# FudanCVL/SynFMC

Measured on AMD Instinct MI355X. Metric: denoising steps/sec, 16x320x512 bf16 U-Net+CMC+OMC, higher is better.
Workload: dtype bf16; 1 GPU; 16x320x512 clip, CFG batch 2, full-width 3D U-Net (1.39B params, random init) + Camera Adapter (CMC) + Object Motion Control (OMC) features, DDIM step; configs/obj.yaml shapes; 1 clip per GPU; frames=16, height=320, width=512, hip_graph=True, fp8_temporal_attention=False, parallelism=dp1 (independent clips, no collective)

## Files before the change

include/fmc_hip.h:

```cpp
#ifndef FMC_HIP_H
#define FMC_HIP_H

#include <stdint.h>

#ifdef __cplusplus
extern "C" {
#endif

#define FMC_VERSION 100

enum { FMC_BF16 = 0, FMC_F32 = 1 };

enum {
    FMC_OK = 0,
    FMC_E_SHAPE = -1,
    FMC_E_DTYPE = -2,
    FMC_E_ALIGN = -3,
    FMC_E_LAUNCH = -4,
    FMC_E_NULL = -5
};

int fmc_version(void);
const char* fmc_last_error(void);

int64_t fmc_groupnorm_workspace_bytes(int N, int C, int G);
int fmc_groupnorm_silu_fwd(const void* x, void* y, const float* gamma, const float* beta, float* stats,
                           void* workspace, int N, int HW, int C, int G, float eps, int act, int dtype,
                           const void* x2, int C1, void* stream);
int fmc_groupnorm_silu_bwd(const void* dy, const void* x, void* dx, const float* gamma, const float* beta,
                           const float* stats, void* workspace, int N, int HW, int C, int G, int act,
                           int dtype, void* stream);

int fmc_layernorm_fwd(const void* x, void* y, const float* gamma, const float* beta, const float* pe,
                      int64_t M, int C, float eps, int pe_inner, int pe_frames, int dtype, void* stream);
int fmc_layernorm_add_fwd(const void* x, const void* addend, void* sum_out, void* y, const float* gamma, const float* beta,
                          const float* pe, int64_t M, int C, float eps, int pe_inner, int pe_frames, int dtype, void* stream);

int fmc_geglu_fwd(const void* x, void* y, int64_t M, int Cff, int dtype, void* stream);

int fmc_spatial_attn_fwd(const void* q, const void* k, const void* v, void* o, float* lse, int B, int H,
                         int Sq, int Skv, int D, int64_t q_batch_stride, int64_t q_row_stride,
                         int64_t kv_batch_stride, int64_t kv_row_stride, int64_t o_batch_stride,
                         int64_t o_row_stride, int kv_batch_div, float scale, int dtype, void* stream);

int fmc_temporal_attn_fwd(const void* q, const void* k, const void* v, void* o, int n_clips, int n_pix,
                          int F, int H, int D, int64_t clip_stride, int64_t frame_stride,
                          int64_t pix_stride, int64_t o_clip_stride, int64_t o_frame_stride,
                          int64_t o_pix_stride, float scale, int dtype, void* stream);

int fmc_plucker_fwd(const float* K, const float* c2w, void* out, int B, int F, int H, int W, int c2w_rows,
                    int layout, int dtype, void* stream);

int fmc_omc_rasterize_fwd(const float* poses, const float* masks, void* feat, float* mask_out, int BF,
                          int n_obj, int H, int W, int layout, int dtype, void* stream);

int fmc_gaussian_circle_mask_fwd(const float* circles, float* out, int N, int H, int W, void* stream);

int fmc_mask_modulate_fwd(const void* x, const float* mask_in, void* y, float* mask_out, int N, int h, int w,
                          int C, int Hin, int Win, int dtype, void* stream);

int fmc_feature_add_fwd(const void* h, const void* t, void* out, int64_t n_elems, int64_t skip_elems,
                        int dtype, void* stream);

int fmc_cfg_ddim_step(const void* eps_uc, const float* x, float* x_out, int64_t n, int has_uncond,
                      float guidance, float alpha_t, float alpha_prev, int dtype, void* stream);

typedef struct fmc_sampler_coef {
    float g;
    float m_x, m_e, m_clamp;
    float c_x, c_e, c_m, c_n;
    float c_h[3];
    float in_scale;
} fmc_sampler_coef;
int64_t fmc_sampler_step_elems_per_trip(void);
int fmc_sampler_step(const void* eps_uc, const float* x, const void* noise, const float* hist0, const float* hist1,
                     const float* hist2, float* x_out, float* m_out, void* x_in, int64_t n, int has_uncond, int n_hist,
                     int in_reps, fmc_sampler_coef coef, int dtype, int in_dtype, void* stream);

int fmc_linear_bf16(const void* x, const void* w, const void* bias, const void* residual, void* out, int64_t M, int N,
                    int K, int64_t ldx, int64_t ldres, int64_t ldo, float alpha, int epilogue, int tile, int split_k,
                    void* workspace, int64_t workspace_bytes, const void* x2, int64_t ldx2, int k_split,
                    const void* residual2, void* stream);

int fmc_conv3x3_bf16(const void* x, const void* w, const void* bias, const void* temb, const void* residual, void* out,
                     int n_img, int H, int W, int Cin, int Cout, int64_t temb_row_stride, int temb_img_div,
                     int upsample2x, int tile, int split_k, void* workspace, int64_t workspace_bytes, void* stream);

int fmc_linear_bf16_gn(const void* x, const void* w, const void* bias, const void* residual, void* out, int64_t M, int N, int K,
                       int64_t ldx, int64_t ldres, int64_t ldo, float alpha, const void* residual2, float* gn_partials, int gn_hw,
                       int w_tilemajor, void* stream);
int fmc_linear_bf16_ln(const void* x, const void* w, const void* bias, const void* residual, void* out, int64_t M, int N, int K,
                       int64_t ldx, int64_t ldres, int64_t ldo, float alpha, const void* residual2, void* ln_out, const float* ln_gamma,
                       const float* ln_beta, float ln_eps, const float* ln_pe, int ln_pe_inner, int ln_pe_frames, float* ln_stats, int w_tilemajor,
                       void* stream);
int fmc_linear_bf16_lnc(const void* x, const void* w_gamma, void* out, int64_t M, int N, int K, int64_t ldx, int64_t ldo, int epilogue,
                        const float* ln_stats, const float* ln_c, const float* ln_bias, int w_tilemajor, void* stream);
int fmc_linear_bf16_ffblk(const void* x, const void* w, const void* bias, const void* residual, void* out, int64_t M, int N, int K,
                          int64_t ldres, float alpha, int epilogue, int x_blocked, int out_blocked, const float* ln_stats, const float* ln_c,
                          const float* ln_bias, int w_tilemajor, void* stream);
int fmc_groupnorm_fold_linear(const float* partials, int part_splits, const float* gamma, const float* beta, const void* w, const void* bias,
                              void* w_out, float* bias_out, int n_img, int HW, int C, int G, int N, float eps, int w_tilemajor, void* stream);
int fmc_linear_bf16_imgw(const void* x, const void* w_img, const float* bias_img, void* out, int64_t M, int N, int K, int64_t ldx, int64_t ldo,
                         int img_rows, float* ln_stats, float ln_eps, int w_tilemajor, void* stream);
int fmc_linear_bf16_fftail(const void* x_blocked, const void* x2, const void* w, const void* bias, const void* residual, void* out, int64_t M,
                           int N, int K, int k_split, int64_t ldx2, int64_t ldres, float* gn_partials, int gn_hw, int w_tilemajor, void* stream);
int fmc_conv3x3_bf16_gn(const void* x, const void* w, const void* bias, const void* temb, const void* residual, void* out, int n_img,
                        int H, int W, int Cin, int Cout, int64_t temb_row_stride, int temb_img_div, int upsample2x,
                        float* gn_partials, int w_tilemajor, void* stream);
int fmc_groupnorm_apply_fwd(const void* x, void* y, const float* gamma, const float* beta, float* stats, const float* partials,
                            int part_splits, int N, int HW, int C, int G, float eps, int act, int dtype, void* stream);

int fmc_linear4_supported(int64_t M, int N, int K, int64_t ldx);
int fmc_linear4_bf16(const void* x, const void* w, const void* bias, const void* residual, const void* residual2, void* out, int64_t M, int N, int K,
                     int64_t ldx, int64_t ldres, int64_t ldo, float alpha, void* stream);

int fmc_vendor_init(void);
int fmc_vendor_destroy(void);
int fmc_vendor_version(void);
int64_t fmc_vendor_workspace_bytes(void);
int fmc_vendor_linear_candidates(int64_t M, int N, int K, int64_t ldx, int64_t ldres, int64_t ldo, int has_bias, int has_residual);
int fmc_vendor_linear_bf16(const void* x, const void* w, const void* bias, const void* residual, void* out, int64_t M, int N, int K,
                           int64_t ldx, int64_t ldres, int64_t ldo, int algo, void* workspace, int64_t workspace_bytes, void* stream);

int fmc_attention_supported(int D);
int fmc_attention_fwd(const void* q, const void* k, const void* v, void* o, const unsigned char* key_keep, int B, int H, int Sq, int Skv, int D,
                      int64_t q_batch_stride, int64_t q_row_stride, int64_t kv_batch_stride, int64_t kv_row_stride, int64_t o_batch_stride,
                      int64_t o_row_stride, float scale, int causal, int dtype, void* stream);

int fmc_geglu_pipe_supported(int64_t M, int cff, int C, int variant);
int fmc_geglu_pipe_ln_bf16(const void* h, void* out, const float* ln_gamma, const float* ln_beta, float ln_eps, const void* w_packed, const void* bias,
                           int64_t M, int cff, int C, int out_blocked, int variant, void* stream);

int fmc_groupnorm_partial_splits(int HW, int C);
int fmc_groupnorm_partials(const void* x, const void* x2, int C1, float* partials, int N, int HW, int C, int G, int dtype, void* stream);
int fmc_conv3x3_halo_supported(int n_img, int H, int W, int Cin, int Cin1, int Cout, int upsample2x);
int64_t fmc_conv3x3_halo_packed_bytes(int Cin, int Cout);
int fmc_conv3x3_halo_pack_weight(const void* w, void* dst, int Cin, int Cout, void* stream);
int fmc_conv3x3_halo_tiles_per_image(int H, int W);
int fmc_conv3x3_halo_bf16(const void* x, const void* x2, int Cin1, const void* w_packed, const void* bias, const void* temb, const void* residual,
                          void* out, int n_img, int H, int W, int Cin, int Cout, int64_t temb_row_stride, int temb_img_div, int upsample2x,
                          const float* gn_coef, int gn_act, float* gn_partials, void* stream);
int fmc_conv3x3_halo4_supported(int n_img, int H, int W, int Cin, int Cin1, int Cout, int upsample2x, int wide);
int fmc_conv3x3_halo4_pack_weight(const void* w, void* dst, int Cin, int Cout, int wide, void* stream);
int fmc_conv3x3_halo4_row_blocks_per_image(int H, int W);
int fmc_conv3x3_halo4_tiles(int n_img, int H, int W, int Cout, int wide);
int fmc_conv3x3_halo4_bf16(const void* x, const void* x2, int Cin1, const void* w_packed, const void* bias, const void* temb, const void* residual,
                           void* out, int n_img, int H, int W, int Cin, int Cout, int64_t temb_row_stride, int temb_img_div, int upsample2x,
                           float* gn_partials, int split_k, void* workspace, int64_t workspace_bytes, int wide, void* stream);
int64_t fmc_conv3x3_upfold_packed_bytes(int Cin, int Cout);
int fmc_conv3x3_upfold_pack_weight(const void* w, void* dst, int Cin, int Cout, int tile_channels, void* stream);
int fmc_conv3x3_halo_fold_supported(int n_img, int Hs, int Ws, int Cin, int Cout);
int fmc_conv3x3_halo_fold_bf16(const void* x, const void* w_folded, const void* bias, void* out, int n_img, int Hs, int Ws, int Cin, int Cout,
                               float* gn_partials, void* stream);
int fmc_conv3x3_halo4_fold_supported(int n_img, int Hs, int Ws, int Cin, int Cout, int wide);
int fmc_conv3x3_halo4_fold_bf16(const void* x, const void* w_folded, const void* bias, void* out, int n_img, int Hs, int Ws, int Cin, int Cout,
                                float* gn_partials, int wide, void* stream);
int fmc_conv3x3_down_bwd_supported(int n_img, int H, int W, int Cin, int Cout);
int64_t fmc_conv3x3_down_bwd_packed_bytes(int Cin, int Cout);
int fmc_conv3x3_down_bwd_pack_weight(const void* w, void* dst, int Cin, int Cout, void* stream);
int fmc_conv3x3_down_bwd_tile(int n_img, int H, int W, int Cin, int Cout);
int fmc_conv3x3_down_bwd_bf16(const void* dy, const void* w_packed, void* dx, int n_img, int H, int W, int Cin, int Cout, int tile, void* stream);
int fmc_conv3x3_up_bwd_supported(int n_img, int Hs, int Ws, int Cin, int Cout);
int64_t fmc_conv3x3_up_bwd_packed_bytes(int Cin, int Cout);
int fmc_conv3x3_up_bwd_pack_weight(const void* w, void* dst, int Cin, int Cout, void* stream);
int fmc_conv3x3_up_bwd_tile(int n_img, int Hs, int Ws, int Cin, int Cout);
int fmc_conv3x3_up_bwd_bf16(const void* dy, const void* w_packed, void* dx, int n_img, int Hs, int Ws, int Cin, int Cout, int tile, void* stream);
int fmc_groupnorm_coef(const float* partials, int part_splits, const float* gamma, const float* beta, float* coef, float* stats, int N, int HW,
                       int C, int G, float eps, void* stream);

int fmc_split_bf16x3(const float* src, void* dst, int64_t rows, int C, int64_t ld_src, int64_t ld_dst, int col0, int K,
                     int role, void* stream);
int fmc_linear_x3_f32(const void* x3, const void* w3, const float* bias, const float* residual, float* out, int64_t M, int N,
                      int K3, int64_t ldx, int64_t ldres, int64_t ldo, float alpha, int epilogue, int tile, int split_k,
                      void* workspace, int64_t workspace_bytes, const float* residual2, void* stream);
int fmc_conv3x3_x3_f32(const void* x3, const void* w3, const float* bias, const float* temb, const float* residual, float* out,
                       int n_img, int H, int W, int Cin3, int Cout, int64_t temb_row_stride, int temb_img_div,
                       int upsample2x, int tile, int split_k, void* workspace, int64_t workspace_bytes, void* stream);

int fmc_layernorm_bwd(const void* dy, const void* x, const float* gamma, void* dx, float* dgamma, float* dbeta,
                      int64_t M, int C, float eps, int dtype, void* stream);
int fmc_layernorm_bwd_add(const void* dy, const void* x, const float* gamma, void* dx, float* dgamma, float* dbeta, const void* addend,
                          int64_t M, int C, float eps, int dtype, void* stream);
int fmc_groupnorm_silu_bwd_add(const void* dy, const void* x, void* dx, const float* gamma, const float* beta, const float* stats,
                               void* workspace, int N, int HW, int C, int G, int act, const void* addend, int dtype, void* stream);
int64_t fmc_groupnorm_silu_bwd_params_workspace_bytes(int N, int HW, int C, int G);
int fmc_groupnorm_silu_bwd_params(const void* dy, const void* x, void* dx, float* dgamma, float* dbeta, const float* gamma,
                                  const float* beta, const float* stats, const void* addend, int accumulate, void* workspace,
                                  int N, int HW, int C, int G, int act, int dtype, void* stream);
int64_t fmc_column_sum_workspace_bytes(int64_t M, int N);
int fmc_column_sum(const void* x, float* out, int64_t M, int N, int64_t ld, float alpha, int accumulate, void* workspace, int dtype,
                   void* stream);
int fmc_geglu_bwd(const void* dy, const void* x, void* dx, int64_t M, int Cff, int dtype, void* stream);
int fmc_spatial_attn_bwd(const void* q, const void* k, const void* v, const void* o, const void* d_o, const float* lse,
                         float* dvec, void* dq, void* dk, void* dv, int B, int H, int Sq, int Skv, int D,
                         int64_t q_batch_stride, int64_t q_row_stride, int64_t kv_batch_stride, int64_t kv_row_stride,
                         int64_t o_batch_stride, int64_t o_row_stride, int64_t dq_batch_stride, int64_t dq_row_stride,
                         int64_t dkv_batch_stride, int64_t dkv_row_stride, int kv_batch_div, float scale, int dtype,
                         void* stream);
int fmc_temporal_attn_bwd(const void* q, const void* k, const void* v, const void* d_o, void* dq, void* dk, void* dv,
                          int n_clips, int n_pix, int F, int H, int D, int64_t clip_stride, int64_t frame_stride,
                          int64_t pix_stride, int64_t do_clip_stride, int64_t do_frame_stride, int64_t do_pix_stride,
                          int64_t dq_clip_stride, int64_t dq_frame_stride, int64_t dq_pix_stride, float scale,
                          int dtype, void* stream);

int fmc_fp8_scales_roll(void* amax, void* scale, void* inv_scale, float margin, void* stream);
int fmc_linear_fp8_qkv(const void* x, const void* w, void* out_fp8, int64_t M, int N, int K, int64_t ldx,
                       const void* inv_scales, void* amax_bits, void* stream);
int fmc_temporal_attn_fp8_fwd(const void* q, const void* k, const void* v, void* o, const void* scales, int n_clips,
                              int n_pix, int F, int H, int D, int64_t clip_stride, int64_t frame_stride,
                              int64_t pix_stride, int64_t o_clip_stride, int64_t o_frame_stride, int64_t o_pix_stride,
                              float scale, void* stream);
int fmc_temporal_attn_fp8_bwd(const void* q, const void* k, const void* v, const void* scales, const void* d_o, void* dq,
                              void* dk, void* dv, int n_clips, int n_pix, int F, int H, int D, int64_t clip_stride,
                              int64_t frame_stride, int64_t pix_stride, int64_t do_clip_stride, int64_t do_frame_stride,
                              int64_t do_pix_stride, int64_t dq_clip_stride, int64_t dq_frame_stride,
                              int64_t dq_pix_stride, float scale, void* stream);

int fmc_nhwc_to_cmajor_padded(const void* src, void* dst, int n_img, int H, int W, int C, int64_t row_len, int guard,
                              int shifts, void* stream);

typedef struct fmc_wgrad_problem {
    const void* a;
    const void* b;
    float* out;
    int64_t M, lda, ldb, ldo;
    int N, K;
    float alpha;
    int accumulate;
} fmc_wgrad_problem;
int64_t fmc_linear_wgrad_workspace_bytes(const fmc_wgrad_problem* problems, int n_problems);
int fmc_linear_wgrad_bf16(const fmc_wgrad_problem* problems, int n_problems, void* workspace, int64_t workspace_bytes, void* stream);

int fmc_temporal_block_bf16(const void* h, void* out, const float* ln_gamma, const float* ln_bpe, float ln_eps, const void* w_merge_tm,
                            const void* pose_term, float merge_scale, const void* w_qkv_packed, const void* w_out_tm, const void* b_out,
                            float* ln_stats, float ln_stats_eps, int n_clips, int frames, int hw, int channels, int heads, float scale,
                            void* stream);
int fmc_xattn_block640_bf16(const void* h, void* out, const float* ln_gamma, const float* ln_bpe, float ln_eps, const void* w_q_packed,
                            const void* kvfrag, const void* w_out_frag, const void* b_out, int n_images, int hw, int n_keys, int images_per_text,
                            float scale, void* stream);
int fmc_xattn_pack_kv(const void* kv, void* out, int batch, int S, int64_t ld_batch, void* stream);
int fmc_xattn_block320_bf16(const void* h, void* out, const float* ln_gamma, const float* ln_bpe, float ln_eps, const void* w_q_packed,
                            const void* kvfrag, const void* w_out_tm, const void* b_out, float* ln_stats, float ln_stats_eps, int n_images, int hw,
                            int n_keys, int images_per_text, float scale, void* stream);
int fmc_xattn_pack_kv40(const void* kv, void* out, int batch, int S, int64_t ld_batch, void* stream);
int fmc_geglu640_ln_bf16(const void* h, void* out, const float* ln_gamma, const float* ln_beta, float ln_eps, const void* w_packed, const void* bias,
                         int64_t M, int cff, int out_blocked, void* stream);
int fmc_geglu320_ln_bf16(const void* h, void* out, const float* ln_gamma, const float* ln_beta, float ln_eps, const void* w_packed, const void* bias,
                         int64_t M, int cff, int out_blocked, void* stream);
int fmc_temporal_block_set_debug(void* buf);

enum { FMC_OPTIM_ZERO_GRAD = 1 };
typedef struct fmc_optim_tensor {
    float* p;
    float* g;
    float* m;
    float* v;
    uint16_t* shadow_bf16;
    float* shadow_f32;
    float* step;
    int64_t n;
    int32_t clip_group;
    int32_t hyper_group;
    int32_t flags;
    int32_t reserved;
} fmc_optim_tensor;
typedef struct fmc_optim_chunk {
    int32_t tensor;
    int32_t chunk;
} fmc_optim_chunk;
int fmc_optim_chunk_elems(void);
int64_t fmc_optim_workspace_bytes(int n_tensors, int n_chunks, int n_clip_groups);
int fmc_optim_check_tables(const fmc_optim_tensor* h_tensors, int n_tensors, const fmc_optim_chunk* h_chunks, int n_chunks, int n_hyper,
                           int n_clip_groups);
int fmc_optim_grad_norm(const fmc_optim_tensor* tensors, int n_tensors, const fmc_optim_chunk* chunks, int n_chunks, const float* hyper,
                        int n_hyper, int n_clip_groups, void* workspace, int64_t workspace_bytes, void* stream);
int fmc_optim_adamw_step(const fmc_optim_tensor* tensors, int n_tensors, const fmc_optim_chunk* chunks, int n_chunks, const float* hyper,
                         int n_hyper, int n_clip_groups, void* workspace, int64_t workspace_bytes, void* stream);

#ifdef __cplusplus
}
#endif
#endif
```

synfmc_amd/_lib.py:

```python
from __future__ import annotations

import ctypes
import os
from ctypes import c_char_p, c_float, c_int, c_int64, c_void_p

_HERE = os.path.dirname(os.path.abspath(__file__))
LIB_PATH = os.environ.get("FMC_HIP_LIB") or os.path.join(_HERE, "lib", "libfmc_hip.so")

FMC_BF16, FMC_F32 = 0, 1

_ERRORS = {-1: ValueError, -2: TypeError, -3: ValueError, -4: RuntimeError, -5: ValueError}


class SamplerCoef(ctypes.Structure):
    _fields_ = [("g", c_float), ("m_x", c_float), ("m_e", c_float), ("m_clamp", c_float), ("c_x", c_float), ("c_e", c_float),
                ("c_m", c_float), ("c_n", c_float), ("c_h", c_float * 3), ("in_scale", c_float)]

SIGNATURES = {
    "fmc_version": (c_int, []),
    "fmc_last_error": (c_char_p, []),
    "fmc_groupnorm_workspace_bytes": (c_int64, [c_int, c_int, c_int]),
    "fmc_groupnorm_silu_fwd": (c_int, [c_void_p, c_void_p, c_void_p, c_void_p, c_void_p, c_void_p, c_int, c_int, c_int,
                                       c_int, c_float, c_int, c_int, c_void_p, c_int, c_void_p]),
    "fmc_groupnorm_silu_bwd": (c_int, [c_void_p, c_void_p, c_void_p, c_void_p, c_void_p, c_void_p, c_void_p, c_int,
                                       c_int, c_int, c_int, c_int, c_int, c_void_p]),
    "fmc_layernorm_add_fwd": (c_int, [c_void_p, c_void_p, c_void_p, c_void_p, c_void_p, c_void_p, c_void_p, c_int64, c_int, c_float, c_int,
                                      c_int, c_int, c_void_p]),
    "fmc_layernorm_fwd": (c_int, [c_void_p, c_void_p, c_void_p, c_void_p, c_void_p, c_int64, c_int, c_float, c_int,
                                  c_int, c_int, c_void_p]),
    "fmc_geglu_fwd": (c_int, [c_void_p, c_void_p, c_int64, c_int, c_int, c_void_p]),
    "fmc_spatial_attn_fwd": (c_int, [c_void_p, c_void_p, c_void_p, c_void_p, c_void_p, c_int, c_int, c_int, c_int, c_int,
                                     c_int64, c_int64, c_int64, c_int64, c_int64, c_int64, c_int, c_float, c_int,
                                     c_void_p]),
    "fmc_temporal_attn_fwd": (c_int, [c_void_p, c_void_p, c_void_p, c_void_p, c_int, c_int, c_int, c_int, c_int,
                                      c_int64, c_int64, c_int64, c_int64, c_int64, c_int64, c_float, c_int, c_void_p]),
    "fmc_plucker_fwd": (c_int, [c_void_p, c_void_p, c_void_p, c_int, c_int, c_int, c_int, c_int, c_int, c_int, c_void_p]),
    "fmc_omc_rasterize_fwd": (c_int, [c_void_p, c_void_p, c_void_p, c_void_p, c_int, c_int, c_int, c_int, c_int, c_int,
                                      c_void_p]),
    "fmc_gaussian_circle_mask_fwd": (c_int, [c_void_p, c_void_p, c_int, c_int, c_int, c_void_p]),
    "fmc_mask_modulate_fwd": (c_int, [c_void_p, c_void_p, c_void_p, c_void_p, c_int, c_int, c_int, c_int, c_int, c_int,
                                      c_int, c_void_p]),
    "fmc_feature_add_fwd": (c_int, [c_void_p, c_void_p, c_void_p, c_int64, c_int64, c_int, c_void_p]),
    "fmc_cfg_ddim_step": (c_int, [c_void_p, c_void_p, c_void_p, c_int64, c_int, c_float, c_float, c_float, c_int,
                                  c_void_p]),
    "fmc_sampler_step_elems_per_trip": (c_int64, []),
    "fmc_sampler_step": (c_int, [c_void_p] * 9 + [c_int64, c_int, c_int, c_int, SamplerCoef, c_int, c_int, c_void_p]),
    "fmc_linear_bf16": (c_int, [c_void_p, c_void_p, c_void_p, c_void_p, c_void_p, c_int64, c_int, c_int, c_int64,
                                c_int64, c_int64, c_float, c_int, c_int, c_int, c_void_p, c_int64, c_void_p, c_int64, c_int,
                                c_void_p, c_void_p]),
    "fmc_linear_bf16_gn": (c_int, [c_void_p, c_void_p, c_void_p, c_void_p, c_void_p, c_int64, c_int, c_int, c_int64, c_int64, c_int64,
                                   c_float, c_void_p, c_void_p, c_int, c_int, c_void_p]),
    "fmc_linear_bf16_ln": (c_int, [c_void_p, c_void_p, c_void_p, c_void_p, c_void_p, c_int64, c_int, c_int, c_int64, c_int64, c_int64,
                                   c_float, c_void_p, c_void_p, c_void_p, c_void_p, c_float, c_void_p, c_int, c_int, c_void_p, c_int, c_void_p]),
    "fmc_linear_bf16_lnc": (c_int, [c_void_p, c_void_p, c_void_p, c_int64, c_int, c_int, c_int64, c_int64, c_int, c_void_p, c_void_p, c_void_p,
                                    c_int, c_void_p]),
    "fmc_linear_bf16_ffblk": (c_int, [c_void_p, c_void_p, c_void_p, c_void_p, c_void_p, c_int64, c_int, c_int, c_int64, c_float, c_int, c_int, c_int,
                                      c_void_p, c_void_p, c_void_p, c_int, c_void_p]),
    "fmc_groupnorm_fold_linear": (c_int, [c_void_p, c_int, c_void_p, c_void_p, c_void_p, c_void_p, c_void_p, c_void_p, c_int, c_int, c_int, c_int, c_int,
                                          c_float, c_int, c_void_p]),
    "fmc_linear_bf16_imgw": (c_int, [c_void_p, c_void_p, c_void_p, c_void_p, c_int64, c_int, c_int, c_int64, c_int64, c_int, c_void_p, c_float, c_int,
                                     c_void_p]),
    "fmc_linear_bf16_fftail": (c_int, [c_void_p, c_void_p, c_void_p, c_void_p, c_void_p, c_void_p, c_int64, c_int, c_int, c_int, c_int64, c_int64,
                                       c_void_p, c_int, c_int, c_void_p]),
    "fmc_conv3x3_bf16_gn": (c_int, [c_void_p, c_void_p, c_void_p, c_void_p, c_void_p, c_void_p, c_int, c_int, c_int, c_int, c_int,
                                    c_int64, c_int, c_int, c_void_p, c_int, c_void_p]),
    "fmc_groupnorm_partial_splits": (c_int, [c_int, c_int]),
    "fmc_groupnorm_partials": (c_int, [c_void_p, c_void_p, c_int, c_void_p, c_int, c_int, c_int, c_int, c_int, c_void_p]),
    "fmc_conv3x3_halo_supported": (c_int, [c_int, c_int, c_int, c_int, c_int, c_int, c_int]),
    "fmc_conv3x3_halo_packed_bytes": (c_int64, [c_int, c_int]),
    "fmc_conv3x3_halo_pack_weight": (c_int, [c_void_p, c_void_p, c_int, c_int, c_void_p]),
    "fmc_conv3x3_halo_tiles_per_image": (c_int, [c_int, c_int]),
    "fmc_conv3x3_halo_bf16": (c_int, [c_void_p, c_void_p, c_int, c_void_p, c_void_p, c_void_p, c_void_p, c_void_p, c_int, c_int, c_int, c_int, c_int,
                                      c_int64, c_int, c_int, c_void_p, c_int, c_void_p, c_void_p]),
    "fmc_conv3x3_halo4_supported": (c_int, [c_int, c_int, c_int, c_int, c_int, c_int, c_int, c_int]),
    "fmc_conv3x3_halo4_pack_weight": (c_int, [c_void_p, c_void_p, c_int, c_int, c_int, c_void_p]),
    "fmc_conv3x3_halo4_row_blocks_per_image": (c_int, [c_int, c_int]),
    "fmc_conv3x3_halo4_tiles": (c_int, [c_int, c_int, c_int, c_int, c_int]),
    "fmc_conv3x3_halo4_bf16": (c_int, [c_void_p, c_void_p, c_int, c_void_p, c_void_p, c_void_p, c_void_p, c_void_p, c_int, c_int, c_int, c_int, c_int,
                                       c_int64, c_int, c_int, c_void_p, c_int, c_void_p, c_int64, c_int, c_void_p]),
    "fmc_conv3x3_upfold_packed_bytes": (c_int64, [c_int, c_int]),
    "fmc_conv3x3_upfold_pack_weight": (c_int, [c_void_p, c_void_p, c_int, c_int, c_int, c_void_p]),
    "fmc_conv3x3_halo_fold_supported": (c_int, [c_int, c_int, c_int, c_int, c_int]),
    "fmc_conv3x3_halo_fold_bf16": (c_int, [c_void_p, c_void_p, c_void_p, c_void_p, c_int, c_int, c_int, c_int, c_int, c_void_p, c_void_p]),
    "fmc_conv3x3_halo4_fold_supported": (c_int, [c_int, c_int, c_int, c_int, c_int, c_int]),
    "fmc_conv3x3_halo4_fold_bf16": (c_int, [c_void_p, c_void_p, c_void_p, c_void_p, c_int, c_int, c_int, c_int, c_int, c_void_p, c_int, c_void_p]),
    "fmc_conv3x3_down_bwd_supported": (c_int, [c_int, c_int, c_int, c_int, c_int]),
    "fmc_conv3x3_down_bwd_packed_bytes": (c_int64, [c_int, c_int]),
    "fmc_conv3x3_down_bwd_pack_weight": (c_int, [c_void_p, c_void_p, c_int, c_int, c_void_p]),
    "fmc_conv3x3_down_bwd_tile": (c_int, [c_int, c_int, c_int, c_int, c_int]),
    "fmc_conv3x3_down_bwd_bf16": (c_int, [c_void_p, c_void_p, c_void_p, c_int, c_int, c_int, c_int, c_int, c_int, c_void_p]),
    "fmc_conv3x3_up_bwd_supported": (c_int, [c_int, c_int, c_int, c_int, c_int]),
    "fmc_conv3x3_up_bwd_packed_bytes": (c_int64, [c_int, c_int]),
    "fmc_conv3x3_up_bwd_pack_weight": (c_int, [c_void_p, c_void_p, c_int, c_int, c_void_p]),
    "fmc_conv3x3_up_bwd_tile": (c_int, [c_int, c_int, c_int, c_int, c_int]),
    "fmc_conv3x3_up_bwd_bf16": (c_int, [c_void_p, c_void_p, c_void_p, c_int, c_int, c_int, c_int, c_int, c_int, c_void_p]),
    "fmc_linear4_supported": (c_int, [c_int64, c_int, c_int, c_int64]),
    "fmc_vendor_linear_candidates": (c_int, [c_int64, c_int, c_int, c_int64, c_int64, c_int64, c_int, c_int]),
    "fmc_vendor_linear_bf16": (c_int, [c_void_p, c_void_p, c_void_p, c_void_p, c_void_p, c_int64, c_int, c_int, c_int64, c_int64, c_int64, c_int, c_void_p,
                                       c_int64, c_void_p]),
    "fmc_geglu_pipe_supported": (c_int, [c_int64, c_int, c_int, c_int]),
    "fmc_geglu_pipe_ln_bf16": (c_int, [c_void_p, c_void_p, c_void_p, c_void_p, c_float, c_void_p, c_void_p, c_int64, c_int, c_int, c_int, c_int, c_void_p]),
    "fmc_attention_supported": (c_int, [c_int]),
    "fmc_attention_fwd": (c_int, [c_void_p, c_void_p, c_void_p, c_void_p, c_void_p, c_int, c_int, c_int, c_int, c_int, c_int64, c_int64, c_int64, c_int64,
                                  c_int64, c_int64, c_float, c_int, c_int, c_void_p]),
    "fmc_vendor_init": (c_int, []),
    "fmc_vendor_destroy": (c_int, []),
    "fmc_vendor_version": (c_int, []),
    "fmc_vendor_workspace_bytes": (c_int64, []),
    "fmc_linear4_bf16": (c_int, [c_void_p, c_void_p, c_void_p, c_void_p, c_void_p, c_void_p, c_int64, c_int, c_int, c_int64, c_int64, c_int64, c_float, c_void_p]),
    "fmc_groupnorm_coef": (c_int, [c_void_p, c_int, c_void_p, c_void_p, c_void_p, c_void_p, c_int, c_int, c_int, c_int, c_float, c_void_p]),
    "fmc_groupnorm_apply_fwd": (c_int, [c_void_p, c_void_p, c_void_p, c_void_p, c_void_p, c_void_p, c_int, c_int, c_int, c_int, c_int,
                                        c_float, c_int, c_int, c_void_p]),
    "fmc_split_bf16x3": (c_int, [c_void_p, c_void_p, c_int64, c_int, c_int64, c_int64, c_int, c_int, c_int, c_void_p]),
    "fmc_linear_x3_f32": (c_int, [c_void_p, c_void_p, c_void_p, c_void_p, c_void_p, c_int64, c_int, c_int, c_int64,
                                  c_int64, c_int64, c_float, c_int, c_int, c_int, c_void_p, c_int64, c_void_p, c_void_p]),
    "fmc_conv3x3_x3_f32": (c_int, [c_void_p, c_void_p, c_void_p, c_void_p, c_void_p, c_void_p, c_int, c_int, c_int,
                                   c_int, c_int, c_int64, c_int, c_int, c_int, c_int, c_void_p, c_int64, c_void_p]),
    "fmc_layernorm_bwd": (c_int, [c_void_p, c_void_p, c_void_p, c_void_p, c_void_p, c_void_p, c_int64, c_int, c_float,
                                  c_int, c_void_p]),
    "fmc_layernorm_bwd_add": (c_int, [c_void_p, c_void_p, c_void_p, c_void_p, c_void_p, c_void_p, c_void_p, c_int64, c_int, c_float,
                                      c_int, c_void_p]),
    "fmc_groupnorm_silu_bwd_add": (c_int, [c_void_p, c_void_p, c_void_p, c_void_p, c_void_p, c_void_p, c_void_p, c_int, c_int, c_int, c_int,
                                           c_int, c_void_p, c_int, c_void_p]),
    "fmc_groupnorm_silu_bwd_params_workspace_bytes": (c_int64, [c_int, c_int, c_int, c_int]),
    "fmc_groupnorm_silu_bwd_params": (c_int, [c_void_p] * 9 + [c_int, c_void_p] + [c_int] * 6 + [c_void_p]),
    "fmc_column_sum_workspace_bytes": (c_int64, [c_int64, c_int]),
    "fmc_column_sum": (c_int, [c_void_p, c_void_p, c_int64, c_int, c_int64, c_float, c_int, c_void_p, c_int, c_void_p]),
    "fmc_geglu_bwd": (c_int, [c_void_p, c_void_p, c_void_p, c_int64, c_int, c_int, c_void_p]),
    "fmc_spatial_attn_bwd": (c_int, [c_void_p] * 10 + [c_int] * 5 + [c_int64] * 10 + [c_int, c_float, c_int, c_void_p]),
    "fmc_temporal_attn_bwd": (c_int, [c_void_p] * 7 + [c_int] * 5 + [c_int64] * 9 + [c_float, c_int, c_void_p]),
    "fmc_fp8_scales_roll": (c_int, [c_void_p, c_void_p, c_void_p, c_float, c_void_p]),
    "fmc_linear_fp8_qkv": (c_int, [c_void_p, c_void_p, c_void_p, c_int64, c_int, c_int, c_int64, c_void_p, c_void_p, c_void_p]),
    "fmc_temporal_attn_fp8_fwd": (c_int, [c_void_p] * 5 + [c_int] * 5 + [c_int64] * 6 + [c_float, c_void_p]),
    "fmc_temporal_attn_fp8_bwd": (c_int, [c_void_p] * 8 + [c_int] * 5 + [c_int64] * 9 + [c_float, c_void_p]),
    "fmc_nhwc_to_cmajor_padded": (c_int, [c_void_p, c_void_p, c_int, c_int, c_int, c_int, c_int64, c_int, c_int, c_void_p]),
    "fmc_linear_wgrad_workspace_bytes": (c_int64, [c_void_p, c_int]),
    "fmc_linear_wgrad_bf16": (c_int, [c_void_p, c_int, c_void_p, c_int64, c_void_p]),
    "fmc_optim_chunk_elems": (c_int, []),
    "fmc_optim_workspace_bytes": (c_int64, [c_int, c_int, c_int]),
    "fmc_optim_check_tables": (c_int, [c_void_p, c_int, c_void_p, c_int, c_int, c_int]),
    "fmc_optim_grad_norm": (c_int, [c_void_p, c_int, c_void_p, c_int, c_void_p, c_int, c_int, c_void_p, c_int64, c_void_p]),
    "fmc_optim_adamw_step": (c_int, [c_void_p, c_int, c_void_p, c_int, c_void_p, c_int, c_int, c_void_p, c_int64, c_void_p]),
    "fmc_temporal_block_bf16": (c_int, [c_void_p, c_void_p, c_void_p, c_void_p, c_float, c_void_p, c_void_p, c_float, c_void_p, c_void_p, c_void_p,
                                        c_void_p, c_float, c_int, c_int, c_int, c_int, c_int, c_float, c_void_p]),
    "fmc_temporal_block_set_debug": (c_int, [c_void_p]),
    "fmc_xattn_block640_bf16": (c_int, [c_void_p, c_void_p, c_void_p, c_void_p, c_float, c_void_p, c_void_p, c_void_p, c_void_p, c_int, c_int, c_int, c_int,
                                        c_float, c_void_p]),
    "fmc_xattn_pack_kv": (c_int, [c_void_p, c_void_p, c_int, c_int, c_int64, c_void_p]),
    "fmc_geglu320_ln_bf16": (c_int, [c_void_p, c_void_p, c_void_p, c_void_p, c_float, c_void_p, c_void_p, c_int64, c_int, c_int, c_void_p]),
    "fmc_geglu640_ln_bf16": (c_int, [c_void_p, c_void_p, c_void_p, c_void_p, c_float, c_void_p, c_void_p, c_int64, c_int, c_int, c_void_p]),
    "fmc_xattn_pack_kv40": (c_int, [c_void_p, c_void_p, c_int, c_int, c_int64, c_void_p]),
    "fmc_xattn_block320_bf16": (c_int, [c_void_p, c_void_p, c_void_p, c_void_p, c_float, c_void_p, c_void_p, c_void_p, c_void_p, c_void_p, c_float,
                                        c_int, c_int, c_int, c_int, c_float, c_void_p]),
    "fmc_conv3x3_bf16": (c_int, [c_void_p, c_void_p, c_void_p, c_void_p, c_void_p, c_void_p, c_int, c_int, c_int,
                                 c_int, c_int, c_int64, c_int, c_int, c_int, c_int, c_void_p, c_int64, c_void_p]),
}

_lib = None


class FmcLibraryMissing(ImportError):
    pass


def load() -> ctypes.CDLL:
    global _lib
    if _lib is not None:
        return _lib
    if not os.path.isfile(LIB_PATH):
        raise FmcLibraryMissing(
            f"{LIB_PATH} not found: build it with `make -C synfmc_amd/csrc` (hipcc --offload-arch=gfx950). "
            "There is no fallback path.")
    import torch
    lib = ctypes.CDLL(LIB_PATH)
    for name, (res, args) in SIGNATURES.items():
        fn = getattr(lib, name)
        fn.restype, fn.argtypes = res, args
    _lib = lib
    return lib


def check(rc: int, what: str) -> None:
    if rc != 0:
        msg = load().fmc_last_error()
        raise _ERRORS.get(rc, RuntimeError)(f"{what} failed ({rc}): {msg.decode() if msg else '?'}")
```

synfmc_amd/csrc/conv_halo.hip:

```cpp
#include "conv_halo_common.h"

namespace {

using halo::IC;
constexpr int TH = 10, TW = 32, BM = TH * TW, BN = 160;
constexpr int HWID = TW + 2, HPIX = (TH + 2) * HWID;
constexpr int NP = 416;
constexpr int PLANE = NP * 16;
constexpr int HALO = 8 * PLANE;
constexpr int NBW = 5;
constexpr int WSUB = BN * 64;
constexpr int OFF_W = 2 * HALO, OFF_COEF = OFF_W + NBW * WSUB;
constexpr int LDS_BYTES = OFF_COEF + 2 * 512;
constexpr int NPIECE = 7;

struct CHParams : halo::Params {
    const float* gn_coef; int gn_act;
    float* gn_part;
    int tiles_y, tiles_x, tiles_n;
    int64_t x_bytes, x2_bytes, w_bytes;
};

__device__ __forceinline__ float silu_fast(float z) { return z * __builtin_amdgcn_rcpf(1.f + __builtin_amdgcn_exp2f(-1.4426950408889634f * z)); }

constexpr int nh(int i) { return (i >= 0 && i <= 12 && (i & 1) == 0) ? 1 : 0; }

constexpr int nhp(int i) { return (i >= 0 && i <= 3) ? (i < 3 ? 2 : 1) : 0; }

template <int GN, bool PH = false>
__global__ __launch_bounds__(512, 2)
void conv_halo_kernel(const CHParams P) {
    extern __shared__ __attribute__((aligned(16))) unsigned char smem_raw[];
    const int tid = threadIdx.x, lane = tid & 63;
    const int wave = __builtin_amdgcn_readfirstlane(tid >> 6);
    const int half = wave >> 2, wq = wave & 3;
    const int wc = wq & 1, wr = half * 2 + (wq >> 1);
    const int l15 = lane & 15, kq = lane >> 4;
    const bool clsA = wave < 2;

    int tile_p, tile_n;
    {
        const int total = P.n_img * P.tiles_y * P.tiles_x * P.tiles_n;
        const int id = blockIdx.x, q = total >> 3, r = total & 7, xcd = id & 7;
        const int lin = (xcd < r ? xcd * (q + 1) : r * (q + 1) + (xcd - r) * q) + (id >> 3);
        tile_p = lin / P.tiles_n;
        tile_n = lin - tile_p * P.tiles_n;
    }
    const int tpi = P.tiles_y * P.tiles_x;
    const int img = tile_p / tpi, tin = tile_p - img * tpi;
    const int y0 = (tin / P.tiles_x) * TH, x0 = (tin % P.tiles_x) * TW;
    constexpr int NS = PH ? 8 : 18;
    const int tn1 = P.cout / BN;
    const int phase = PH ? tile_n / tn1 : 0, py = phase >> 1, px_ = phase & 1;
    const int n0 = (tile_n - phase * tn1) * BN;
    const int nchunk = P.cin >> 6, nsub = nchunk * NS;

    const int Hs = P.ups ? P.H >> 1 : P.H, Ws = P.ups ? P.W >> 1 : P.W;
    const int pp = lane & 7, pg = ((lane & 7) + (lane >> 3)) & 7;
    int h_pix[NPIECE];
#pragma unroll
    for (int j = 0; j < NPIECE; ++j) {
        const int b = 8 * j + wave, px = 8 * b + pp;
        const int hy = px / HWID, hx = px - hy * HWID;
        const int y = y0 - 1 + hy, x = x0 - 1 + hx;
        const bool in = b < HPIX / 8 && (unsigned)y < (unsigned)P.H && (unsigned)x < (unsigned)P.W;
        const int ys = P.ups ? y >> 1 : y, xs = P.ups ? x >> 1 : x;
        h_pix[j] = in ? (img * Hs + ys) * Ws + xs : -1;
    }
    const int h_lds = pg * PLANE + (8 * wave + pp) * 16;
    const bool last_piece = wave < HPIX / 8 - 48;
    const __amdgpu_buffer_rsrc_t rsX = __builtin_amdgcn_make_buffer_rsrc((void*)P.x, 0, (int)P.x_bytes, 0x00020000);
    const __amdgpu_buffer_rsrc_t rsX2 = __builtin_amdgcn_make_buffer_rsrc((void*)(P.x2 ? P.x2 : P.x), 0, (int)(P.x2 ? P.x2_bytes : P.x_bytes), 0x00020000);
    const __amdgpu_buffer_rsrc_t rsW = __builtin_amdgcn_make_buffer_rsrc((void*)P.w, 0, (int)P.w_bytes, 0x00020000);
    const int c2 = P.cin - P.c1;
    u32x4 hreg[2];
    auto halo_load = [&](int j, int ch64, u32x4& dst) { dst = halo::piece_load(rsX, rsX2, P.c1, c2, h_pix[j], pg, ch64 * 64, ch64, nchunk); };
    auto halo_transform = [&](int j, int coefbuf, const u32x4& raw) -> u32x4 {
        if constexpr (GN == 0) return raw;
        const f32x4* src = reinterpret_cast<const f32x4*>(smem_raw + OFF_COEF + coefbuf * 512 + pg * 64);
        float f[8];
#pragma unroll
        for (int k = 0; k < 4; ++k) { f[2 * k] = __uint_as_float(raw[k] << 16); f[2 * k + 1] = __uint_as_float(raw[k] & 0xffff0000u); }
#pragma unroll
        for (int k = 0; k < 4; ++k) {
            const f32x4 t = src[k];
            const float z0 = fmaf(f[2 * k], t[0], t[1]), z1 = fmaf(f[2 * k + 1], t[2], t[3]);
            f[2 * k] = GN == 1 ? silu_fast(z0) : z0;
            f[2 * k + 1] = GN == 1 ? silu_fast(z1) : z1;
        }
        const bool in = h_pix[j] >= 0;
        u32x4 v;
#pragma unroll
        for (int k = 0; k < 4; ++k) v[k] = in ? pack_bf2(f[2 * k], f[2 * k + 1]) : 0u;
        return v;
    };
    auto halo_store = [&](int j, int buf, const u32x4& v) {
        if (j == NPIECE - 1 && !last_piece) return;
        *reinterpret_cast<u32x4*>(smem_raw + buf * HALO + h_lds + j * 1024) = v;
    };
    auto coef_fetch = [&](int ch64) -> float {
        const int cc = ch64 < nchunk ? ch64 : nchunk - 1;
        const float* src = GN ? P.gn_coef + ((size_t)img * P.cin + cc * 64) * 2 + (tid & 127) : reinterpret_cast<const float*>(P.w);
        return *src;
    };

    const int my_piece = clsA ? 2 * wave : wave + 2;
    const unsigned w_vo0 = (unsigned)(lane * 16 + my_piece * 1024);
    const int w_dst0 = OFF_W + my_piece * 1024;
    halo::WStream<NBW, WSUB, 1024> ws;
    ws.start(tile_n * nsub * WSUB, nsub);
    auto w_issue = [&](auto cls) { ws.template issue<decltype(cls)::value>(smem_raw, rsW, w_vo0, w_dst0, 0, tile_n * nsub * WSUB, nsub); };

    f32x4 acc[5][5];
    bf16x8 wf[5], af[5];
    const int wfrag = OFF_W + ((wc * 80 + l15) * 32 + (kq ^ (3 * ((l15 >> 3) & 1))) * 8) * 2;
    int afrag[5];
#pragma unroll
    for (int mb = 0; mb < 5; ++mb) {
        const int idx = wr * 80 + mb * 16 + l15, ty = idx >> 5, tx = idx & 31;
        afrag[mb] = kq * PLANE + (ty * HWID + tx) * 16 + (PH ? (py * HWID + px_) * 16 : 0);
    }

    {
        u32x4 t[NPIECE];
#pragma unroll
        for (int j = 0; j < NPIECE; ++j) halo_load(j, 0, t[j]);
        const float c0v = coef_fetch(0), c1v = coef_fetch(1);
        if (tid < 128) {
            *reinterpret_cast<float*>(smem_raw + OFF_COEF + tid * 4) = c0v;
            *reinterpret_cast<float*>(smem_raw + OFF_COEF + 512 + tid * 4) = c1v;
        }
        __syncthreads();
#pragma unroll
        for (int j = 0; j < NPIECE; ++j) halo_store(j, 0, halo_transform(j, 0, t[j]));
    }
    asm volatile("s_waitcnt vmcnt(0) lgkmcnt(0)" ::: "memory");

    auto main_loop = [&](auto cls) {
        constexpr int NW = decltype(cls)::value ? 2 : 1;
        int rd_slot = 0;
        w_issue(cls); w_issue(cls); w_issue(cls);
        asm volatile("s_waitcnt vmcnt(%0)" ::"n"(2 * NW) : "memory");
        __builtin_amdgcn_s_barrier();
        if (half == 1) __builtin_amdgcn_s_barrier();
        __builtin_amdgcn_sched_barrier(0);
#pragma unroll
        for (int a = 0; a < 5; ++a)
#pragma unroll
            for (int b = 0; b < 5; ++b) acc[a][b] = f32x4{0.f, 0.f, 0.f, 0.f};
        __builtin_amdgcn_sched_barrier(0);

        int cbuf = 0;
        float coef_next = 0.f;
        u32x4 hpk = {0u, 0u, 0u, 0u};
        u32x4 hregp[3][2];
        for (int c = 0; c < nchunk; ++c) {
            const int abase = cbuf * HALO, nbuf = cbuf ^ 1;
            if constexpr (PH) {
                static_assert(!PH || GN == 0, "the phase mode has no GroupNorm operand path");
                auto subp = [&](auto ic) {
                    constexpr int i = decltype(ic)::value;
                    constexpr int tap = i >> 1, hk = i & 1, ta = tap >> 1, tb = tap & 1;
                    constexpr int aimm = hk * 4 * PLANE + (ta * HWID + tb) * 16;
                    if constexpr (nhp(i - 3) >= 1) halo_store(2 * (i - 3), nbuf, hregp[(i - 3) % 3][0]);
                    if constexpr (nhp(i - 3) == 2) halo_store(2 * (i - 3) + 1, nbuf, hregp[(i - 3) % 3][1]);
                    {
                        const unsigned char* Wp = smem_raw + wfrag + rd_slot * WSUB;
#pragma unroll
                        for (int nb = 0; nb < 5; ++nb) wf[nb] = __builtin_bit_cast(bf16x8, *reinterpret_cast<const u32x4*>(Wp + nb * 1024));
#pragma unroll
                        for (int mb = 0; mb < 5; ++mb)
                            af[mb] = __builtin_bit_cast(bf16x8, *reinterpret_cast<const u32x4*>(smem_raw + abase + afrag[mb] + aimm));
                        rd_slot = rd_slot + 1 == NBW ? 0 : rd_slot + 1;
                    }
                    if constexpr (nhp(i) >= 1) halo_load(2 * i, c + 1, hregp[i % 3][0]);
                    if constexpr (nhp(i) == 2) halo_load(2 * i + 1, c + 1, hregp[i % 3][1]);
                    w_issue(cls);
                    {
                        constexpr int extra = nhp(i - 1) + nhp(i);
                        asm volatile("s_waitcnt vmcnt(%0)" ::"n"(2 * NW + extra) : "memory");
                    }
                    __builtin_amdgcn_sched_barrier(0);
                    __builtin_amdgcn_s_barrier();
                    __builtin_amdgcn_sched_barrier(0);
                    __builtin_amdgcn_s_setprio(1);
#pragma unroll
                    for (int mb = 0; mb < 5; ++mb)
#pragma unroll
                        for (int nb = 0; nb < 5; ++nb)
                            acc[mb][nb] = __builtin_amdgcn_mfma_f32_16x16x32_bf16(wf[nb], af[mb], acc[mb][nb], 0, 0, 0);
                    __builtin_amdgcn_s_setprio(0);
                    __builtin_amdgcn_sched_barrier(0);
                    __builtin_amdgcn_s_barrier();
                    __builtin_amdgcn_sched_barrier(0);
                };
                subp(IC<0>{}); subp(IC<1>{}); subp(IC<2>{}); subp(IC<3>{}); subp(IC<4>{}); subp(IC<5>{}); subp(IC<6>{}); subp(IC<7>{});
                cbuf = nbuf;
                continue;
            }
            auto sub = [&](auto ic) {
                constexpr int i = decltype(ic)::value;
                constexpr int tap = i >> 1, hk = i & 1, ky = tap / 3, kx = tap % 3;
                constexpr int aimm = hk * 4 * PLANE + (ky * HWID + kx) * 16;
                if constexpr (i >= 3 && i <= 15 && (i & 1) == 1) halo_store((i - 3) / 2, nbuf, hpk);
                if constexpr (i == 16) {
                    if (tid < 128) *reinterpret_cast<float*>(smem_raw + OFF_COEF + cbuf * 512 + tid * 4) = coef_next;
                }
                {
                    const unsigned char* Wp = smem_raw + wfrag + rd_slot * WSUB;
#pragma unroll
                    for (int nb = 0; nb < 5; ++nb) wf[nb] = __builtin_bit_cast(bf16x8, *reinterpret_cast<const u32x4*>(Wp + nb * 1024));
#pragma unroll
                    for (int mb = 0; mb < 5; ++mb)
                        af[mb] = __builtin_bit_cast(bf16x8, *reinterpret_cast<const u32x4*>(smem_raw + abase + afrag[mb] + aimm));
                    rd_slot = rd_slot + 1 == NBW ? 0 : rd_slot + 1;
                }
                if constexpr (nh(i) == 1) halo_load(i / 2, c + 1, hreg[(i / 2) & 1]);
                if constexpr (i == 13) coef_next = coef_fetch(c + 2);
                w_issue(cls);
                {
                    constexpr int extra = nh(i - 1) + nh(i) + (i == 13 || i == 14 ? 1 : 0);
                    asm volatile("s_waitcnt vmcnt(%0)" ::"n"(2 * NW + extra) : "memory");
                }
                __builtin_amdgcn_sched_barrier(0);
                __builtin_amdgcn_s_barrier();
                __builtin_amdgcn_sched_barrier(0);
                __builtin_amdgcn_s_setprio(1);
                if constexpr (i >= 2 && i <= 14 && (i & 1) == 0) hpk = halo_transform((i - 2) / 2, nbuf, hreg[((i - 2) / 2) & 1]);
#pragma unroll
                for (int mb = 0; mb < 5; ++mb)
#pragma unroll
                    for (int nb = 0; nb < 5; ++nb)
                        acc[mb][nb] = __builtin_amdgcn_mfma_f32_16x16x32_bf16(wf[nb], af[mb], acc[mb][nb], 0, 0, 0);
                if constexpr (GN != 0 && i >= 2 && i <= 14 && (i & 1) == 0) {
#pragma unroll
                    for (int k = 0; k < 25; ++k) {
                        __builtin_amdgcn_sched_group_barrier(0x008, 1, 0);
                        __builtin_amdgcn_sched_group_barrier(0x102, 3, 0);
                    }
                }
                __builtin_amdgcn_s_setprio(0);
                __builtin_amdgcn_sched_barrier(0);
                __builtin_amdgcn_s_barrier();
                __builtin_amdgcn_sched_barrier(0);
            };
            sub(IC<0>{}); sub(IC<1>{}); sub(IC<2>{}); sub(IC<3>{}); sub(IC<4>{}); sub(IC<5>{});
            sub(IC<6>{}); sub(IC<7>{}); sub(IC<8>{}); sub(IC<9>{}); sub(IC<10>{}); sub(IC<11>{});
            sub(IC<12>{}); sub(IC<13>{}); sub(IC<14>{}); sub(IC<15>{}); sub(IC<16>{}); sub(IC<17>{});
            cbuf = nbuf;
        }
    };
    if (clsA) main_loop(std::true_type{}); else main_loop(std::false_type{});
    if (half == 0) __builtin_amdgcn_s_barrier();
    asm volatile("s_waitcnt vmcnt(0)" ::: "memory");
    __syncthreads();

    constexpr int OP = BN + 8;
    bf16_t* Os = reinterpret_cast<bf16_t*>(smem_raw);
    constexpr int CPR = BN / 8;
    const int vrows = min(TH, P.H - y0) * TW;
    auto row_pixel = [&](int r) -> int64_t {
        if constexpr (PH) return ((int64_t)img * (2 * P.H) + 2 * (y0 + (r >> 5)) + py) * (2 * P.W) + 2 * (x0 + (r & 31)) + px_;
        return ((int64_t)img * P.H + y0 + (r >> 5)) * P.W + x0 + (r & 31);
    };
    {
        u32x2 bt[5], tt[5];
        if (P.bias) {
#pragma unroll
            for (int nb = 0; nb < 5; ++nb) bt[nb] = *reinterpret_cast<const u32x2*>(P.bias + n0 + wc * 80 + nb * 16 + 4 * kq);
        }
        if (P.temb) {
            const bf16_t* trow = P.temb + (int64_t)(img / P.temb_div) * P.temb_ld + n0 + wc * 80 + 4 * kq;
#pragma unroll
            for (int nb = 0; nb < 5; ++nb) tt[nb] = *reinterpret_cast<const u32x2*>(trow + nb * 16);
        }
#pragma unroll
        for (int nb = 0; nb < 5; ++nb) {
            float b4[4] = {0.f, 0.f, 0.f, 0.f};
            if (P.bias) {
                b4[0] = __uint_as_float(bt[nb][0] << 16); b4[1] = __uint_as_float(bt[nb][0] & 0xffff0000u);
                b4[2] = __uint_as_float(bt[nb][1] << 16); b4[3] = __uint_as_float(bt[nb][1] & 0xffff0000u);
            }
            if (P.temb) {
                b4[0] += __uint_as_float(tt[nb][0] << 16); b4[1] += __uint_as_float(tt[nb][0] & 0xffff0000u);
                b4[2] += __uint_as_float(tt[nb][1] << 16); b4[3] += __uint_as_float(tt[nb][1] & 0xffff0000u);
            }
#pragma unroll
            for (int mb = 0; mb < 5; ++mb)
#pragma unroll
                for (int j = 0; j < 4; ++j) acc[mb][nb][j] += b4[j];
        }
    }
    if (P.res) {
#pragma unroll
        for (int h = 0; h < 2; ++h) {
            u32x4 rv[7];
#pragma unroll
            for (int it = 0; it < 7; ++it) {
                const int cidx = min(tid + (7 * h + it) * 512, BM * CPR - 1), r = cidx / CPR, ch = cidx - r * CPR;
                rv[it] = *reinterpret_cast<const u32x4*>(P.res + row_pixel(r < vrows ? r : 0) * P.cout + n0 + ch * 8);
            }
#pragma unroll
            for (int it = 0; it < 7; ++it) {
                const int cidx = tid + (7 * h + it) * 512, r = cidx / CPR, ch = cidx - r * CPR;
                if (cidx < BM * CPR) *reinterpret_cast<u32x4*>(Os + r * OP + ch * 8) = rv[it];
            }
        }
        __syncthreads();
#pragma unroll
        for (int mb = 0; mb < 5; ++mb)
#pragma unroll
            for (int nb = 0; nb < 5; ++nb) {
                const u32x2 t = *reinterpret_cast<const u32x2*>(Os + (wr * 80 + mb * 16 + l15) * OP + wc * 80 + nb * 16 + 4 * kq);
                acc[mb][nb][0] += __uint_as_float(t[0] << 16); acc[mb][nb][1] += __uint_as_float(t[0] & 0xffff0000u);
                acc[mb][nb][2] += __uint_as_float(t[1] << 16); acc[mb][nb][3] += __uint_as_float(t[1] & 0xffff0000u);
            }
        __syncthreads();
    }
#pragma unroll
    for (int mb = 0; mb < 5; ++mb)
#pragma unroll
        for (int nb = 0; nb < 5; ++nb)
            *reinterpret_cast<u32x2*>(Os + (wr * 80 + mb * 16 + l15) * OP + wc * 80 + nb * 16 + 4 * kq) =
                u32x2{pack_bf2(acc[mb][nb][0], acc[mb][nb][1]), pack_bf2(acc[mb][nb][2], acc[mb][nb][3])};
    __syncthreads();
    float gs = 0.f, gss = 0.f;
    const int cpg = P.cout >> 5, GT = BN / cpg, RP = 512 / GT;
    if (P.gn_part) {
        const int gl = tid % GT;
        for (int r = tid / GT; r < vrows; r += RP) {
            const unsigned* wsrc = reinterpret_cast<const unsigned*>(Os + r * OP + gl * cpg);
            for (int k = 0; k < cpg / 2; ++k) {
                const unsigned u = wsrc[k];
                const float a = __uint_as_float(u << 16), b = __uint_as_float(u & 0xffff0000u);
                gs += a + b;
                gss += a * a + b * b;
            }
        }
    }
    for (int cidx = tid; cidx < BM * CPR; cidx += 512) {
        const int r = cidx / CPR, ch = cidx - r * CPR;
        if (r < vrows)
            *reinterpret_cast<u32x4*>(P.out + row_pixel(r) * P.cout + n0 + ch * 8) = *reinterpret_cast<const u32x4*>(Os + r * OP + ch * 8);
    }
    if (P.gn_part) {
        float* red = reinterpret_cast<float*>(smem_raw + (size_t)BM * OP * 2);
        red[2 * tid] = gs;
        red[2 * tid + 1] = gss;
        __syncthreads();
        if (tid < GT) {
            float a = 0.f, b = 0.f;
            for (int k = 0; k < RP; ++k) { a += red[2 * (tid + k * GT)]; b += red[2 * (tid + k * GT) + 1]; }
            float* dst = P.gn_part + ((PH ? ((int64_t)img * tpi + tin) * 4 + phase : (int64_t)img * tpi + tin) * 32 + (n0 / cpg + tid)) * 2;
            dst[0] = a;
            dst[1] = b;
        }
    }
}

__global__ __launch_bounds__(256) void conv_halo_pack_kernel(const bf16_t* __restrict__ w, bf16_t* __restrict__ dst, int cout, int cin, int BN) {
    const int64_t total = (int64_t)cout * 9 * cin / 8;
    for (int64_t id = (int64_t)blockIdx.x * blockDim.x + threadIdx.x; id < total; id += (int64_t)gridDim.x * blockDim.x) {
        int64_t t = id;
        const int p = (int)(t & 3); t >>= 2;
        const int row = (int)(t % BN); t /= BN;
        const int hk = (int)(t & 1); t >>= 1;
        const int tap = (int)(t % 9); t /= 9;
        const int nchunk = cin >> 6;
        const int ch64 = (int)(t % nchunk); t /= nchunk;
        const int nt = (int)t;
        const int lc = p ^ (3 * ((row >> 3) & 1));
        const int64_t src = (((int64_t)(nt * BN + row) * 9 + tap) * cin + ch64 * 64 + hk * 32 + lc * 8);
        *reinterpret_cast<u32x4*>(dst + id * 8) = *reinterpret_cast<const u32x4*>(w + src);
    }
}

__global__ __launch_bounds__(256) void conv_upfold_pack_kernel(const bf16_t* __restrict__ w, bf16_t* __restrict__ dst, int cout, int cin, int BN) {
    const int64_t total = (int64_t)cout * 16 * cin / 8;
    const int nchunk = cin >> 6, tn1 = cout / BN;
    for (int64_t id = (int64_t)blockIdx.x * blockDim.x + threadIdx.x; id < total; id += (int64_t)gridDim.x * blockDim.x) {
        int64_t t = id;
        const int p = (int)(t & 3); t >>= 2;
        const int row = (int)(t % BN); t /= BN;
        const int hk = (int)(t & 1); t >>= 1;
        const int tap = (int)(t & 3); t >>= 2;
        const int ch64 = (int)(t % nchunk); t /= nchunk;
        const int nt = (int)(t % tn1), phase = (int)(t / tn1);
        const int py = phase >> 1, px = phase & 1, ta = tap >> 1, tb = tap & 1;
        const int ky0 = py == 0 ? ta : 2 * ta, ky1 = py == 0 ? 2 * ta : ta + 1;
        const int kx0 = px == 0 ? tb : 2 * tb, kx1 = px == 0 ? 2 * tb : tb + 1;
        const int lc = p ^ (3 * ((row >> 3) & 1));
        float v[8] = {0.f, 0.f, 0.f, 0.f, 0.f, 0.f, 0.f, 0.f};
        for (int ky = ky0; ky <= ky1; ++ky)
            for (int kx = kx0; kx <= kx1; ++kx) {
                float f[8];
                Vec8<bf16_t>::unpack(Vec8<bf16_t>::load_raw(w + (((int64_t)(nt * BN + row) * 9 + ky * 3 + kx) * cin + ch64 * 64 + hk * 32 + lc * 8)), f);
#pragma unroll
                for (int k = 0; k < 8; ++k) v[k] += f[k];
            }
        Vec8<bf16_t>::store(dst + id * 8, v);
    }
}

__global__ __launch_bounds__(256) void gn_coef_kernel(const float* __restrict__ part, int splits, const float* __restrict__ gamma,
                                                      const float* __restrict__ beta, float* __restrict__ coef, float* __restrict__ stats,
                                                      int C, int G, double count, float eps) {
    __shared__ float s_mean[64], s_rstd[64];
    const int n = blockIdx.x;
    if ((int)threadIdx.x < G) {
        double a = 0.0, b = 0.0;
        for (int s = 0; s < splits; ++s) {
            const float* p = part + (((int64_t)n * splits + s) * G + threadIdx.x) * 2;
            a += (double)p[0];
            b += (double)p[1];
        }
        const double mean = a / count;
        double var = b / count - mean * mean;
        if (var < 0.0) var = 0.0;
        const float rstd = (float)(1.0 / sqrt(var + (double)eps));
        s_mean[threadIdx.x] = (float)mean;
        s_rstd[threadIdx.x] = rstd;
        if (stats) { stats[((int64_t)n * G + threadIdx.x) * 2] = (float)mean; stats[((int64_t)n * G + threadIdx.x) * 2 + 1] = rstd; }
    }
    __syncthreads();
    const int cpg = C / G;
    for (int c = threadIdx.x; c < C; c += blockDim.x) {
        const int g = c / cpg;
        const float a = s_rstd[g] * gamma[c];
        coef[((int64_t)n * C + c) * 2] = a;
        coef[((int64_t)n * C + c) * 2 + 1] = beta[c] - s_mean[g] * a;
    }
}

}

void halo::pack_filter(const bf16_t* w, bf16_t* dst, int Cin, int Cout, int bn, hipStream_t st) {
    const int64_t chunks = (int64_t)Cout * 9 * Cin / 8;
    const int grid = (int)((chunks + 255) / 256 < 4096 ? (chunks + 255) / 256 : 4096);
    hipLaunchKernelGGL(conv_halo_pack_kernel, dim3(grid), dim3(256), 0, st, w, dst, Cout, Cin, bn);
}

extern "C" int64_t fmc_conv3x3_halo_packed_bytes(int Cin, int Cout) { return (int64_t)Cout * 9 * Cin * 2; }

extern "C" int fmc_conv3x3_halo_pack_weight(const void* w, void* dst, int Cin, int Cout, void* stream) {
    if (!w || !dst) FMC_FAIL(FMC_E_NULL, "conv3x3_halo_pack_weight: NULL pointer");
    if (Cin % 64 || Cout % BN) FMC_FAIL(FMC_E_SHAPE, "conv3x3_halo_pack_weight: Cin %% 64 / Cout %% 160 (Cin=%d Cout=%d)", Cin, Cout);
    if (!fmc_aligned16(w) || !fmc_aligned16(dst)) FMC_FAIL(FMC_E_ALIGN, "conv3x3_halo_pack_weight: pointers must be 16-byte aligned");
    halo::pack_filter((const bf16_t*)w, (bf16_t*)dst, Cin, Cout, BN, (hipStream_t)stream);
    FMC_CHECK_LAUNCH("fmc_conv3x3_halo_pack_weight");
    return 0;
}

extern "C" int fmc_conv3x3_halo_supported(int n_img, int H, int W, int Cin, int Cin1, int Cout, int upsample2x) {
    if (n_img < 1 || H < 1 || W < 1 || W % TW || Cin % 64 || Cout % BN) return 0;
    if (Cin1 <= 0 || Cin1 > Cin || Cin1 % 64) return 0;
    if (upsample2x && ((H | W) & 1)) return 0;
    const int64_t hs = upsample2x ? H / 2 : H, ws = upsample2x ? W / 2 : W;
    if ((int64_t)n_img * hs * ws * Cin1 * 2 >= (1ll << 31) || (int64_t)n_img * hs * ws * (Cin - Cin1) * 2 >= (1ll << 31)) return 0;
    if ((int64_t)Cout * 9 * Cin * 2 >= (1ll << 31)) return 0;
    return 1;
}

extern "C" int fmc_conv3x3_halo_bf16(const void* x, const void* x2, int Cin1, const void* w_packed, const void* bias, const void* temb,
                                     const void* residual, void* out, int n_img, int H, int W, int Cin, int Cout, int64_t temb_row_stride,
                                     int temb_img_div, int upsample2x, const float* gn_coef, int gn_act, float* gn_partials, void* stream) {
    if (!x2) Cin1 = Cin;
    if (int e = halo::check_args("conv3x3_halo", true, x, x2, w_packed, bias, temb, residual, out, temb_row_stride, temb_img_div, gn_partials, Cout, BN,
                                 fmc_conv3x3_halo_supported(n_img, H, W, Cin, Cin1, Cout, upsample2x),
                                 "%s: needs W %% 32 == 0, Cin %% 64 == 0 (both sources), Cout %% 160 == 0, operands < 2 GiB "
                                 "(n=%d H=%d W=%d Cin=%d+%d Cout=%d ups=%d)", n_img, H, W, Cin1, Cin - Cin1, Cout, upsample2x))
        return e;
    CHParams P;
    halo::fill_params(P, x, x2, Cin1, w_packed, bias, temb, residual, out, n_img, H, W, Cin, Cout, temb_row_stride, temb_img_div, upsample2x, gn_partials, 9);
    P.gn_coef = gn_coef; P.gn_act = gn_act;
    P.tiles_y = (H + TH - 1) / TH; P.tiles_x = W / TW; P.tiles_n = Cout / BN;
    const unsigned grid = (unsigned)(n_img * P.tiles_y * P.tiles_x * P.tiles_n);
    if (!gn_coef) fmc_launch<conv_halo_kernel<0>>(dim3(grid), dim3(512), LDS_BYTES, (hipStream_t)stream, P);
    else if (gn_act) fmc_launch<conv_halo_kernel<1>>(dim3(grid), dim3(512), LDS_BYTES, (hipStream_t)stream, P);
    else fmc_launch<conv_halo_kernel<2>>(dim3(grid), dim3(512), LDS_BYTES, (hipStream_t)stream, P);
    FMC_CHECK_LAUNCH("fmc_conv3x3_halo_bf16");
    return 0;
}

extern "C" int64_t fmc_conv3x3_upfold_packed_bytes(int Cin, int Cout) { return (int64_t)Cout * 16 * Cin * 2; }

extern "C" int fmc_conv3x3_upfold_pack_weight(const void* w, void* dst, int Cin, int Cout, int tile_channels, void* stream) {
    if (!w || !dst) FMC_FAIL(FMC_E_NULL, "conv3x3_upfold_pack_weight: NULL pointer");
    if ((tile_channels != 80 && tile_channels != 160) || Cin % 64 || Cout % tile_channels)
        FMC_FAIL(FMC_E_SHAPE, "conv3x3_upfold_pack_weight: tile_channels 80 / 160, Cin %% 64, Cout %% tile_channels (Cin=%d Cout=%d tile=%d)", Cin, Cout, tile_channels);
    if (!fmc_aligned16(w) || !fmc_aligned16(dst)) FMC_FAIL(FMC_E_ALIGN, "conv3x3_upfold_pack_weight: pointers must be 16-byte aligned");
    const int64_t chunks = (int64_t)Cout * 16 * Cin / 8;
    const int grid = (int)((chunks + 255) / 256 < 4096 ? (chunks + 255) / 256 : 4096);
    hipLaunchKernelGGL(conv_upfold_pack_kernel, dim3(grid), dim3(256), 0, (hipStream_t)stream, (const bf16_t*)w, (bf16_t*)dst, Cout, Cin, tile_channels);
    FMC_CHECK_LAUNCH("fmc_conv3x3_upfold_pack_weight");
    return 0;
}

extern "C" int fmc_conv3x3_halo_fold_supported(int n_img, int Hs, int Ws, int Cin, int Cout) {
    if (!fmc_conv3x3_halo_supported(n_img, Hs, Ws, Cin, Cin, Cout, 0)) return 0;
    if ((int64_t)Cout * 16 * Cin * 2 >= (1ll << 31)) return 0;
    if ((int64_t)n_img * Hs * Ws * 4 >= (1ll << 31)) return 0;
    return 1;
}

extern "C" int fmc_conv3x3_halo_fold_bf16(const void* x, const void* w_folded, const void* bias, void* out, int n_img, int Hs, int Ws, int Cin,
                                          int Cout, float* gn_partials, void* stream) {
    if (int e = halo::check_args("conv3x3_halo_fold", false, x, nullptr, w_folded, bias, nullptr, nullptr, out, 0, 1, gn_partials, Cout, BN,
                                 fmc_conv3x3_halo_fold_supported(n_img, Hs, Ws, Cin, Cout),
                                 "%s: needs Ws %% 32 == 0, Cin %% 64 == 0, Cout %% 160 == 0, operands < 2 GiB (n=%d Hs=%d Ws=%d Cin=%d Cout=%d)",
                                 n_img, Hs, Ws, Cin, Cout))
        return e;
    CHParams P;
    halo::fill_params(P, x, nullptr, Cin, w_folded, bias, nullptr, nullptr, out, n_img, Hs, Ws, Cin, Cout, 0, 1, 0, gn_partials, 16);
    P.gn_coef = nullptr; P.gn_act = 0;
    P.tiles_y = (Hs + TH - 1) / TH; P.tiles_x = Ws / TW; P.tiles_n = 4 * (Cout / BN);
    const unsigned grid = (unsigned)(n_img * P.tiles_y * P.tiles_x * P.tiles_n);
    fmc_launch<conv_halo_kernel<0, true>>(dim3(grid), dim3(512), LDS_BYTES, (hipStream_t)stream, P);
    FMC_CHECK_LAUNCH("fmc_conv3x3_halo_fold_bf16");
    return 0;
}

extern "C" int fmc_conv3x3_halo_tiles_per_image(int H, int W) { return ((H + TH - 1) / TH) * (W / TW); }

extern "C" int fmc_groupnorm_coef(const float* partials, int part_splits, const float* gamma, const float* beta, float* coef, float* stats,
                                  int N, int HW, int C, int G, float eps, void* stream) {
    if (!partials || !gamma || !beta || !coef) FMC_FAIL(FMC_E_NULL, "groupnorm_coef: NULL pointer");
    if (N < 1 || C < 1 || G < 1 || G > 64 || C % G || part_splits < 1) FMC_FAIL(FMC_E_SHAPE, "groupnorm_coef: N=%d C=%d G=%d splits=%d", N, C, G, part_splits);
    hipLaunchKernelGGL(gn_coef_kernel, dim3((unsigned)N), dim3(256), 0, (hipStream_t)stream, partials, part_splits, gamma, beta, coef, stats, C, G,
                       (double)HW * (double)(C / G), eps);
    FMC_CHECK_LAUNCH("fmc_groupnorm_coef");
    return 0;
}
```

synfmc_amd/csrc/conv_halo_common.h:

```cpp
#pragma once
#include <type_traits>

#include "common.h"

namespace halo {

constexpr unsigned OOB = 0x80000000u;

template <int I> using IC = std::integral_constant<int, I>;

struct Params {
    const bf16_t* x; const bf16_t* x2;
    int c1;
    const bf16_t* w;
    const bf16_t* bias; const bf16_t* temb; const bf16_t* res; bf16_t* out;
    int n_img, H, W, cin, cout, ups;
    int64_t temb_ld; int temb_div;
};

__device__ __forceinline__ u32x4 piece_load(const __amdgpu_buffer_rsrc_t& rsX, const __amdgpu_buffer_rsrc_t& rsX2, int c1, int c2, int hp, int pg,
                                            int cbeg, int crel, int nchunk) {
    const bool second = cbeg >= c1, past = crel >= nchunk;
    const int pitch = past ? 0 : (second ? c2 : c1) * 2;
    const unsigned coff = past ? OOB : (unsigned)(((second ? cbeg - c1 : cbeg) + pg * 8) * 2);
    unsigned vo = (unsigned)(hp * pitch) + coff;
    vo = hp < 0 ? OOB : vo;
    const __amdgpu_buffer_rsrc_t rs = second ? rsX2 : rsX;
    return __builtin_bit_cast(u32x4, __builtin_amdgcn_raw_buffer_load_b128(rs, (int)vo, 0, 0));
}

template <int NBW, int WSUB, int SECOND> struct WStream {
    int slot, left, soff;
    __device__ __forceinline__ void start(int base, int nsub) { soff = base; left = nsub; slot = 0; }
    template <bool TWO>
    __device__ __forceinline__ void issue(unsigned char* smem_raw, const __amdgpu_buffer_rsrc_t& rs, unsigned vo, int ring, int piece, int base, int nsub) {
        unsigned char* dst = smem_raw + ring + slot * WSUB + piece;
        __builtin_amdgcn_raw_ptr_buffer_load_lds(rs, (__attribute__((address_space(3))) void*)dst, 16, (int)vo, soff, 0, 0);
        if constexpr (TWO)
            __builtin_amdgcn_raw_ptr_buffer_load_lds(rs, (__attribute__((address_space(3))) void*)(dst + SECOND), 16, (int)vo, soff + SECOND, 0, 0);
        soff += WSUB;
        if (--left == 0) { left = nsub; soff = base; }
        slot = slot + 1 == NBW ? 0 : slot + 1;
    }
};

void pack_filter(const bf16_t* w, bf16_t* dst, int Cin, int Cout, int bn, hipStream_t st);

template <class... A>
int check_args(const char* name, bool full, const void* x, const void* x2, const void* w, const void* bias, const void* temb, const void* residual,
               const void* out, int64_t temb_row_stride, int temb_img_div, const float* gn_partials, int Cout, int bn, bool shape_ok,
               const char* shape_fmt, A... shape_args) {
    if (!x || !w || !out) FMC_FAIL(FMC_E_NULL, "%s: NULL x / w / out", name);
    if (!shape_ok) FMC_FAIL(FMC_E_SHAPE, shape_fmt, name, shape_args...);
    if (!fmc_aligned16(x) || !fmc_aligned16(w) || !fmc_aligned16(out) || (x2 && !fmc_aligned16(x2)) || (residual && !fmc_aligned16(residual)) ||
        (bias && (reinterpret_cast<uintptr_t>(bias) & 7)) || (temb && ((reinterpret_cast<uintptr_t>(temb) & 7) || temb_row_stride % 4)))
        FMC_FAIL(FMC_E_ALIGN, full ? "%s: x / w / out / residual must be 16-byte aligned, bias / temb rows 8-byte aligned"
                                   : "%s: x / w / out must be 16-byte aligned, bias 8-byte aligned", name);
    if (temb && temb_img_div < 1) FMC_FAIL(FMC_E_SHAPE, "%s: temb_img_div %d", name, temb_img_div);
    if (gn_partials && (Cout % 64 || bn % (Cout / 32)))
        FMC_FAIL(FMC_E_SHAPE, "%s: the statistics epilogue needs Cout %% 64 == 0 and %d %% (Cout / 32) == 0 (Cout=%d)", name, bn, Cout);
    return 0;
}

template <class P_>
void fill_params(P_& P, const void* x, const void* x2, int Cin1, const void* w, const void* bias, const void* temb, const void* residual, void* out,
                 int n_img, int H, int W, int Cin, int Cout, int64_t temb_row_stride, int temb_img_div, int upsample2x, float* gn_partials, int taps) {
    P.x = (const bf16_t*)x; P.x2 = (const bf16_t*)x2; P.c1 = Cin1;
    P.w = (const bf16_t*)w; P.bias = (const bf16_t*)bias; P.temb = (const bf16_t*)temb; P.res = (const bf16_t*)residual; P.out = (bf16_t*)out;
    P.n_img = n_img; P.H = H; P.W = W; P.cin = Cin; P.cout = Cout; P.ups = upsample2x ? 1 : 0;
    P.temb_ld = temb_row_stride; P.temb_div = temb ? temb_img_div : 1;
    P.gn_part = gn_partials;
    const int64_t hs = upsample2x ? H / 2 : H, ws = upsample2x ? W / 2 : W;
    P.x_bytes = (int64_t)n_img * hs * ws * Cin1 * 2; P.x2_bytes = (int64_t)n_img * hs * ws * (Cin - Cin1) * 2;
    P.w_bytes = (int64_t)Cout * taps * Cin * 2;
}

}
```

synfmc_amd/hip_ops.py:

```python
from __future__ import annotations

import atexit
import ctypes
import math
import os
from typing import Optional, Tuple

import torch

from . import _lib
from ._lib import FMC_BF16, FMC_F32
from .derived import derived_on_owner

_DT = {torch.bfloat16: FMC_BF16, torch.float32: FMC_F32}


def _dt(t: torch.Tensor) -> int:
    try:
        return _DT[t.dtype]
    except KeyError:
        raise TypeError(f"fmc kernels take bf16 or fp32 activations, got {t.dtype}") from None


def _dev(*ts: torch.Tensor) -> None:
# ... 1372 lines not shown
            and (ln.pe is None or (ln.pe.dtype == torch.float32 and ln.pe.is_contiguous() and ln.pe.shape[-1] == 320 and ln.pe_inner % 160 == 0
                                   and ln.pe.shape[0] >= ln.pe_frames))
            and (residual is None or (residual.is_contiguous() and residual.dtype == x.dtype))
            and (residual2 is None or residual2.is_contiguous()) and M * max(Kd, 320) * 2 < (1 << 31) and os.environ.get("FMC_G160_PERSIST", "1") != "0")


def carry_ln(src: torch.Tensor, dst: torch.Tensor) -> torch.Tensor:
    tag = getattr(src, "_fmc_ln", None)
    if tag is not None:
        dst._fmc_ln = tag
    return dst


def take_ln(x: torch.Tensor, key) -> Optional[torch.Tensor]:
    tag = getattr(x, "_fmc_ln", None)
    if tag is None or tag[1] != key or torch.is_grad_enabled() or tag[2]:
        return None
    ln_epilogue_calls["consumed"] += 1
    return tag[0].view(x.shape)


def take_ln_stats(x: torch.Tensor, key) -> Optional[torch.Tensor]:
    tag = getattr(x, "_fmc_ln", None)
    if tag is None or tag[1] != key or torch.is_grad_enabled() or not tag[2]:
        return None
    return tag[0]


def pending_ln(x: torch.Tensor, stats: torch.Tensor, gamma: torch.Tensor, beta: torch.Tensor, eps: float) -> torch.Tensor:
    v = x.view(x.shape)
    v._fmc_pending_ln = (stats, gamma, beta, eps)
    return v


def resolve_pending_ln(x: torch.Tensor) -> torch.Tensor:
    pend = getattr(x, "_fmc_pending_ln", None)
    if pend is None:
        return x
    ln_epilogue_calls["materialised"] = ln_epilogue_calls.get("materialised", 0) + 1
    return _layernorm_raw(x.contiguous(), pend[1], pend[2], pend[3], None, 1, 1)


def _ln_folded_weight(weight: torch.Tensor, bias: Optional[torch.Tensor], gamma: torch.Tensor, beta: torch.Tensor):
    def build():
        w32 = weight.detach().float()
        wg = (w32 * gamma.float()[None, :]).to(torch.bfloat16).contiguous()
        b = w32 @ beta.float()
        if bias is not None:
            b = b + bias.detach().float()
        return wg, wg.float().sum(dim=1).contiguous(), b.contiguous()
    tag = (gamma.data_ptr(), gamma._version, beta.data_ptr(), beta._version, None if bias is None else (bias.data_ptr(), bias._version))
    return derived_on_owner(weight, "_fmc_lnw", tag, build)


def lnc_ok(x: torch.Tensor, weight: torch.Tensor) -> bool:
    N, Kd = weight.shape
    M = x.numel() // x.shape[-1]
    return (LN_EPILOGUE and not torch.is_grad_enabled() and x.is_cuda and x.dtype == torch.bfloat16 and weight.dtype == torch.bfloat16
            and x.is_contiguous() and N % 320 == 0 and Kd % 64 == 0 and M % 160 == 0 and (M // 160) * (N // 320) > _cus(x.device)
            and M * max(Kd, 320) * 2 < (1 << 31) and N * Kd * 2 < (1 << 31) and os.environ.get("FMC_G160_PERSIST", "1") != "0")


def linear_lnc(x: torch.Tensor, weight: torch.Tensor, bias, pend, geglu: bool = False) -> torch.Tensor:
    stats, gamma, beta, _ = pend
    wg, c, b = _ln_folded_weight(weight, bias, gamma, beta)
    _dev(x, wg, c, b, stats)
    N, Kd = weight.shape
    M, ldx = _rows2d(x)
    n_out = N // 2 if geglu else N
    out = torch.empty(*x.shape[:-1], n_out, dtype=x.dtype, device=x.device)
    ln_epilogue_calls["consumed"] += 1
    wt = _w_tilemajor(wg) if W_TILEMAJOR else wg
    _log_call("own_linear", (M, N, Kd, "lnc-geglu" if geglu else "lnc", 0), 2.0 * M * N * Kd)
    _lib.check(_lib.load().fmc_linear_bf16_lnc(x.data_ptr(), wt.data_ptr(), out.data_ptr(), M, N, Kd, ldx, n_out, int(geglu), stats.data_ptr(),
                                               c.data_ptr(), b.data_ptr(), int(W_TILEMAJOR), _stream()), "fmc_linear_bf16_lnc")
    return out


def linear_ln(x: torch.Tensor, weight: torch.Tensor, bias, residual, alpha: float, residual2, ln: LnSpec) -> torch.Tensor:
    _dev(x, weight, bias, residual, ln.gamma, ln.beta, ln.pe)
    N, Kd = weight.shape
    M, ldx = _rows2d(x)
    out = torch.empty(*x.shape[:-1], N, dtype=x.dtype, device=x.device)
    ldres = 0 if residual is None else _rows2d(residual)[1]
    ln_epilogue_calls["emitted"] += 1
    if ln.stats_only:
        stats = torch.empty(M, 2, dtype=torch.float32, device=x.device)
        ln_out = None
    else:
        stats, ln_out = None, torch.empty_like(out)
    wt = _w_tilemajor(weight) if W_TILEMAJOR else weight
    _log_call("own_linear", (M, N, Kd, "ln", (residual is not None) + (residual2 is not None)), 2.0 * M * N * Kd)
    _lib.check(_lib.load().fmc_linear_bf16_ln(x.data_ptr(), wt.data_ptr(), _p(bias), _p(residual), out.data_ptr(), M, N, Kd, ldx, ldres, N,
                                              float(alpha), _p(residual2), _p(ln_out), ln.gamma.data_ptr(), ln.beta.data_ptr(), float(ln.eps),
                                              _p(ln.pe), int(ln.pe_inner), int(ln.pe_frames), _p(stats), int(W_TILEMAJOR), _stream()),
               "fmc_linear_bf16_ln")
    out._fmc_ln = (stats, ln.key, True) if ln.stats_only else (ln_out, ln.key, False)
    return out


GN_FOLD = os.environ.get("FMC_GN_FOLD", "1") != "0"
GN_FOLD_MAX_BYTES = 8 << 20


def gn_fold_ok(x: torch.Tensor, gn_tag, groups: int, weight: torch.Tensor, ln: Optional[LnSpec]) -> bool:
    if not GN_FOLD or gn_tag is None or torch.is_grad_enabled() or x.ndim != 3 or weight.ndim != 2:
        return False
    n_img, hw, C = x.shape
    N = weight.shape[0]
    M = n_img * hw
    return (x.is_cuda and x.dtype == torch.bfloat16 and x.is_contiguous() and weight.dtype == torch.bfloat16 and weight.is_contiguous() and weight.shape[1] == C
            and groups == 32 and gn_tag[1] == C and gn_tag[0].shape[0] == n_img and gn_tag[0].shape[1] <= 64 and gn_tag[0].shape[2] == groups
            and hw % 160 == 0 and C % 64 == 0 and N % 320 == 0 and (M // 160) * (N // 320) >= _cus(x.device) and n_img * N * C * 2 <= GN_FOLD_MAX_BYTES
            and M * max(C, N) * 2 < (1 << 31) and (ln is None or (LN_EPILOGUE and ln.stats_only and N == 320))
            and os.environ.get("FMC_G160_PERSIST", "1") != "0")


def linear_gnfold(x: torch.Tensor, gn_tag, gamma: torch.Tensor, beta: torch.Tensor, groups: int, eps: float, weight: torch.Tensor, bias,
                  ln: Optional[LnSpec] = None) -> torch.Tensor:
    part = gn_tag[0]
    _dev(x, part, gamma, beta, weight, bias)
    n_img, hw, C = x.shape
    N = weight.shape[0]
    M = n_img * hw
    lib = _lib.load()
    w_img = torch.empty(n_img, N, C, dtype=torch.bfloat16, device=x.device)
    b_img = torch.empty(n_img, N, dtype=torch.float32, device=x.device)
    gn_epilogue_calls["consumed"] += 1
    _lib.check(lib.fmc_groupnorm_fold_linear(part.data_ptr(), int(part.shape[1]), gamma.data_ptr(), beta.data_ptr(), weight.data_ptr(), _p(bias),
                                             w_img.data_ptr(), b_img.data_ptr(), n_img, hw, C, int(groups), N, float(eps), int(W_TILEMAJOR), _stream()),
               "fmc_groupnorm_fold_linear")
    out = torch.empty(n_img, hw, N, dtype=x.dtype, device=x.device)
    stats = None
    if ln is not None:
        stats = torch.empty(M, 2, dtype=torch.float32, device=x.device)
        ln_epilogue_calls["emitted"] += 1
    _log_call("own_linear", (M, N, C, "gn-fold", 0), 2.0 * M * N * C)
    _lib.check(lib.fmc_linear_bf16_imgw(x.data_ptr(), w_img.data_ptr(), b_img.data_ptr(), out.data_ptr(), M, N, C, C, N, hw, _p(stats),
                                        float(ln.eps) if ln is not None else 0.0, int(W_TILEMAJOR), _stream()), "fmc_linear_bf16_imgw")
    if ln is not None:
        out._fmc_ln = (stats, ln.key, True)
    return out


FF_BLOCKED = os.environ.get("FMC_FF_BLOCKED", "1") != "0"


def ff_blocked_ok(x: torch.Tensor, w1_il160: Optional[torch.Tensor], w2: torch.Tensor, residual) -> bool:
    if not FF_BLOCKED or w1_il160 is None or torch.is_grad_enabled():
        return False
    N1, Kd = w1_il160.shape
    N2, Cff = w2.shape
    M = x.numel() // x.shape[-1]
    return (x.is_cuda and x.dtype == torch.bfloat16 and w1_il160.dtype == torch.bfloat16 and w2.dtype == torch.bfloat16 and x.is_contiguous()
            and w1_il160.is_contiguous() and w2.is_contiguous() and N1 == 2 * Cff and Cff % 160 == 0 and N2 % 320 == 0 and Kd % 64 == 0
            and M % 160 == 0 and M >= 16384 and (M // 160) * (N1 // 320) > _cus(x.device) and M * Cff * 2 < (1 << 31)
            and (residual is None or (residual.is_contiguous() and residual.dtype == x.dtype))
            and os.environ.get("FMC_G160_PERSIST", "1") != "0")


def geglu_linear_blocked(x: torch.Tensor, weight_il160: torch.Tensor, bias_il160) -> torch.Tensor:
    pend = getattr(x, "_fmc_pending_ln", None)
    N, Kd = weight_il160.shape
    M = x.numel() // Kd
    out = torch.empty(*x.shape[:-1], N // 2, dtype=x.dtype, device=x.device)
    if pend is not None:
        stats, gamma, beta, _ = pend
        wg, c, b = _ln_folded_weight(weight_il160, bias_il160, gamma, beta)
        _dev(x, wg, c, b, stats)
        ln_epilogue_calls["consumed"] += 1
        wt = _w_tilemajor(wg) if W_TILEMAJOR else wg
        args = (wt.data_ptr(), None, None, out.data_ptr(), M, N, Kd, 0, 1.0, 1, 0, 1, stats.data_ptr(), c.data_ptr(), b.data_ptr(), int(W_TILEMAJOR))
    else:
        _dev(x, weight_il160, bias_il160)
        wt = _w_tilemajor(weight_il160) if W_TILEMAJOR else weight_il160
        args = (wt.data_ptr(), _p(bias_il160), None, out.data_ptr(), M, N, Kd, 0, 1.0, 1, 0, 1, None, None, None, int(W_TILEMAJOR))
    _log_call("own_linear", (M, N, Kd, "geglu-blocked", 0), 2.0 * M * N * Kd)
    _lib.check(_lib.load().fmc_linear_bf16_ffblk(x.data_ptr(), *args, _stream()), "fmc_linear_bf16_ffblk")
    return out


def linear_from_blocked(xb: torch.Tensor, weight: torch.Tensor, bias, residual, alpha: float = 1.0, out: Optional[torch.Tensor] = None) -> torch.Tensor:
    _dev(xb, weight, bias, residual, out)
    N, Kd = weight.shape
    M = xb.numel() // Kd
    if out is None:
        out = torch.empty(*xb.shape[:-1], N, dtype=xb.dtype, device=xb.device)
    assert out.is_contiguous() and out.numel() == M * N and out.dtype == xb.dtype
    wt = _w_tilemajor(weight) if W_TILEMAJOR else weight
    _log_call("own_linear", (M, N, Kd, "from-blocked", int(residual is not None)), 2.0 * M * N * Kd)
    _lib.check(_lib.load().fmc_linear_bf16_ffblk(xb.data_ptr(), wt.data_ptr(), _p(bias), _p(residual), out.data_ptr(), M, N, Kd,
                                                 0 if residual is None else N, float(alpha), 0, 1, 0, None, None, None, int(W_TILEMAJOR), _stream()),
               "fmc_linear_bf16_ffblk")
    return out


FF_TAIL = os.environ.get("FMC_FF_TAIL", "1") != "0"


def ff_tail_ok(h: torch.Tensor, w2: torch.Tensor, wp: torch.Tensor, tail_residual: Optional[torch.Tensor]) -> bool:
    C = h.shape[-1]
    M = h.numel() // C
    return (FF_TAIL and not torch.is_grad_enabled() and h.dtype == torch.bfloat16 and h.is_contiguous() and wp.dtype == torch.bfloat16 and w2.dtype == torch.bfloat16
            and wp.ndim == 2 and wp.shape[1] == w2.shape[0] == C and wp.shape[0] % 320 == 0 and C % 64 == 0 and w2.shape[1] % 64 == 0
            and M % 160 == 0 and (M // 160) * (wp.shape[0] // 320) >= _cus(h.device) and M * max(w2.shape[1], C) * 2 < (1 << 31)
            and tail_residual is not None and tail_residual.dtype == h.dtype and tail_residual.is_contiguous()
            and tail_residual.numel() == M * wp.shape[0] and os.environ.get("FMC_G160_PERSIST", "1") != "0")


def fold_ff_tail(w2: torch.Tensor, b2: Optional[torch.Tensor], wp: torch.Tensor, bp: Optional[torch.Tensor]):
    with torch.no_grad():
        wpf = wp.detach().float()
        wc = torch.cat([wpf @ w2.detach().float(), wpf], dim=1).to(torch.bfloat16).contiguous()
        bc = None
        if b2 is not None or bp is not None:
            bc = (wpf @ b2.detach().float()) if b2 is not None else torch.zeros(wp.shape[0], dtype=torch.float32, device=wp.device)
            if bp is not None:
                bc = bc + bp.detach().float()
            bc = bc.to(torch.bfloat16).contiguous()
    return wc, bc


def ff_tail(mid_blocked: torch.Tensor, h: torch.Tensor, w_cat: torch.Tensor, b_cat: Optional[torch.Tensor], tail_residual: torch.Tensor,
            gn_hw: int = 0) -> torch.Tensor:
    _dev(mid_blocked, h, w_cat, b_cat, tail_residual)
    N, Kd = w_cat.shape
    C = h.shape[-1]
    M = h.numel() // C
    assert mid_blocked.numel() == M * (Kd - C) and tail_residual.numel() == M * N
    out = torch.empty_like(tail_residual)
    part = None
    if gn_hw and gn_emit_ok(M, N, Kd, gn_hw, h.dtype):
        part = torch.empty(M // gn_hw, gn_hw // 160, 32, 2, dtype=torch.float32, device=h.device)
        gn_epilogue_calls["emitted"] += 1
    wt = _w_tilemajor(w_cat) if W_TILEMAJOR else w_cat
    _log_call("own_linear", (M, N, Kd, "ff-tail", 1), 2.0 * M * N * Kd)
    _lib.check(_lib.load().fmc_linear_bf16_fftail(mid_blocked.data_ptr(), h.data_ptr(), wt.data_ptr(), _p(b_cat), tail_residual.data_ptr(), out.data_ptr(),
                                                  M, N, Kd, Kd - C, C, N, _p(part), int(gn_hw if part is not None else 0), int(W_TILEMAJOR), _stream()),
               "fmc_linear_bf16_fftail")
    if part is not None:
        out._fmc_gn = (part, N)
    return out


def linear_gn(x: torch.Tensor, weight: torch.Tensor, bias, residual, alpha: float, residual2, hw: int):
    _dev(x, weight, bias, residual)
    N, Kd = weight.shape
    M, ldx = _rows2d(x)
    out = torch.empty(*x.shape[:-1], N, dtype=x.dtype, device=x.device)
    part = torch.empty(M // hw, hw // 160, 32, 2, dtype=torch.float32, device=x.device)
    ldres = 0 if residual is None else _rows2d(residual)[1]
    gn_epilogue_calls["emitted"] += 1
    wt = _w_tilemajor(weight) if W_TILEMAJOR else weight
    _log_call("own_linear", (M, N, Kd, "gn", (residual is not None) + (residual2 is not None)), 2.0 * M * N * Kd)
    _lib.check(_lib.load().fmc_linear_bf16_gn(x.data_ptr(), wt.data_ptr(), _p(bias), _p(residual), out.data_ptr(), M, N, Kd, ldx, ldres, N,
                                              float(alpha), _p(residual2), part.data_ptr(), int(hw), int(W_TILEMAJOR), _stream()), "fmc_linear_bf16_gn")
    out._fmc_gn = (part, N)
    return out


def conv3x3_gn(x_nhwc: torch.Tensor, weight_cl: torch.Tensor, bias, temb, residual_nhwc, temb_div: int, upsample: bool, stride2: bool):
    n, h, w, cin = x_nhwc.shape
    if upsample:
        h, w = 2 * h, 2 * w
    if stride2:
        h, w = h // 2, w // 2
    cout = weight_cl.shape[0]
    out = torch.empty(n, h, w, cout, dtype=x_nhwc.dtype, device=x_nhwc.device)
    part = torch.empty(n, (h * w) // 160, 32, 2, dtype=torch.float32, device=x_nhwc.device)
    gn_epilogue_calls["emitted"] += 1
    wt = _w_tilemajor_conv(weight_cl) if W_TILEMAJOR else weight_cl
    _lib.check(_lib.load().fmc_conv3x3_bf16_gn(x_nhwc.data_ptr(), wt.data_ptr(), _p(bias), _p(temb), _p(residual_nhwc), out.data_ptr(),
                                               n, h, w, cin, cout, 0 if temb is None else temb.stride(0), int(temb_div),
                                               2 if stride2 else int(upsample), part.data_ptr(), int(W_TILEMAJOR), _stream()), "fmc_conv3x3_bf16_gn")
    return out, (part, cout)


CONV_HALO = os.environ.get("FMC_CONV_HALO", "1") != "0"
CONV_HALO_MIN_TILES = int(os.environ.get("FMC_CONV_HALO_MIN_TILES", "200"))
LINEAR4 = os.environ.get("FMC_LINEAR4", "1") != "0"
CONV_HALO4 = os.environ.get("FMC_CONV_HALO4", "1") != "0"
CONV_GN_FUSED = os.environ.get("FMC_CONV_GN_FUSED", "0") == "1"
conv_halo_calls = {"conv": 0, "gn_fused": 0, "stats_pass": 0, "stats_from_producer": 0}


def conv3x3_halo_supported(n: int, h: int, w: int, cin: int, cin1: int, cout: int, upsample: bool) -> bool:
    return bool(_lib.load().fmc_conv3x3_halo_supported(n, h, w, cin, cin1, cout, int(upsample)))


def _w_packed(weight_cl: torch.Tensor, key: str, factor: int, fn: str, *args) -> torch.Tensor:
    def build():
        cout, cin = weight_cl.shape[:2]
        assert weight_cl.is_contiguous(memory_format=torch.channels_last)
        out = torch.empty(cout * factor * cin, dtype=weight_cl.dtype, device=weight_cl.device)
        _lib.check(getattr(_lib.load(), fn)(weight_cl.data_ptr(), out.data_ptr(), cin, cout, *args, _stream()), fn)
        return out
    return derived_on_owner(weight_cl, "_fmc_wtm", key, build)


def _w_halo_packed(weight_cl: torch.Tensor) -> torch.Tensor:
    return _w_packed(weight_cl, "halo", 9, "fmc_conv3x3_halo_pack_weight")


def _gn_tagged(y, want: bool, cout: int):
    if not want:
        return y.permute(0, 3, 1, 2)
    y, part = y
    gn_epilogue_calls["emitted"] += 1
    y = y.permute(0, 3, 1, 2)
    y._fmc_gn = (part, cout)
    return y


def _halo_args(x_nhwc, weight_cl, temb, residual_nhwc, temb_div, upsample, x2_nhwc):
    n, hs, ws, c1 = x_nhwc.shape
    h, w = (2 * hs, 2 * ws) if upsample else (hs, ws)
    cout, cin = weight_cl.shape[:2]
    assert x_nhwc.is_contiguous() and x_nhwc.dtype == torch.bfloat16 and weight_cl.dtype == torch.bfloat16
    if x2_nhwc is not None:
        assert x2_nhwc.is_contiguous() and x2_nhwc.shape[:3] == x_nhwc.shape[:3] and x2_nhwc.dtype == x_nhwc.dtype and c1 + x2_nhwc.shape[3] == cin
    else:
        assert c1 == cin
    assert temb is None or (temb.stride(1) == 1 and temb.shape == (n // temb_div, cout) and n % temb_div == 0)
    assert residual_nhwc is None or (residual_nhwc.is_contiguous() and residual_nhwc.shape == (n, h, w, cout))
    return n, h, w, c1, cin, cout


def groupnorm_coef(partials: torch.Tensor, gamma: torch.Tensor, beta: torch.Tensor, hw: int, C: int, groups: int, eps: float,
                   want_stats: bool = False):
    _dev(partials, gamma, beta)
    N, splits, G, _ = partials.shape
    assert G == groups and partials.dtype == torch.float32 and partials.is_contiguous() and gamma.dtype == torch.float32
    coef = torch.empty(N, C, 2, dtype=torch.float32, device=partials.device)
    stats = torch.empty(N, G, 2, dtype=torch.float32, device=partials.device) if want_stats else None
    _lib.check(_lib.load().fmc_groupnorm_coef(partials.data_ptr(), splits, gamma.data_ptr(), beta.data_ptr(), coef.data_ptr(), _p(stats), N, hw, C,
                                              groups, float(eps), _stream()), "fmc_groupnorm_coef")
    return (coef, stats) if want_stats else coef


def conv3x3_halo4_supported(n: int, h: int, w: int, cin: int, cin1: int, cout: int, upsample: bool, wide: bool = False) -> bool:
    return bool(_lib.load().fmc_conv3x3_halo4_supported(n, h, w, cin, cin1, cout, int(upsample), int(wide)))


def _w_halo4_packed(weight_cl: torch.Tensor, wide: bool = False) -> torch.Tensor:
    return _w_packed(weight_cl, "halo4w" if wide else "halo4", 9, "fmc_conv3x3_halo4_pack_weight", int(wide))


def conv3x3_halo4_split(n: int, h: int, w: int, cin: int, cout: int, cus: int = 256, wide: bool = False) -> int:
    tiles = _lib.load().fmc_conv3x3_halo4_tiles(n, h, w, cout, int(wide))
    if tiles >= (3 * cus) // 4:
        return 1
    nchunk = cin // 64
    best = 1
    for s in range(2, min(nchunk, 16) + 1):
        if nchunk % s == 0 and tiles * s <= cus + cus // 8:
            best = s
    return best


def conv3x3_halo4(x_nhwc: torch.Tensor, weight_cl: torch.Tensor, bias=None, temb=None, residual_nhwc=None, temb_div: int = 1, upsample: bool = False,
                  x2_nhwc: Optional[torch.Tensor] = None, emit_gn: bool = False, split_k: Optional[int] = None, wide: bool = False):
    _dev(x_nhwc, weight_cl, bias, temb, residual_nhwc, x2_nhwc)
    n, h, w, c1, cin, cout = _halo_args(x_nhwc, weight_cl, temb, residual_nhwc, temb_div, upsample, x2_nhwc)
    L = _lib.load()
    wp = _w_halo4_packed(weight_cl, wide)
    out = torch.empty(n, h, w, cout, dtype=x_nhwc.dtype, device=x_nhwc.device)
    if split_k is None:
        split_k = 1 if emit_gn else conv3x3_halo4_split(n, h, w, cin, cout, wide=wide)
    ws, ws_bytes = (None, 0) if split_k <= 1 else _splitk_workspace(x_nhwc.device, split_k, n * h * w, cout)
    part = torch.empty(n, L.fmc_conv3x3_halo4_row_blocks_per_image(h, w), 32, 2, dtype=torch.float32, device=x_nhwc.device) if emit_gn else None
    conv_halo_calls["conv4"] = conv_halo_calls.get("conv4", 0) + 1
    if call_log is not None:
        call_log.append(("conv_halo4", (n, h, w, cin, cout, bool(upsample)), 2.0 * n * h * w * cout * 9 * cin))
    _lib.check(L.fmc_conv3x3_halo4_bf16(x_nhwc.data_ptr(), _p(x2_nhwc), c1, wp.data_ptr(), _p(bias), _p(temb), _p(residual_nhwc), out.data_ptr(),
                                        n, h, w, cin, cout, 0 if temb is None else temb.stride(0), int(temb_div), int(upsample), _p(part), int(split_k),
                                        ws, ws_bytes, int(wide), _stream()), "fmc_conv3x3_halo4_bf16")
    return (out, part) if emit_gn else out


def groupnorm_partials(x: torch.Tensor, groups: int, x2: Optional[torch.Tensor] = None) -> torch.Tensor:
    _dev(x, x2)
    N, S, C1 = x.shape
    C = C1 + (x2.shape[2] if x2 is not None else 0)
    assert x.is_contiguous() and (x2 is None or (x2.is_contiguous() and x2.shape[:2] == x.shape[:2] and x2.dtype == x.dtype))
    L = _lib.load()
    part = torch.empty(N, L.fmc_groupnorm_partial_splits(S, C), groups, 2, dtype=torch.float32, device=x.device)
    conv_halo_calls["stats_pass"] += 1
    _lib.check(L.fmc_groupnorm_partials(x.data_ptr(), _p(x2), C1 if x2 is not None else 0, part.data_ptr(), N, S, C, groups, _dt(x), _stream()),
               "fmc_groupnorm_partials")
    return part


def conv3x3_halo(x_nhwc: torch.Tensor, weight_cl: torch.Tensor, bias=None, temb=None, residual_nhwc=None, temb_div: int = 1, upsample: bool = False,
                 x2_nhwc: Optional[torch.Tensor] = None, gn_coef: Optional[torch.Tensor] = None, gn_act: bool = True, emit_gn: bool = False):
    _dev(x_nhwc, weight_cl, bias, temb, residual_nhwc, x2_nhwc, gn_coef)
    n, h, w, c1, cin, cout = _halo_args(x_nhwc, weight_cl, temb, residual_nhwc, temb_div, upsample, x2_nhwc)
    assert gn_coef is None or (gn_coef.shape == (n, cin, 2) and gn_coef.dtype == torch.float32 and gn_coef.is_contiguous())
    L = _lib.load()
    wp = _w_halo_packed(weight_cl)
    out = torch.empty(n, h, w, cout, dtype=x_nhwc.dtype, device=x_nhwc.device)
    part = torch.empty(n, L.fmc_conv3x3_halo_tiles_per_image(h, w), 32, 2, dtype=torch.float32, device=x_nhwc.device) if emit_gn else None
    conv_halo_calls["conv"] += 1
    conv_halo_calls["gn_fused"] += gn_coef is not None
    if call_log is not None:
        call_log.append(("conv_halo", (n, h, w, cin, cout, bool(upsample)), 2.0 * n * h * w * cout * 9 * cin))
    _lib.check(L.fmc_conv3x3_halo_bf16(x_nhwc.data_ptr(), _p(x2_nhwc), c1, wp.data_ptr(), _p(bias), _p(temb), _p(residual_nhwc), out.data_ptr(),
                                       n, h, w, cin, cout, 0 if temb is None else temb.stride(0), int(temb_div), int(upsample), _p(gn_coef),
                                       int(gn_act), _p(part), _stream()), "fmc_conv3x3_halo_bf16")
    return (out, part) if emit_gn else out


UPS_FOLD = os.environ.get("FMC_UPS_FOLD", "1") != "0"
UPS_FOLD_MIN_WS = int(os.environ.get("FMC_UPS_FOLD_MIN_WS", "8"))
UPS_FOLD_WIDE = os.environ.get("FMC_UPS_FOLD_WIDE", "0") == "1"


def upsample_fold_weights(weight: torch.Tensor) -> torch.Tensor:
    rows = (((0,), (1, 2)), ((0, 1), (2,)))
    cout, cin = weight.shape[:2]
    wf = weight.new_zeros(2, 2, 2, 2, cout, cin)
    for py in range(2):
        for px in range(2):
            for a in range(2):
                for b in range(2):
                    for ky in rows[py][a]:
                        for kx in rows[px][b]:
                            wf[py, px, a, b] += weight[:, :, ky, kx]
    return wf


def conv3x3_upfold_reference(x_nchw: torch.Tensor, wf: torch.Tensor, bias: Optional[torch.Tensor] = None) -> torch.Tensor:
    import torch.nn.functional as F
    n, _, hs, ws = x_nchw.shape
    cout = wf.shape[4]
    xp = F.pad(x_nchw, (1, 1, 1, 1))
    out = x_nchw.new_zeros(n, cout, 2 * hs, 2 * ws)
    for py in range(2):
        for px in range(2):
            k = wf[py, px].permute(2, 3, 0, 1)
            out[:, :, py::2, px::2] = F.conv2d(xp[:, :, py:py + hs + 1, px:px + ws + 1], k)
    return out if bias is None else out + bias[None, :, None, None]


def conv3x3_upfold_arm(n: int, hs: int, ws: int, cin: int, cout: int) -> Optional[str]:
    if not (UPS_FOLD and CONV_HALO) or ws < UPS_FOLD_MIN_WS:
        return None
    L = _lib.load()
    if (L.fmc_conv3x3_halo_fold_supported(n, hs, ws, cin, cout)
            and n * L.fmc_conv3x3_halo_tiles_per_image(hs, ws) * 4 * (cout // 160) >= CONV_HALO_MIN_TILES):
        return "halo"
    if not CONV_HALO4:
        return None
    wide = UPS_FOLD_WIDE and bool(L.fmc_conv3x3_halo4_fold_supported(n, hs, ws, cin, cout, 1))
    if (L.fmc_conv3x3_halo4_fold_supported(n, hs, ws, cin, cout, int(wide))
            and 4 * L.fmc_conv3x3_halo4_tiles(n, hs, ws, cout, int(wide)) >= CONV_HALO_MIN_TILES):
        return "halo4w" if wide else "halo4"
    return None


def _w_upfold_packed(weight_cl: torch.Tensor, tile_channels: int) -> torch.Tensor:
    return _w_packed(weight_cl, "upfold%d" % tile_channels, 16, "fmc_conv3x3_upfold_pack_weight", tile_channels)


def conv3x3_upfold(x_nhwc: torch.Tensor, weight_cl: torch.Tensor, bias=None, emit_gn: bool = False, arm: Optional[str] = None):
    _dev(x_nhwc, weight_cl, bias)
    n, hs, ws, cin = x_nhwc.shape
    cout = weight_cl.shape[0]
    assert x_nhwc.is_contiguous() and x_nhwc.dtype == torch.bfloat16 and weight_cl.dtype == torch.bfloat16 and weight_cl.shape[1] == cin
    assert not (torch.is_grad_enabled() and (x_nhwc.requires_grad or weight_cl.requires_grad)), "conv3x3_upfold: inference only"
    if arm is None:
        arm = conv3x3_upfold_arm(n, hs, ws, cin, cout)
    if arm not in ("halo", "halo4", "halo4w"):
        raise ValueError(f"conv3x3_upfold: no phase-mode launch for n={n} {hs}x{ws} {cin}->{cout} (arm {arm})")
    L = _lib.load()
    out = torch.empty(n, 2 * hs, 2 * ws, cout, dtype=x_nhwc.dtype, device=x_nhwc.device)
    shape, flops = (n, 2 * hs, 2 * ws, cin, cout, True), 2.0 * n * 4 * hs * ws * cout * 9 * cin
    conv_halo_calls["upfold"] = conv_halo_calls.get("upfold", 0) + 1
    if arm == "halo":
        wp = _w_upfold_packed(weight_cl, 160)
        part = torch.empty(n, 4 * L.fmc_conv3x3_halo_tiles_per_image(hs, ws), 32, 2, dtype=torch.float32, device=x_nhwc.device) if emit_gn else None
        conv_halo_calls["conv"] += 1
        if call_log is not None:
            call_log.append(("conv_halo", shape, flops))
        _lib.check(L.fmc_conv3x3_halo_fold_bf16(x_nhwc.data_ptr(), wp.data_ptr(), _p(bias), out.data_ptr(), n, hs, ws, cin, cout, _p(part), _stream()),
                   "fmc_conv3x3_halo_fold_bf16")
    else:
        wide = arm == "halo4w"
        wp = _w_upfold_packed(weight_cl, 160 if wide else 80)
        part = torch.empty(n, 4 * L.fmc_conv3x3_halo4_row_blocks_per_image(hs, ws), 32, 2, dtype=torch.float32, device=x_nhwc.device) if emit_gn else None
        conv_halo_calls["conv4"] = conv_halo_calls.get("conv4", 0) + 1
        if call_log is not None:
            call_log.append(("conv_halo4", shape, flops))
        _lib.check(L.fmc_conv3x3_halo4_fold_bf16(x_nhwc.data_ptr(), wp.data_ptr(), _p(bias), out.data_ptr(), n, hs, ws, cin, cout, _p(part), int(wide),
                                                 _stream()), "fmc_conv3x3_halo4_fold_bf16")
    return (out, part) if emit_gn else out


F32_GEMM = os.environ.get("FMC_F32_GEMM", "1") != "0"
f32_gemm_calls = {"linear": 0, "geglu": 0, "conv3x3": 0}


def split_bf16x3(src: torch.Tensor, role: int, dst: Optional[torch.Tensor] = None, col0: int = 0, K: Optional[int] = None) -> torch.Tensor:
    _dev(src)
    assert src.dtype == torch.float32
    C = src.shape[-1]
    rows, ld = _rows2d(src)
    K = C if K is None else K
    if dst is None:
        dst = torch.empty(rows, 3 * K, dtype=torch.bfloat16, device=src.device)
    assert dst.shape == (rows, 3 * K) and dst.is_contiguous()
    _lib.check(_lib.load().fmc_split_bf16x3(src.data_ptr(), dst.data_ptr(), rows, C, ld, 3 * K, col0, K, role, _stream()),
               "fmc_split_bf16x3")
    return dst


def _split_weight_cached(weight: torch.Tensor, rows: int, C: int) -> torch.Tensor:
    def build():
        w2 = weight.detach()
        w2 = w2.contiguous(memory_format=torch.channels_last).permute(0, 2, 3, 1).reshape(rows, C) if weight.ndim == 4 else w2.reshape(rows, C)
        return split_bf16x3(w2.contiguous(), 1)
    return derived_on_owner(weight, "_fmc_w3", (rows, C), build)


def _f32_arm(key_bf16, tile: int) -> int:
    if tile:
        return tile
    return _f32_arm_of(_choice.get(key_bf16, 0))


def _f32_arm_of(use: int) -> int:
    if ARM_160 <= use < ARM_160 + 5 or ARM_160B <= use < ARM_160B + 5 or use == ARM_256:
        return ARM_160
    if use >= 384:
        use -= 384
    elif use >= 256:
        use -= 256
    elif use >= 128:
        use -= 128
    if 16 <= use < 128:
        use &= 15
    return use if 1 <= use <= 14 else 0


def linear_f32(x: torch.Tensor, weight: torch.Tensor, bias=None, residual=None, alpha: float = 1.0, geglu: bool = False,
               tile: int = 0, split_k: int = 1, x2=None, residual2=None) -> torch.Tensor:
    tile, split_k = _decode_arm(tile, split_k)
    if split_k < 1:
        split_k = 1
    _dev(x, weight, bias, residual, x2)
    N, Kd = weight.shape
    M, _ = _rows2d(x)
    if x2 is None:
        x3 = split_bf16x3(x, 0)
    else:
        k1 = x.shape[-1]
        assert k1 + x2.shape[-1] == Kd and _rows2d(x2)[0] == M
        x3 = torch.empty(M, 3 * Kd, dtype=torch.bfloat16, device=x.device)
        split_bf16x3(x, 0, x3, 0, Kd)
        split_bf16x3(x2, 0, x3, k1, Kd)
    w3 = _split_weight_cached(weight, N, Kd)
    n_out = N // 2 if geglu else N
    out = torch.empty(*x.shape[:-1], n_out, dtype=torch.float32, device=x.device)
    ldres = 0
    if residual is not None:
        assert residual.shape == out.shape and residual.dtype == torch.float32
        _, ldres = _rows2d(residual)
    if residual2 is not None:
        assert residual is not None and residual2.shape == out.shape and _rows2d(residual2)[1] == ldres
    b = None if bias is None else bias.float()
    ws, ws_bytes = _splitk_workspace(x.device, split_k, M, N)
    f32_gemm_calls["geglu" if geglu else "linear"] += 1
    _lib.check(_lib.load().fmc_linear_x3_f32(x3.data_ptr(), w3.data_ptr(), _p(b), _p(residual), out.data_ptr(), M, N, 3 * Kd,
                                             3 * Kd, ldres, n_out, float(alpha), int(geglu), int(tile), int(split_k), ws, ws_bytes,
                                             _p(residual2), _stream()), "fmc_linear_x3_f32")
    return out


def conv3x3_f32(x_nhwc: torch.Tensor, weight: torch.Tensor, bias=None, temb=None, residual_nhwc=None, tile: int = 0,
                split_k: int = 1, temb_div: int = 1, upsample: bool = False, stride2: bool = False) -> torch.Tensor:
    tile, split_k = _decode_arm(tile, split_k)
    if split_k < 1:
        split_k = 1
    _dev(x_nhwc, weight, bias, temb, residual_nhwc)
    n, h, w, cin = x_nhwc.shape
    if upsample:
        h, w = 2 * h, 2 * w
    if stride2:
        assert not upsample and h % 2 == 0 and w % 2 == 0
        h, w = h // 2, w // 2
    cout = weight.shape[0]
    assert x_nhwc.is_contiguous() and x_nhwc.dtype == torch.float32
    assert temb is None or (temb.stride(1) == 1 and temb.shape == (n // temb_div, cout) and temb.dtype == torch.float32)
    assert residual_nhwc is None or (residual_nhwc.is_contiguous() and residual_nhwc.shape == (n, h, w, cout))
    x3 = split_bf16x3(x_nhwc.view(-1, cin), 0)
    w3 = _split_weight_cached(weight, cout * 9, cin)
    out = torch.empty(n, h, w, cout, dtype=torch.float32, device=x_nhwc.device)
    b = None if bias is None else bias.float()
    ws, ws_bytes = _splitk_workspace(x_nhwc.device, split_k, n * h * w, cout)
    f32_gemm_calls["conv3x3"] += 1
    _lib.check(_lib.load().fmc_conv3x3_x3_f32(x3.data_ptr(), w3.data_ptr(), _p(b), _p(temb), _p(residual_nhwc), out.data_ptr(),
                                              n, h, w, 3 * cin, cout, 0 if temb is None else temb.stride(0), int(temb_div),
                                              2 if stride2 else int(upsample), int(tile), int(split_k), ws, ws_bytes, _stream()),
               "fmc_conv3x3_x3_f32")
    return out


_choice = {}
_tune_log = {}
_calls = {}
AUTOTUNE = os.environ.get("FMC_AUTOTUNE", "1") != "0"
DETERMINISTIC = os.environ.get("FMC_DETERMINISTIC", "0") == "1"
_CACHE_ENV = os.environ.get("FMC_AUTOTUNE_CACHE", "")
_cache_state = {"loaded": False, "dirty": False, "meta": None}


def _cache_path():
    if _CACHE_ENV == "0":
        return None
    return _CACHE_ENV or os.path.join(os.path.dirname(_lib.LIB_PATH), "autotune_cache.json")


def _cache_meta():
    if _cache_state["meta"] is None:
        import hashlib
        with open(_lib.LIB_PATH, "rb") as f:
            sha = hashlib.sha256(f.read()).hexdigest()[:16]
        _cache_state["meta"] = {"lib_sha16": sha, "device": torch.cuda.get_device_name() if torch.cuda.is_available() else "cpu",
                                "arms": list(GEMM_TILES), "hipblaslt": vendor_version() if torch.cuda.is_available() else 0}
    return _cache_state["meta"]


DEFAULT_ARM_TABLE = os.path.join(os.path.dirname(os.path.abspath(__file__)), "autotune_default_mi355x.json")
stale_table_entries = [0]
autotune_sources = {"cache": 0, "defaults": 0}


def _load_table_file(path: str, strict_meta: bool) -> int:
    import ast
    import json
    if not path or not os.path.isfile(path):
        return 0
    try:
        with open(path) as f:
            blob = json.load(f)
        meta, mine = blob.get("meta") or {}, _cache_meta()
        if strict_meta and meta != mine:
            return 0
        if not strict_meta:
            arch = torch.cuda.get_device_properties(torch.cuda.current_device()).gcnArchName.split(":")[0]
            if meta.get("arch") != arch:
                return 0
        n = 0
        for k, v in blob["choices"].items():
            key = ast.literal_eval(k)
            if key[0] == "valgo" and meta.get("hipblaslt") != mine["hipblaslt"]:
                continue
            if key not in _choice:
                _choice[key] = int(v["arm"])
                _tune_log[key] = {int(a): ms for a, ms in v.get("ms", {}).items()}
                n += 1
        return n
    except Exception:
        return 0


def load_autotune_table(path: Optional[str] = None) -> int:
    _cache_state["loaded"] = True
    n = _load_table_file(path or _cache_path(), True)
    autotune_sources["cache"] += n
    if os.environ.get("FMC_AUTOTUNE_DEFAULTS", "1") != "0" and torch.cuda.is_available():
        d = _load_table_file(DEFAULT_ARM_TABLE, False)
        autotune_sources["defaults"] += d
        n += d
    return n


def save_autotune_table(path: Optional[str] = None) -> Optional[str]:
    import json
    path = path or _cache_path()
    if not path or not _choice:
        return None
    blob = {"meta": _cache_meta(),
            "choices": {repr(k): {"arm": v, "ms": _tune_log.get(k, {})} for k, v in _choice.items()}}
    tmp = f"{path}.{os.getpid()}.tmp"
    try:
        with open(tmp, "w") as f:
            json.dump(blob, f)
        os.replace(tmp, path)
    except OSError:
        return None
    _cache_state["dirty"] = False
    return path


def _save_at_exit():
    if _cache_state["dirty"] and os.environ.get("RANK", "0") == "0":
        save_autotune_table()


atexit.register(_save_at_exit)
GEMM_TILES = (1, 2, 3, 4, 5, 6, 7, 11,
              13,
              15,
              ARM_160B if W_TILEMAJOR else ARM_160,
              128 + 2, 128 + 3,
              128 + 13,
              256 + 13,
              384 + 13)
if os.environ.get("FMC_GEMM_ARMS"):
    GEMM_TILES = tuple(int(a) for a in os.environ["FMC_GEMM_ARMS"].split(","))


def autotune_report():
    return [(k, _choice[k], _tune_log.get(k, {}), _calls.get(k, 0)) for k in _choice]


_tune_stream = None
def _graph_ms(body, reps):
    g = torch.cuda.CUDAGraph()
    with torch.cuda.graph(g, stream=_tune_stream):
        for _ in range(reps):
            body()
    g.replay()
    _tune_stream.synchronize()
    ms = float("inf")
    for _ in range(3):
        e0, e1 = torch.cuda.Event(enable_timing=True), torch.cuda.Event(enable_timing=True)
        e0.record()
        g.replay()
        e1.record()
        _tune_stream.synchronize()
        ms = min(ms, e0.elapsed_time(e1) / reps)
    del g
    return ms


def _time_ms(fn, reps=8):
    global _tune_stream
    if _tune_stream is None:
        _tune_stream = torch.cuda.Stream()
    cur = torch.cuda.current_stream()
    _tune_stream.wait_stream(cur)
    with torch.cuda.stream(_tune_stream):
        fn()
        _tune_stream.synchronize()
        ms = _graph_ms(fn, reps)
    cur.wait_stream(_tune_stream)
    return ms


NO_VENDOR = os.environ.get("FMC_NO_VENDOR", "0") == "1"
dispatch_calls = {k: {"own": 0, "vendor": 0, "ineligible": 0} for k in ("linear", "geglu", "conv3x3")}
call_log = None


def _log_call(family: str, shape: tuple, flops: float) -> None:
    if call_log is not None:
        call_log.append((family, tuple(shape), float(flops)))


def _pick(key, hip_fn, lib_fn, static_hip: bool, extra_arms=(), k320: bool = False, own_only: bool = False) -> int:
    if not _cache_state["loaded"]:
        load_autotune_table()
    no_lib = (DETERMINISTIC and key[0] == "conv") or own_only or NO_VENDOR
    if no_lib:
        key = key + ("det",)
    use = _choice.get(key)
    _calls[key] = _calls.get(key, 0) + 1
    n320 = (key[5] if key[0] == "conv" else key[2]) % 320 == 0
    cands = tuple(t for t in GEMM_TILES + tuple(extra_arms)
                  if (t != 15 or k320)
                  and (not (ARM_160 <= t < ARM_160 + 5 or ARM_160B <= t < ARM_160B + 5 or t == ARM_256) or n320))
    if use is not None and not (use in cands or (use == 0 and not no_lib) or (use == -1 and key not in _tune_log)):
        _choice.pop(key, None)
        _tune_log.pop(key, None)
        stale_table_entries[0] += 1
        use = None
    if use is None:
        if not AUTOTUNE or torch.cuda.is_current_stream_capturing():
            return 0 if not (static_hip or no_lib) else -1
        times = ([] if no_lib else [(_time_ms(lib_fn), 0)]) + [(_time_ms(lambda t=t: hip_fn(t)), t) for t in cands]
        use = min(times)[1]
        _choice[key] = use
        _tune_log[key] = {arm: round(ms, 4) for ms, arm in times}
        _cache_state["dirty"] = True
    return use


def linear(x: torch.Tensor, weight: torch.Tensor, bias: Optional[torch.Tensor] = None,
           residual: Optional[torch.Tensor] = None, alpha: float = 1.0, x2: Optional[torch.Tensor] = None,
           residual2: Optional[torch.Tensor] = None, gn_hw: int = 0, ln: Optional["LnSpec"] = None,
           lazy_residual: bool = False) -> torch.Tensor:
    import torch.nn.functional as F
    pend = getattr(x, "_fmc_pending_ln", None)
    if pend is not None:
        if (x2 is None and residual is None and residual2 is None and alpha == 1.0 and not gn_hw and ln is None and weight.is_contiguous()
                and lnc_ok(x, weight)):
            dispatch_calls["linear"]["own"] += 1
            return linear_lnc(x, weight, bias, pend)
        x = resolve_pending_ln(x)

    def lib():
        xin = x if x2 is None else torch.cat([x, x2], dim=-1)
        if alpha == 1.0 and vendor_linear_ok(xin, weight, bias, residual):
            y = vendor_linear(xin, weight, bias, residual)
            return y if residual2 is None else y + residual2
        y = F.linear(xin, weight, bias)
        _log_call("vendor", (xin.numel() // xin.shape[-1], weight.shape[0], weight.shape[1], bias is not None, False), 2.0 * xin.numel() * weight.shape[0])
        if residual is not None:
            y = torch.add(residual, y, alpha=alpha)
            return y if residual2 is None else y + residual2
        return y if alpha == 1.0 else y * alpha

    N, Kd = weight.shape
    if (F32_GEMM and x.is_cuda and x.dtype == torch.float32 and weight.dtype == torch.float32 and Kd % 64 == 0 and N % 8 == 0
            and x.shape[-1] % 8 == 0 and (x.is_contiguous() or x.ndim == 2) and (x2 is None or x2.is_contiguous())
            and (residual is None or residual.dtype == torch.float32)):
        M = x.numel() // x.shape[-1]
        key = ("lin", M, N, Kd, bias is not None, (residual is not None) + (residual2 is not None), 0 if x2 is None else x.shape[-1])
        return linear_f32(x, weight, bias, residual, alpha, tile=_f32_arm(key, 0), x2=x2, residual2=residual2)
    ok = x.is_cuda and x.dtype == torch.bfloat16 and weight.dtype == torch.bfloat16 and Kd % 64 == 0 and N % 8 == 0
    if x2 is None:
        ok = ok and linear_supported(x, weight)
    else:
        ok = ok and x.shape[-1] % 64 == 0 and x2.dtype == x.dtype and x2.is_contiguous()
    if not ok or (x.ndim > 2 and not x.is_contiguous()):
        dispatch_calls["linear"]["ineligible"] += 1
        return lib()
    M = x.numel() // x.shape[-1]
    if ln is not None and x2 is None and not gn_hw and ln_emit_ok(x, weight, residual, residual2, ln):
        dispatch_calls["linear"]["own"] += 1
        return linear_ln(x, weight, bias, residual, alpha, residual2, ln)
    if (gn_hw and x2 is None and x.is_contiguous() and gn_emit_ok(M, N, Kd, gn_hw, x.dtype)
            and (residual is None or (residual.is_contiguous() and residual.dtype == x.dtype))
            and (residual2 is None or residual2.is_contiguous())):
        dispatch_calls["linear"]["own"] += 1
        return linear_gn(x, weight, bias, residual, alpha, residual2, gn_hw)
    key = ("lin", M, N, Kd, bias is not None, (residual is not None) + (residual2 is not None),
           0 if x2 is None else x.shape[-1])
    hip = lambda tile: (linear4_bf16(x, weight, bias, residual, alpha, residual2) if tile == ARM_G4
                        else linear_bf16(x, weight, bias, residual, alpha, tile=tile, x2=x2, residual2=residual2))
    small = (ARM_SMALLM, ARM_SMALLM + 2) if (M <= 2560 and x2 is None and residual2 is None) else ()
    t160 = ((M + 159) // 160) * ((N + 159) // 160)
    if (LINEAR4 and x2 is None and weight.is_contiguous() and 48 <= t160 <= 640 and Kd >= 320
            and _lib.load().fmc_linear4_supported(M, N, Kd, _rows2d(x)[1])
            and (residual is None or _rows2d(residual)[1] % 8 == 0)
            and (residual2 is None or (residual is not None and _rows2d(residual2)[1] == _rows2d(residual)[1]))):
        small = small + (ARM_G4,)
    use = _pick(key, hip, lib, Kd <= 640 and N <= 1024 and M >= 16384, split_arms(M, N, Kd) + small,
                k320=(Kd == 320 and N % 320 == 0 and M % 64 == 0 and x2 is None and residual2 is None))
    if (use == 0 and lazy_residual and LAZY_RESIDUAL and residual is not None and residual2 is None and alpha == 1.0 and x2 is None
            and N in (320, 640, 1280) and residual.is_contiguous() and not torch.is_grad_enabled()
            and not vendor_linear_ok(x, weight, bias, residual)):
        dispatch_calls["linear"]["vendor"] += 1
        y = F.linear(x, weight, bias)
        y._fmc_pending_add = residual
        return y
    dispatch_calls["linear"]["vendor" if use == 0 else "own"] += 1
    return lib() if use == 0 else hip(max(use, 0))


def geglu_linear(x: torch.Tensor, weight: torch.Tensor, bias, weight_il: torch.Tensor, bias_il, weight_il160=None,
                 bias_il160=None) -> torch.Tensor:
    import torch.nn.functional as F
    pend = getattr(x, "_fmc_pending_ln", None)
    if pend is not None:
        if weight_il160 is not None and weight_il160.is_contiguous() and lnc_ok(x, weight_il160):
            return linear_lnc(x, weight_il160, bias_il160, pend, geglu=True)
        x = resolve_pending_ln(x)
    lib = lambda: geglu(F.linear(x, weight, bias))
    if (F32_GEMM and x.is_cuda and x.dtype == torch.float32 and weight_il.dtype == torch.float32 and weight_il.shape[0] % 64 == 0
            and weight_il.shape[1] % 64 == 0 and x.is_contiguous()):
        N, Kd = weight.shape
        arm = _f32_arm(("geglu", x.numel() // Kd, N, Kd), 0)
        if arm in (ARM_160, ARM_160B) and weight_il160 is not None:
            return linear_f32(x, weight_il160, bias_il160, geglu=True, tile=ARM_160)
        return linear_f32(x, weight_il, bias_il, geglu=True, tile=0 if arm in (ARM_160, ARM_160B) else arm)
    if not linear_supported(x, weight_il) or weight_il.shape[0] % 64 or (x.ndim > 2 and not x.is_contiguous()):
        dispatch_calls["geglu"]["ineligible"] += 1
        return lib()
    N, Kd = weight.shape
    M = x.numel() // Kd
    has160 = weight_il160 is not None and N % 320 == 0

    def hip(tile):
        if tile in (ARM_160, ARM_256, ARM_160B):
            return linear_bf16(x, weight_il160, bias_il160, geglu=True, tile=tile) if has160 else linear_bf16(x, weight_il, bias_il, geglu=True, tile=13)
        return linear_bf16(x, weight_il, bias_il, geglu=True, tile=tile)
    use = _pick(("geglu", M, N, Kd), hip, lib, M >= 65536)
    dispatch_calls["geglu"]["vendor" if use == 0 else "own"] += 1
    return lib() if use == 0 else hip(max(use, 0))


def conv3x3(x_nchw: torch.Tensor, weight_cl: torch.Tensor, bias, temb=None, residual_nchw=None, stride=(1, 1),
            padding=(1, 1), temb_div: int = 1, upsample: bool = False, emit_gn: bool = False, own_only: bool = False) -> torch.Tensor:
    import torch.nn.functional as F

    def lib():
        xin = F.interpolate(x_nchw, scale_factor=2.0, mode="nearest") if upsample else x_nchw
        y = F.conv2d(xin, weight_cl, bias, stride, padding)
        if temb is not None:
            y = y + (temb if temb_div == 1 else temb.repeat_interleave(temb_div, dim=0))[:, :, None, None]
        if residual_nchw is not None:
            y = y + residual_nchw
        return y

    if (F32_GEMM and x_nchw.is_cuda and x_nchw.dtype == torch.float32 and weight_cl.dtype == torch.float32
            and tuple(weight_cl.shape[2:]) == (3, 3) and tuple(padding) == (1, 1) and weight_cl.shape[1] % 64 == 0
            and weight_cl.shape[0] % 8 == 0 and (tuple(stride) == (1, 1) or (tuple(stride) == (2, 2) and not upsample
                                                                           and x_nchw.shape[-1] % 2 == 0 and x_nchw.shape[-2] % 2 == 0))):
        n, cin, h, w = x_nchw.shape
        x = x_nchw.permute(0, 2, 3, 1)
        r = None if residual_nchw is None else residual_nchw.permute(0, 2, 3, 1)
        if x.is_contiguous() and (r is None or r.is_contiguous()) and (temb is None or temb.stride(1) == 1):
            s2 = tuple(stride) == (2, 2)
            ho, wo = (2 * h, 2 * w) if upsample else ((h // 2, w // 2) if s2 else (h, w))
            key = ("conv", n, ho, wo, cin, weight_cl.shape[0], temb is not None, r is not None, upsample, s2)
            return conv3x3_f32(x, weight_cl, bias, temb, r, tile=_f32_arm(key, 0), temb_div=temb_div, upsample=upsample,
                               stride2=s2).permute(0, 3, 1, 2)
    if not conv3x3_supported(x_nchw, weight_cl, stride, padding):
        dispatch_calls["conv3x3"]["ineligible"] += 1
        return lib()
    n, cin, h, w = x_nchw.shape
    cout = weight_cl.shape[0]
    x = x_nchw.permute(0, 2, 3, 1)
    r = None if residual_nchw is None else residual_nchw.permute(0, 2, 3, 1)
    if not x.is_contiguous() or (r is not None and not r.is_contiguous()):
        dispatch_calls["conv3x3"]["ineligible"] += 1
        return lib()
    if upsample:
        h, w = 2 * h, 2 * w
    stride2 = tuple(stride) == (2, 2)
    if stride2:
        h, w = h // 2, w // 2
    if upsample and temb is None and r is None and not torch.is_grad_enabled() and x.dtype == torch.bfloat16 and weight_cl.dtype == torch.bfloat16:
        arm = conv3x3_upfold_arm(n, h // 2, w // 2, cin, cout)
        if arm is not None:
            bn = 80 if arm == "halo4" else 160
            want = bool(emit_gn and GN_EPILOGUE and cout % 64 == 0 and bn % (cout // 32) == 0 and (arm == "halo" or h * w >= GN_MIN_HW))
            dispatch_calls["conv3x3"]["own"] += 1
            y = conv3x3_upfold(x, weight_cl, bias, emit_gn=want, arm=arm)
            return _gn_tagged(y, want, cout)
    if (CONV_HALO and not stride2 and (temb is None or temb.stride(1) == 1) and conv3x3_halo_supported(n, h, w, cin, cin, cout, upsample)
            and n * _lib.load().fmc_conv3x3_halo_tiles_per_image(h, w) * (cout // 160) >= CONV_HALO_MIN_TILES):
        want = bool(emit_gn and GN_EPILOGUE and cout % 64 == 0 and 160 % (cout // 32) == 0 and not torch.is_grad_enabled())
        dispatch_calls["conv3x3"]["own"] += 1
        y = conv3x3_halo(x, weight_cl, bias, temb, r, temb_div, upsample, emit_gn=want)
        return _gn_tagged(y, want, cout)
    if (CONV_HALO and CONV_HALO4 and not stride2 and w % 8 == 0 and (temb is None or temb.stride(1) == 1)
            and conv3x3_halo4_supported(n, h, w, cin, cin, cout, upsample)
            and _lib.load().fmc_conv3x3_halo4_tiles(n, h, w, cout, 0) * conv3x3_halo4_split(n, h, w, cin, cout) >= CONV_HALO_MIN_TILES):
        dispatch_calls["conv3x3"]["own"] += 1
        want = bool(emit_gn and GN_EPILOGUE and h * w >= GN_MIN_HW and cout % 64 == 0 and 80 % (cout // 32) == 0 and not torch.is_grad_enabled()
                    and conv3x3_halo4_split(n, h, w, cin, cout) == 1)
        y = conv3x3_halo4(x, weight_cl, bias, temb, r, temb_div, upsample, emit_gn=want)
        return _gn_tagged(y, want, cout)
    if emit_gn and gn_emit_ok(n * h * w, cout, 9 * cin, h * w, x.dtype):
        dispatch_calls["conv3x3"]["own"] += 1
        y, tag = conv3x3_gn(x, weight_cl, bias, temb, r, temb_div, upsample, stride2)
        y = y.permute(0, 3, 1, 2)
        y._fmc_gn = tag
        return y
    key = ("conv", n, h, w, cin, cout, temb is not None, r is not None, upsample, stride2)
    hip = lambda tile: conv3x3_bf16(x, weight_cl, bias, temb, r, tile=tile, temb_div=temb_div,
                                    upsample=upsample, stride2=stride2).permute(0, 3, 1, 2)
    tiles = ((n * h * w + 127) // 128) * ((cout + 127) // 128)
    use = _pick(key, hip, lib, tiles >= 256, split_arms(n * h * w, cout, 9 * cin), own_only=own_only)
    dispatch_calls["conv3x3"]["vendor" if use == 0 else "own"] += 1
    return lib() if use == 0 else hip(max(use, 0))


def _flipped_filter(weight_cl: torch.Tensor) -> torch.Tensor:
    return derived_on_owner(weight_cl, "_fmc_flipped", None,
                            lambda: weight_cl.detach().flip(2, 3).permute(1, 0, 2, 3).contiguous(memory_format=torch.channels_last))


class _Conv3x3Frozen(torch.autograd.Function):
    @staticmethod
    def forward(ctx, x, weight_cl, bias, temb, residual, temb_div):
        ctx.save_for_backward(weight_cl)
        ctx.has_res = residual is not None and residual.requires_grad
        with torch.no_grad():
            return conv3x3(x, weight_cl, bias, temb, residual, (1, 1), (1, 1), temb_div)

    @staticmethod
    def backward(ctx, dy):
        (weight_cl,) = ctx.saved_tensors
        dy = dy.contiguous(memory_format=torch.channels_last)
        dx = None
        if ctx.needs_input_grad[0]:
            with torch.no_grad():
                dx = conv3x3(dy, _flipped_filter(weight_cl), None)
        return dx, None, None, None, (dy if ctx.has_res else None), None


def conv3x3_frozen(x, weight_cl, bias, temb=None, residual=None, temb_div: int = 1):
    return _Conv3x3Frozen.apply(x, weight_cl, bias, temb, residual, temb_div)


RESAMPLE_BWD = os.environ.get("FMC_RESAMPLE_BWD", "1") != "0"
resample_bwd_calls = {"down": 0, "up": 0, "edge": 0}


def conv3x3_down_bwd_supported(n: int, h: int, w: int, cin: int, cout: int) -> bool:
    return bool(_lib.load().fmc_conv3x3_down_bwd_supported(n, h, w, cin, cout))


def conv3x3_up_bwd_supported(n: int, hs: int, ws: int, cin: int, cout: int) -> bool:
    return bool(_lib.load().fmc_conv3x3_up_bwd_supported(n, hs, ws, cin, cout))


def _w_resample_bwd_packed(weight_cl: torch.Tensor, up: bool) -> torch.Tensor:
    return _w_packed(weight_cl, "up_bwd" if up else "down_bwd", 16 if up else 9,
                     "fmc_conv3x3_up_bwd_pack_weight" if up else "fmc_conv3x3_down_bwd_pack_weight")


def conv3x3_down_bwd(dy_nhwc: torch.Tensor, w_packed: torch.Tensor, cin: int, out: Optional[torch.Tensor] = None, tile: int = 0) -> torch.Tensor:
    _dev(dy_nhwc, w_packed, out)
    n, ho, wo, cout = dy_nhwc.shape
    assert dy_nhwc.is_contiguous() and dy_nhwc.dtype == torch.bfloat16 and w_packed.dtype == torch.bfloat16 and w_packed.numel() == 9 * cin * cout
    if out is None:
        out = torch.empty(n, 2 * ho, 2 * wo, cin, dtype=dy_nhwc.dtype, device=dy_nhwc.device)
    assert out.is_contiguous() and out.shape == (n, 2 * ho, 2 * wo, cin) and out.dtype == dy_nhwc.dtype
    resample_bwd_calls["down"] += 1
    if call_log is not None:
        call_log.append(("conv_down_bwd", (n, 2 * ho, 2 * wo, cin, cout), 2.0 * n * ho * wo * 9 * cin * cout))
    _lib.check(_lib.load().fmc_conv3x3_down_bwd_bf16(dy_nhwc.data_ptr(), w_packed.data_ptr(), out.data_ptr(), n, 2 * ho, 2 * wo, cin, cout, tile,
                                                     _stream()),
               "fmc_conv3x3_down_bwd_bf16")
    return out


def conv3x3_up_bwd(dy_nhwc: torch.Tensor, w_packed: torch.Tensor, cin: int, out: Optional[torch.Tensor] = None, tile: int = 0) -> torch.Tensor:
    _dev(dy_nhwc, w_packed, out)
    n, hd, wd, cout = dy_nhwc.shape
    assert hd % 2 == 0 and wd % 2 == 0
    hs, ws = hd // 2, wd // 2
    assert dy_nhwc.is_contiguous() and dy_nhwc.dtype == torch.bfloat16 and w_packed.dtype == torch.bfloat16 and w_packed.numel() == 16 * cin * cout
    if out is None:
        out = torch.empty(n, hs, ws, cin, dtype=dy_nhwc.dtype, device=dy_nhwc.device)
    assert out.is_contiguous() and out.shape == (n, hs, ws, cin) and out.dtype == dy_nhwc.dtype
    resample_bwd_calls["up"] += 1
    if call_log is not None:
        call_log.append(("conv_up_bwd", (n, hs, ws, cin, cout), 2.0 * n * hs * ws * 16 * cin * cout))
    _lib.check(_lib.load().fmc_conv3x3_up_bwd_bf16(dy_nhwc.data_ptr(), w_packed.data_ptr(), out.data_ptr(), n, hs, ws, cin, cout, tile, _stream()),
               "fmc_conv3x3_up_bwd_bf16")
    return out


def _nhwc(t: torch.Tensor) -> torch.Tensor:
    return t.permute(0, 2, 3, 1).contiguous()


class _Conv3x3DownFrozen(torch.autograd.Function):
    @staticmethod
    def forward(ctx, x, weight_cl, bias):
        ctx.save_for_backward(weight_cl)
        with torch.no_grad():
            return conv3x3(x, weight_cl, bias, None, None, (2, 2), (1, 1))

    @staticmethod
    def backward(ctx, dy):
        (weight_cl,) = ctx.saved_tensors
        if not ctx.needs_input_grad[0]:
            return None, None, None
        with torch.no_grad():
            dx = conv3x3_down_bwd(_nhwc(dy), _w_resample_bwd_packed(weight_cl, False), weight_cl.shape[1])
        return dx.permute(0, 3, 1, 2), None, None


class _Conv3x3UpFrozen(torch.autograd.Function):
    @staticmethod
    def forward(ctx, x, weight_cl, bias):
        ctx.save_for_backward(weight_cl)
        with torch.no_grad():
            return conv3x3(x, weight_cl, bias, None, None, (1, 1), (1, 1), 1, True)

    @staticmethod
    def backward(ctx, dy):
        (weight_cl,) = ctx.saved_tensors
        if not ctx.needs_input_grad[0]:
            return None, None, None
        with torch.no_grad():
            dx = conv3x3_up_bwd(_nhwc(dy), _w_resample_bwd_packed(weight_cl, True), weight_cl.shape[1])
        return dx.permute(0, 3, 1, 2), None, None


def conv3x3_down_frozen(x, weight_cl, bias):
    return _Conv3x3DownFrozen.apply(x, weight_cl, bias)


def conv3x3_up_frozen(x, weight_cl, bias):
    return _Conv3x3UpFrozen.apply(x, weight_cl, bias)


def _edge_flipped_filter(weight: torch.Tensor) -> torch.Tensor:
    def build():
        cout, cin = weight.shape[:2]
        wf = torch.zeros(cin, (cout + 63) // 64 * 64, 3, 3, dtype=weight.dtype, device=weight.device)
        wf[:, :cout] = weight.detach().flip(2, 3).permute(1, 0, 2, 3)
        return wf.contiguous(memory_format=torch.channels_last)
    return derived_on_owner(weight, "_fmc_flipped", "edge", build)


class _Conv3x3EdgeFrozen(torch.autograd.Function):
    @staticmethod
    def forward(ctx, x, weight, fwd):
        ctx.save_for_backward(weight)
        with torch.no_grad():
            return fwd(x)

    @staticmethod
    def backward(ctx, dy):
        (weight,) = ctx.saved_tensors
        if not ctx.needs_input_grad[0]:
            return None, None, None
        with torch.no_grad():
            wf = _edge_flipped_filter(weight)
            n, cout, h, w = dy.shape
            dyp = torch.zeros(n, h, w, wf.shape[1], dtype=dy.dtype, device=dy.device)
            dyp[..., :cout] = dy.permute(0, 2, 3, 1)
            resample_bwd_calls["edge"] += 1
            dx = conv3x3(dyp.permute(0, 3, 1, 2), wf, None, own_only=True)
        return dx, None, None


def conv3x3_edge_frozen(x, weight, fwd):
    return _Conv3x3EdgeFrozen.apply(x, weight, fwd)


def _transposed_weight(weight: torch.Tensor) -> torch.Tensor:
    return derived_on_owner(weight, "_fmc_wt", None, lambda: weight.detach().t().contiguous())


def linear_backward_data(dy: torch.Tensor, weight: torch.Tensor, alpha: float = 1.0) -> torch.Tensor:
    if dy.is_cuda and dy.dtype == torch.bfloat16 and weight.dtype == torch.bfloat16 and weight.shape[0] % 64 == 0 \
            and weight.shape[1] % 8 == 0:
        with torch.no_grad():
            return linear(dy if dy.is_contiguous() else dy.contiguous(), _transposed_weight(weight), None, None, alpha)
    dx = torch.matmul(dy, weight)
    return dx if alpha == 1.0 else dx * alpha


class _LinearFrozen(torch.autograd.Function):
    @staticmethod
    def forward(ctx, x, weight, bias, residual, alpha):
        ctx.save_for_backward(weight)
        ctx.alpha = alpha
        ctx.has_res = residual is not None and residual.requires_grad
        with torch.no_grad():
            return linear(x, weight, bias, residual, alpha)

    @staticmethod
    def backward(ctx, dy):
        (weight,) = ctx.saved_tensors
        dx = linear_backward_data(dy, weight, ctx.alpha) if ctx.needs_input_grad[0] else None
        return dx, None, None, (dy if ctx.has_res else None), None


def linear_frozen(x, weight, bias=None, residual=None, alpha: float = 1.0):
    return _LinearFrozen.apply(x, weight, bias, residual, alpha)


def column_sum(x: torch.Tensor, alpha: float = 1.0, out: Optional[torch.Tensor] = None, accumulate: bool = False) -> torch.Tensor:
    _dev(x, out)
    M, ld = _rows2d(x)
    N = x.shape[-1]
    if out is None:
        out, accumulate = torch.empty(N, dtype=torch.float32, device=x.device), False
    assert out.dtype == torch.float32 and out.is_contiguous() and out.numel() == N
    lib = _lib.load()
    ws = _workspace(x.device, lib.fmc_column_sum_workspace_bytes(M, N))
    _lib.check(lib.fmc_column_sum(x.data_ptr(), out.data_ptr(), M, N, ld, float(alpha), int(accumulate), ws.data_ptr(), _dt(x), _stream()),
               "fmc_column_sum")
    return out


class _LinearTrainable(torch.autograd.Function):

    @staticmethod
    def forward(ctx, x, weight, bias, residual, w_run, b_run):
        with torch.no_grad():
            y = linear(x, w_run, b_run, residual)
        ctx.save_for_backward(x, w_run)
        ctx.has_res = residual is not None and residual.requires_grad
        ctx.dtypes = (weight.dtype, None if bias is None else bias.dtype)
        return y

    @staticmethod
    def backward(ctx, dy):
        x, w_run = ctx.saved_tensors
        dy = dy if dy.dtype == x.dtype else dy.to(x.dtype)
        dy = dy if dy.is_contiguous() else dy.contiguous()
        N, Kd = w_run.shape
        dy2 = dy.view(-1, N)
        x2 = x if (x.ndim == 2 and not x.is_contiguous()) else x.reshape(-1, Kd)
        dx = dw = db = None
        with torch.no_grad():
            if ctx.needs_input_grad[0]:
# ... 335 lines not shown
```

synfmc_amd/models/layers.py:

```python
from __future__ import annotations

import os

import math
from typing import Optional

import torch
import torch.nn.functional as F
from torch import nn

from .. import hip_ops as K
from ..derived import derived, drop


def to_tokens(x: torch.Tensor) -> torch.Tensor:
    n, c, h, w = x.shape
    t = x.permute(0, 2, 3, 1)
    if not t.is_contiguous():
        t = t.contiguous()
    return K.carry_gn(x, t.view(n, h * w, c))


def from_tokens(t: torch.Tensor, h: int, w: int) -> torch.Tensor:
    n, _, c = t.shape
    return K.carry_gn(t, t.view(n, h, w, c).permute(0, 3, 1, 2))


def f32_param(mod: nn.Module, name: str) -> torch.Tensor:
    p = getattr(mod, name)
    if p.dtype == torch.float32:
        return p
    if torch.is_grad_enabled() and p.requires_grad:
        return p.float()
    return derived(mod, "_f32_cache", [p], lambda: p.detach().float(), tag=name)


def bf16_param(mod: nn.Module, name: str, rounded_f32: bool = False) -> torch.Tensor:
    p = getattr(mod, name)
    if p is None or p.dtype != torch.float32:
        return p if (p is None or not rounded_f32) else f32_param(mod, name)
    cache = mod.__dict__.setdefault("_bf16_shadow", {})
    hit = cache.get(name)
    if hit is None or hit[1].shape != p.shape or hit[1].device != p.device:
        hit = [None, torch.empty(p.shape, dtype=torch.bfloat16, device=p.device), torch.empty(p.shape, dtype=torch.float32, device=p.device)]
        cache[name] = hit
    key = (p.data_ptr(), p._version)
    if hit[0] != key:
        with torch.no_grad():
            hit[1].copy_(p.detach())
            hit[2].copy_(hit[1])
        hit[0] = key
    return hit[2] if rounded_f32 else hit[1]


def bf16_shadow_owners(model: nn.Module, params) -> dict:
    want = {id(p) for p in params}
    return {id(p): (mod, name) for mod in model.modules() for name, p in mod._parameters.items() if p is not None and id(p) in want}


def bf16_shadow_tensors(mod: nn.Module, name: str):
    p = getattr(mod, name)
    hit = mod.__dict__.get("_bf16_shadow", {}).get(name)
    if hit is None or p is None or p.dtype != torch.float32 or hit[1].shape != p.shape or hit[1].device != p.device:
        return None
    return hit[1], hit[2]


def bf16_shadow_mark_fresh(mod: nn.Module, name: str) -> None:
    p = getattr(mod, name)
    hit = mod.__dict__.get("_bf16_shadow", {}).get(name)
    if hit is not None:
        hit[0] = (p.data_ptr(), p._version)


class GroupNorm(nn.GroupNorm):

    def forward(self, x: torch.Tensor, act: bool = False, x2: Optional[torch.Tensor] = None) -> torch.Tensor:
        n, c, h, w = x.shape
        y = K.groupnorm_silu(to_tokens(x), f32_param(self, "weight"), f32_param(self, "bias"), self.num_groups,
                             self.eps, act, None if x2 is None else to_tokens(x2), gn_tag=getattr(x, "_fmc_gn", None))
        return from_tokens(y, h, w)

    def skip(self, x: torch.Tensor, act: bool = False):
        if NORM_SKIP and torch.is_grad_enabled() and x.requires_grad and x.is_cuda and x.dtype in (torch.bfloat16, torch.float32):
            n, c, h, w = x.shape
            xs, y = K.groupnorm_silu_skip(to_tokens(x), f32_param(self, "weight"), f32_param(self, "bias"), self.num_groups, self.eps, act)
            return from_tokens(xs, h, w), from_tokens(y, h, w)
        return x, self(x, act=act)


NORM_SKIP = os.environ.get("FMC_NORM_SKIP", "1") != "0"


class LayerNorm(nn.LayerNorm):
    def skip(self, x: torch.Tensor, pe: Optional[torch.Tensor] = None, pe_inner: int = 1, pe_frames: int = 1, defer: bool = False):
        if NORM_SKIP and torch.is_grad_enabled() and x.requires_grad and x.is_cuda and x.dtype in (torch.bfloat16, torch.float32):
            return K.layernorm_skip(x if x.is_contiguous() else x.contiguous(), f32_param(self, "weight"), f32_param(self, "bias"), self.eps,
                                    pe, pe_inner, pe_frames)
        r = getattr(x, "_fmc_pending_add", None)
        if r is not None:
            if x.is_contiguous() and x.shape[-1] in (320, 640, 1280) and x.dtype == r.dtype:
                return K.layernorm_add(x, r, f32_param(self, "weight"), f32_param(self, "bias"), self.eps, pe, pe_inner, pe_frames)
            x = K.resolve_pending_add(x)
        return x, self(x, pe, pe_inner, pe_frames, defer=defer)

    def ln_spec(self, pe: Optional[torch.Tensor] = None, pe_inner: int = 1, pe_frames: int = 1, stats_only: bool = False):
        return K.LnSpec(f32_param(self, "weight"), f32_param(self, "bias"), self.eps, pe, pe_inner, pe_frames, self._ln_key(pe, pe_inner, pe_frames),
                        stats_only)

    def _ln_key(self, pe, pe_inner, pe_frames):
        return (id(self), self.weight._version, self.bias._version, None if pe is None else (pe.data_ptr(), pe._version), pe_inner, pe_frames)

    def forward(self, x: torch.Tensor, pe: Optional[torch.Tensor] = None, pe_inner: int = 1,
                pe_frames: int = 1, defer: bool = False) -> torch.Tensor:
        x = K.resolve_pending_add(x)
        key = self._ln_key(pe, pe_inner, pe_frames)
        if defer and pe is None:
            stats = K.take_ln_stats(x, key)
            if stats is not None:
                return K.pending_ln(x, stats, f32_param(self, "weight"), f32_param(self, "bias"), self.eps)
        done = K.take_ln(x, key)
        if done is not None:
            return done
        if not x.is_contiguous():
            x = x.contiguous()
        return K.layernorm(x, f32_param(self, "weight"), f32_param(self, "bias"), self.eps, pe, pe_inner, pe_frames)


PADDED_EDGE_CONVS = os.environ.get("FMC_PADDED_EDGE_CONVS", "1") != "0"


class Conv2d(nn.Conv2d):

    frozen_resample_bwd = True

    def forward(self, x: torch.Tensor, scale: float = 1.0, temb: Optional[torch.Tensor] = None,
                residual: Optional[torch.Tensor] = None, temb_div: int = 1, upsample: bool = False,
                x2: Optional[torch.Tensor] = None, emit_gn: bool = False) -> torch.Tensor:
        if self.kernel_size == (1, 1) and self.stride == (1, 1) and self.padding == (0, 0):
            n, c, h, w = x.shape
            assert temb is None
            y = linear_op(to_tokens(x), self.weight.view(self.out_channels, self.in_channels), self.bias,
                          None if residual is None else to_tokens(residual), 1.0, None if x2 is None else to_tokens(x2),
                          gn_hw=h * w if emit_gn else 0)
            return from_tokens(y, h, w)
        assert x2 is None, "two-source input: 1x1 convs only"
        if not x.is_contiguous(memory_format=torch.channels_last):
            x = x.contiguous(memory_format=torch.channels_last)
        needs_grad = torch.is_grad_enabled() and (x.requires_grad or self.weight.requires_grad or
                                                  (residual is not None and residual.requires_grad))
        if (needs_grad and not upsample and self.kernel_size == (3, 3) and self.stride == (1, 1) and self.padding == (1, 1)
                and self.dilation == (1, 1) and self.groups == 1 and x.is_cuda and x.dtype == torch.bfloat16
                and self.weight.dtype == torch.bfloat16 and not self.weight.requires_grad
                and (self.bias is None or not self.bias.requires_grad) and (temb is None or not temb.requires_grad)
                and self.in_channels % 64 == 0 and self.out_channels % 64 == 0):
            return K.conv3x3_frozen(x, self._weight_cl(), self.bias, temb, residual, temb_div)
        if (needs_grad and not upsample and temb is None and residual is None and self.kernel_size == (3, 3)
                and self.stride == (1, 1) and self.padding == (1, 1) and self.dilation == (1, 1) and self.groups == 1
                and x.is_cuda and x.dtype == torch.bfloat16 and self.in_channels % 64 == 0 and self.out_channels % 64 == 0
                and self.weight.requires_grad):
            return K.conv3x3_trainable(x, self.weight, self.bias)
        if (needs_grad and K.RESAMPLE_BWD and self.frozen_resample_bwd and temb is None and residual is None and self.kernel_size == (3, 3) and self.padding == (1, 1)
                and self.dilation == (1, 1) and self.groups == 1 and x.is_cuda and x.dtype == torch.bfloat16 and self.weight.dtype == torch.bfloat16
                and not self.weight.requires_grad and (self.bias is None or not self.bias.requires_grad) and self.in_channels % 64 == 0):
            n, c, h, w = x.shape
            if (self.stride == (2, 2) and not upsample and self.out_channels % 64 == 0
                    and K.conv3x3_down_bwd_supported(n, h, w, self.in_channels, self.out_channels)):
                return K.conv3x3_down_frozen(x, self._weight_cl(), self.bias)
            if (self.stride == (1, 1) and upsample and self.out_channels % 64 == 0
                    and K.conv3x3_up_bwd_supported(n, h, w, self.in_channels, self.out_channels)):
                return K.conv3x3_up_frozen(x, self._weight_cl(), self.bias)
            if self.stride == (1, 1) and not upsample and self.out_channels % 64 and PADDED_EDGE_CONVS:
                fwd = self.padded_conv3x3 if self.out_channels % 8 else (lambda t: K.conv3x3(t, self._weight_cl(), self.bias))
                return K.conv3x3_edge_frozen(x, self.weight, fwd)
        if (self.kernel_size == (3, 3) and self.dilation == (1, 1) and self.groups == 1 and x.is_cuda and not needs_grad
                and self.stride == (1, 1) and self.padding == (1, 1) and x.dtype == torch.bfloat16 and self.weight.dtype == torch.bfloat16
                and (self.in_channels % 64 or self.out_channels % 8) and temb is None and residual is None and not upsample and PADDED_EDGE_CONVS):
            return self.padded_conv3x3(x)
        if self.kernel_size == (3, 3) and self.dilation == (1, 1) and self.groups == 1 and x.is_cuda and not needs_grad:
            return K.conv3x3(x, self._weight_cl(), self.bias, temb, residual, self.stride, self.padding, temb_div,
                             upsample, emit_gn=emit_gn)
        if upsample:
            x = F.interpolate(x, scale_factor=2.0, mode="nearest")
        y = F.conv2d(x, self._weight_cl(), self.bias, self.stride, self.padding, self.dilation, self.groups)
        if temb is not None:
            y = y + (temb if temb_div == 1 else temb.repeat_interleave(temb_div, dim=0))[:, :, None, None]
        if residual is not None:
            y = y + residual
        return y

    def padded_conv3x3(self, x: torch.Tensor) -> torch.Tensor:
        cout, cin = self.weight.shape[:2]
        cin_p, cout_p = (cin + 63) // 64 * 64, (cout + 7) // 8 * 8

        def build():
            w = torch.zeros(cout_p, cin_p, 3, 3, dtype=self.weight.dtype, device=self.weight.device)
            w[:cout, :cin] = self.weight
            b = torch.zeros(cout_p, dtype=self.weight.dtype, device=self.weight.device)
            if self.bias is not None:
                b[:cout] = self.bias
            return w.contiguous(memory_format=torch.channels_last), b
        wp, bp = derived(self, "_padded", [self.weight, self.bias], build)
        if cin_p != cin:
            xp = torch.zeros(x.shape[0], cin_p, x.shape[2], x.shape[3], dtype=x.dtype, device=x.device).contiguous(memory_format=torch.channels_last)
            xp[:, :cin] = x
            x = xp
        y = K.conv3x3(x.contiguous(memory_format=torch.channels_last), wp, bp, own_only=True)
        return y[:, :cout]

    def _weight_cl(self) -> torch.Tensor:
        w = self.weight
        if w.is_contiguous(memory_format=torch.channels_last) or (torch.is_grad_enabled() and w.requires_grad):
            return w
        return derived(self, "_w_cl", [w], lambda: w.detach().contiguous(memory_format=torch.channels_last))


def linear_op(x, weight, bias=None, residual=None, alpha: float = 1.0, x2=None, gn_hw: int = 0, ln=None, lazy_residual: bool = False):
    x = K.resolve_pending_add(x)
    if residual is not None:
        residual = K.resolve_pending_add(residual)
    if getattr(x, "_fmc_pending_ln", None) is not None and not (x.dtype == torch.bfloat16 and weight.dtype == torch.bfloat16 and not torch.is_grad_enabled()):
        x = K.resolve_pending_ln(x)
    if x.is_cuda and x.dtype == torch.bfloat16 and weight.dtype == torch.bfloat16:
        grad = torch.is_grad_enabled()
        if not (grad and (x.requires_grad or weight.requires_grad or (residual is not None and residual.requires_grad)
                          or (x2 is not None and x2.requires_grad))):
            return K.linear(x, weight, bias, residual, alpha, x2, gn_hw=gn_hw, ln=ln, lazy_residual=lazy_residual)
        if x2 is not None:
            x, x2 = torch.cat([x, x2], dim=-1), None
        if not weight.requires_grad and (bias is None or not bias.requires_grad):
            return K.linear_frozen(x, weight, bias, residual, alpha)
    elif (x.is_cuda and x.dtype == torch.float32 and weight.dtype == torch.float32 and K.F32_GEMM and not
          (torch.is_grad_enabled() and (x.requires_grad or weight.requires_grad or (residual is not None and residual.requires_grad)
                                        or (x2 is not None and x2.requires_grad)))):
        return K.linear(x, weight, bias, residual, alpha, x2)
    if x2 is not None:
        x = torch.cat([x, x2], dim=-1)
    y = F.linear(x, weight, bias)
    if alpha != 1.0:
        y = y * alpha
    return y if residual is None else y + residual


class Linear(nn.Linear):
    def forward(self, x: torch.Tensor, scale: float = 1.0, residual: Optional[torch.Tensor] = None) -> torch.Tensor:
        return linear_op(x, self.weight, self.bias, residual)


class Timesteps(nn.Module):
    def __init__(self, num_channels: int, flip_sin_to_cos: bool, downscale_freq_shift: float):
        super().__init__()
        self.num_channels, self.flip_sin_to_cos = num_channels, flip_sin_to_cos
        self.downscale_freq_shift = downscale_freq_shift

    def forward(self, timesteps: torch.Tensor) -> torch.Tensor:
        half = self.num_channels // 2
        k = torch.arange(half, dtype=torch.float32, device=timesteps.device)
        freqs = torch.exp(-math.log(10000.0) * k / (half - self.downscale_freq_shift))
        ang = timesteps[:, None].float() * freqs[None, :]
        emb = torch.cat([torch.cos(ang), torch.sin(ang)] if self.flip_sin_to_cos
                        else [torch.sin(ang), torch.cos(ang)], dim=-1)
        return F.pad(emb, (0, 1)) if self.num_channels % 2 else emb


class TimestepEmbedding(nn.Module):
    def __init__(self, in_channels: int, time_embed_dim: int):
        super().__init__()
        self.linear_1 = nn.Linear(in_channels, time_embed_dim)
        self.act = nn.SiLU()
        self.linear_2 = nn.Linear(time_embed_dim, time_embed_dim)

    def forward(self, sample):
        return self.linear_2(self.act(self.linear_1(sample)))


class LoRALinearLayer(nn.Module):

    def __init__(self, in_features, out_features, rank=4, network_alpha=None, device=None, dtype=None):
        super().__init__()
        self.down = nn.Linear(in_features, rank, bias=False, device=device, dtype=dtype)
        self.up = nn.Linear(rank, out_features, bias=False, device=device, dtype=dtype)
        self.network_alpha, self.rank = network_alpha, rank
        self.in_features, self.out_features = in_features, out_features
        nn.init.normal_(self.down.weight, std=1 / rank)
        nn.init.zeros_(self.up.weight)

    def delta_weight(self) -> torch.Tensor:
        w = self.up.weight.float() @ self.down.weight.float()
        return w * (self.network_alpha / self.rank) if self.network_alpha is not None else w

    def forward(self, hidden_states):
        y = self.up(self.down(hidden_states))
        return y * (self.network_alpha / self.rank) if self.network_alpha is not None else y


class ResnetBlock2D(nn.Module):
    def __init__(self, *, in_channels, out_channels=None, conv_shortcut=False, dropout=0.0, temb_channels=512,
                 groups=32, groups_out=None, pre_norm=True, eps=1e-6, non_linearity="swish",
                 time_embedding_norm="default", output_scale_factor=1.0, use_in_shortcut=None):
        super().__init__()
        if time_embedding_norm != "default" or non_linearity not in ("swish", "silu"):
            raise NotImplementedError("FMC builds default / SiLU resnets only")
        out_channels = in_channels if out_channels is None else out_channels
        self.in_channels, self.out_channels = in_channels, out_channels
        self.output_scale_factor = output_scale_factor
        self.norm1 = GroupNorm(num_groups=groups, num_channels=in_channels, eps=eps, affine=True)
        self.conv1 = Conv2d(in_channels, out_channels, kernel_size=3, stride=1, padding=1)
        self.time_emb_proj = Linear(temb_channels, out_channels) if temb_channels is not None else None
        self.norm2 = GroupNorm(num_groups=groups if groups_out is None else groups_out, num_channels=out_channels,
                               eps=eps, affine=True)
        self.dropout = nn.Dropout(dropout)
        self.conv2 = Conv2d(out_channels, out_channels, kernel_size=3, stride=1, padding=1)
        self.nonlinearity = nn.SiLU()
        self.use_in_shortcut = in_channels != out_channels if use_in_shortcut is None else use_in_shortcut
        self.conv_shortcut = Conv2d(in_channels, out_channels, kernel_size=1, stride=1, padding=0) \
            if self.use_in_shortcut else None

    _t_pre = None

    def forward(self, input_tensor, temb, scale: float = 1.0, skip: Optional[torch.Tensor] = None):
        t, div = None, 1
        if self._t_pre is not None:
            t, div = self._t_pre
            if t.shape[0] * div > input_tensor.shape[0]:
                t = t[: input_tensor.shape[0] // div]
        elif self.time_emb_proj is not None and temb is not None:
            t = self.time_emb_proj(F.silu(temb))
        if skip is not None and (self.conv_shortcut is None or (torch.is_grad_enabled() and (input_tensor.requires_grad or skip.requires_grad))):
            input_tensor, skip = torch.cat([input_tensor, skip], dim=1), None
        if skip is None and torch.is_grad_enabled() and input_tensor.requires_grad:
            input_tensor, n1 = self.norm1.skip(input_tensor, act=True)
            h = self.conv1(n1, temb=t, temb_div=div)
            if self.conv_shortcut is not None:
                input_tensor = self.conv_shortcut(input_tensor)
            out = self.conv2(self.norm2(h, act=True), residual=input_tensor)
            return out if self.output_scale_factor == 1.0 else out / self.output_scale_factor
        if K.CONV_GN_FUSED and self._gn_fused_ok(input_tensor, skip, t):
            return self._forward_gn_fused(input_tensor, skip, t, div)
        h = self.conv1(self.norm1(input_tensor, act=True, x2=skip), temb=t, temb_div=div, emit_gn=True)
        if self.conv_shortcut is not None:
            input_tensor = self.conv_shortcut(input_tensor, x2=skip)
        out = self.conv2(self.norm2(h, act=True), residual=input_tensor, emit_gn=True)
        return out if self.output_scale_factor == 1.0 else out / self.output_scale_factor


    def _gn_fused_ok(self, x, skip, t) -> bool:
        n, c, h, w = x.shape
        cin = c + (skip.shape[1] if skip is not None else 0)
        if not (K.CONV_HALO and x.is_cuda and x.dtype == torch.bfloat16 and self.conv1.weight.dtype == torch.bfloat16 and not torch.is_grad_enabled()
                and self.output_scale_factor == 1.0 and c % 64 == 0 and cin == self.in_channels
                and self.out_channels % 64 == 0 and 160 % (self.out_channels // 32) == 0
                and self.norm1.num_groups == 32 and self.norm2.num_groups == 32 and (t is None or t.stride(1) == 1)):
            return False
        return (K.conv3x3_halo_supported(n, h, w, cin, c, self.out_channels, False)
                and K.conv3x3_halo_supported(n, h, w, self.out_channels, self.out_channels, self.out_channels, False))

    def _forward_gn_fused(self, x, skip, t, div):
        n, c, h, w = x.shape
        xt = to_tokens(x)
        st = None if skip is None else to_tokens(skip)
        tag = getattr(xt, "_fmc_gn", None)
        if (tag is not None and st is None and tag[1] == c and tag[0].shape[0] == n and tag[0].shape[2] == 32):
            part1 = tag[0]
            K.conv_halo_calls["stats_from_producer"] += 1
        else:
            part1 = K.groupnorm_partials(xt, 32, st)
        coef1 = K.groupnorm_coef(part1, f32_param(self.norm1, "weight"), f32_param(self.norm1, "bias"), h * w, self.in_channels, 32, self.norm1.eps)
        x_nhwc = xt.view(n, h, w, c)
        s_nhwc = None if st is None else st.view(n, h, w, st.shape[2])
        hid, part2 = K.conv3x3_halo(x_nhwc, self.conv1._weight_cl(), self.conv1.bias, t, None, div, False, s_nhwc, coef1, True, emit_gn=True)
        coef2 = K.groupnorm_coef(part2, f32_param(self.norm2, "weight"), f32_param(self.norm2, "bias"), h * w, self.out_channels, 32, self.norm2.eps)
        res = x if self.conv_shortcut is None else self.conv_shortcut(x, x2=skip)
        out, part3 = K.conv3x3_halo(hid, self.conv2._weight_cl(), self.conv2.bias, None, to_tokens(res).view(n, h, w, self.out_channels), 1, False,
                                    None, coef2, True, emit_gn=True)
        out = out.permute(0, 3, 1, 2)
        out._fmc_gn = (part3, self.out_channels)
        return out


class Downsample2D(nn.Module):
    def __init__(self, channels, use_conv=False, out_channels=None, padding=1, name="conv"):
        super().__init__()
        assert use_conv, "FMC only builds conv downsamplers"
        self.channels, self.out_channels = channels, out_channels or channels
        self.use_conv, self.padding, self.name = use_conv, padding, name
        conv = Conv2d(self.channels, self.out_channels, 3, stride=2, padding=padding)
        if name == "conv":
            self.Conv2d_0 = conv
        self.conv = conv

    def forward(self, hidden_states, scale: float = 1.0):
        assert hidden_states.shape[1] == self.channels
        if self.padding == 0:
            hidden_states = F.pad(hidden_states, (0, 1, 0, 1), mode="constant", value=0)
        return self.conv(hidden_states)


class Upsample2D(nn.Module):
    def __init__(self, channels, use_conv=False, use_conv_transpose=False, out_channels=None, name="conv"):
        super().__init__()
        assert use_conv and not use_conv_transpose and name == "conv"
        self.channels, self.out_channels = channels, out_channels or channels
        self.use_conv, self.name = use_conv, name
        self.conv = Conv2d(self.channels, self.out_channels, 3, padding=1)

    def forward(self, hidden_states, output_size=None, scale: float = 1.0):
        assert hidden_states.shape[1] == self.channels
        if not hidden_states.is_contiguous(memory_format=torch.channels_last):
            hidden_states = hidden_states.contiguous(memory_format=torch.channels_last)
        if output_size is None or tuple(output_size) == (2 * hidden_states.shape[-2], 2 * hidden_states.shape[-1]):
            return self.conv(hidden_states, upsample=True)
        else:
            hidden_states = F.interpolate(hidden_states, size=output_size, mode="nearest")
        return self.conv(hidden_states)


TEXT_KV_ONCE = os.environ.get("FMC_TEXT_KV_ONCE", "1") != "0"
text_kv_calls = {"computed": 0, "hit": 0}


class Attention(nn.Module):

    def __init__(self, query_dim, cross_attention_dim=None, heads=8, dim_head=64, dropout=0.0, bias=False,
                 upcast_attention=False, upcast_softmax=False, cross_attention_norm=None,
                 cross_attention_norm_num_groups=32, added_kv_proj_dim=None, norm_num_groups=None,
                 spatial_norm_dim=None, out_bias=True, scale_qk=True, only_cross_attention=False, eps=1e-5,
                 rescale_output_factor=1.0, residual_connection=False, _from_deprecated_attn_block=False,
                 processor=None):
        super().__init__()
        assert cross_attention_norm is None and added_kv_proj_dim is None and norm_num_groups is None
        assert spatial_norm_dim is None and not only_cross_attention
        self.inner_dim = dim_head * heads
        self.query_dim = query_dim
        self.is_cross = cross_attention_dim is not None
        self.cross_attention_dim = cross_attention_dim if cross_attention_dim is not None else query_dim
        self.upcast_attention, self.upcast_softmax = upcast_attention, upcast_softmax
        self.rescale_output_factor, self.residual_connection = rescale_output_factor, residual_connection
        self.scale = dim_head ** -0.5 if scale_qk else 1.0
        self.heads = heads
        self.sliceable_head_dim = heads
        self.group_norm = self.spatial_norm = self.norm_cross = None
        self.to_q = Linear(query_dim, self.inner_dim, bias=bias)
        self.to_k = Linear(self.cross_attention_dim, self.inner_dim, bias=bias)
        self.to_v = Linear(self.cross_attention_dim, self.inner_dim, bias=bias)
        self.to_out = nn.ModuleList([Linear(self.inner_dim, query_dim, bias=out_bias), nn.Dropout(dropout)])
        from .attention_processor import AttnProcessor
        self.set_processor(processor if processor is not None else AttnProcessor())

    def set_processor(self, processor, _remove_lora: bool = False):
        if hasattr(self, "processor") and isinstance(self.processor, nn.Module) \
                and not isinstance(processor, nn.Module):
            self._modules.pop("processor")
        self.processor = processor
        drop(self, "_fused", "_fused_tb", "_fused_xb", "_text_kv")

    def set_use_memory_efficient_attention_xformers(self, *a, **k):
        pass

    def set_attention_slice(self, slice_size):
        pass

    def prepare_attention_mask(self, attention_mask, target_length, batch_size, out_dim=3):
        if attention_mask is not None:
            raise NotImplementedError("attention masks are never passed on the FMC path")
        return None

    def forward(self, hidden_states, encoder_hidden_states=None, attention_mask=None, **cross_attention_kwargs):
        return self.processor(self, hidden_states, encoder_hidden_states=encoder_hidden_states,
                              attention_mask=attention_mask, **cross_attention_kwargs)

    def text_kv(self, text: torch.Tensor, w_kv: torch.Tensor):
        def compute():
            kv = linear_op(text, w_kv)
            C = w_kv.shape[0] // 2
            pack = (kv.is_cuda and kv.dtype == torch.bfloat16 and kv.ndim == 3 and C in (320, 640) and kv.shape[1] <= 80 and self.heads == 8
                    and kv.is_contiguous())
            return kv, (K.xattn_pack_kv(kv) if pack else None)
        if not TEXT_KV_ONCE or torch.is_grad_enabled() or not text.is_cuda:
            return linear_op(text, w_kv), None
        key = (text.data_ptr(), text._version, tuple(text.shape), text.dtype, w_kv.data_ptr(), w_kv._version)
        hit = self.__dict__.get("_text_kv")
        if hit is not None and hit[0] == key:
            text_kv_calls["hit"] += 1
            return hit[1], hit[2]
        kv, frag = compute()
        text_kv_calls["computed"] += 1
        if not torch.cuda.is_current_stream_capturing():
            self.__dict__["_text_kv"] = (key, kv, frag, text, w_kv)
        return kv, frag

    def refresh_text_kv(self, entry=None):
        entry = entry if entry is not None else self.__dict__.get("_text_kv")
        if entry is None:
            return None
        _, kv, frag, text, w_kv = entry
        with torch.no_grad():
            kv.copy_(linear_op(text, w_kv))
            if frag is not None:
                frag.copy_(K.xattn_pack_kv(kv))
        key = (text.data_ptr(), text._version, tuple(text.shape), text.dtype, w_kv.data_ptr(), w_kv._version)
        entry = (key, kv, frag, text, w_kv)
        self.__dict__["_text_kv"] = entry
        return entry

    def fused_weights(self, lora=None, lora_scale: float = 1.0):
        srcs = [self.to_q.weight, self.to_k.weight, self.to_v.weight, self.to_out[0].weight]
        if torch.is_grad_enabled() and any(p.requires_grad for p in srcs):
            assert lora is None, "a LoRA on trainable base weights is not a configuration the reference uses"
            if self.is_cross:
                return self.to_q.weight, torch.cat([self.to_k.weight, self.to_v.weight], dim=0), self.to_out[0].weight
            return torch.cat([self.to_q.weight, self.to_k.weight, self.to_v.weight], dim=0), None, self.to_out[0].weight
        if lora is not None:
            for n in ("to_q_lora", "to_k_lora", "to_v_lora", "to_out_lora"):
                srcs += [getattr(lora, n).down.weight, getattr(lora, n).up.weight]

        def build():
            def w(lin, name):
                if lora is None:
                    return lin.weight
                return (lin.weight.float() + lora_scale * getattr(lora, name).delta_weight()).to(lin.weight.dtype)
            wq, wk, wv = w(self.to_q, "to_q_lora"), w(self.to_k, "to_k_lora"), w(self.to_v, "to_v_lora")
            wo = w(self.to_out[0], "to_out_lora")
            if self.is_cross:
                return wq.contiguous(), torch.cat([wk, wv], dim=0).contiguous(), wo.contiguous()
            return torch.cat([wq, wk, wv], dim=0).contiguous(), None, wo.contiguous()
        return derived(self, "_fused", srcs, build, extra=(lora_scale,))


def interleave_geglu(weight: torch.Tensor, bias: Optional[torch.Tensor], block: int = 32):
    two_cff, k = weight.shape
    cff = two_cff // 2
    assert cff % block == 0
    w = weight.view(2, cff // block, block, k).permute(1, 0, 2, 3).reshape(two_cff, k).contiguous()
    b = None if bias is None else bias.view(2, cff // block, block).permute(1, 0, 2).reshape(two_cff).contiguous()
    return w, b


class GEGLU(nn.Module):
    def __init__(self, dim_in, dim_out):
        super().__init__()
        self.proj = Linear(dim_in, dim_out * 2)

    def interleaved(self):
        w = self.proj.weight

        def build():
            b = None if self.proj.bias is None else self.proj.bias.detach()
            il160 = interleave_geglu(w.detach(), b, 8) if (w.shape[0] // 2) % 160 == 0 else (None, None)
            return interleave_geglu(w.detach(), b) + il160
        return derived(self, "_il", [w], build)

    def forward(self, hidden_states, scale: float = 1.0):
        w = self.proj.weight
        if hidden_states.is_cuda and (hidden_states.dtype == torch.bfloat16 or (hidden_states.dtype == torch.float32 and K.F32_GEMM)) \
                and hidden_states.dtype == w.dtype and w.shape[0] % 256 == 0 \
                and not (torch.is_grad_enabled() and (w.requires_grad or hidden_states.requires_grad)):
            il = self.interleaved()
            return K.geglu_linear(hidden_states, w, self.proj.bias, il[0], il[1], il[2], il[3])
        return K.geglu(self.proj(K.resolve_pending_ln(hidden_states)))


class FeedForward(nn.Module):
    def __init__(self, dim, dim_out=None, mult=4, dropout=0.0, activation_fn="geglu", final_dropout=False):
        super().__init__()
        if activation_fn != "geglu":
            raise NotImplementedError("FMC only builds geglu feed-forwards")
        inner = int(dim * mult)
        self.net = nn.ModuleList([GEGLU(dim, inner), nn.Dropout(dropout),
                                  Linear(inner, dim if dim_out is None else dim_out)])

    def _tail_weights(self, wp, bp):
        out = self.net[2]
        return derived(self, "_tail_fold", [out.weight, out.bias, wp, bp], lambda: K.fold_ff_tail(out.weight, out.bias, wp, bp))

    def forward_ln(self, h, norm, residual, tail=None):
        proj, out = self.net[0], self.net[2]
        w = proj.proj.weight
        if not K.geglu_ln_direct_ok(h, w) or getattr(h, "_fmc_pending_add", None) is not None or getattr(h, "_fmc_ln", None) is not None \
                or getattr(h, "_fmc_pending_ln", None) is not None:
            return None
        M = h.numel() // h.shape[-1]
        pipe = K.geglu_ln_pipe_ok(h, w) and (h.shape[-1] == 320 or K.GEGLU_PIPE_640)
        var = K.geglu_pipe_variant(M, h.shape[-1]) if pipe else -1
        frag = derived(self, "_geglu_frag", [w], lambda: K.pack_geglu_frag(w, 16 if var == 1 else 32) if pipe else K.pack_geglu_frag80(w), extra=(var,))
        blocked = K.geglu_direct_blocked_ok(h, out.weight, residual)
        if pipe:
            mid = K.geglu_ln_pipe(h, f32_param(norm, "weight"), f32_param(norm, "bias"), norm.eps, frag, proj.proj.bias, w.shape[0] // 2, blocked=blocked,
                                  variant=var)
        else:
            mid = K.geglu_ln_direct(h, f32_param(norm, "weight"), f32_param(norm, "bias"), norm.eps, frag, proj.proj.bias, w.shape[0] // 2, blocked=blocked)
        if blocked and tail is not None and residual is h and K.ff_tail_ok(h, out.weight, tail[0], tail[2]):
            wc, bc = self._tail_weights(tail[0], tail[1])
            y = K.ff_tail(mid, h, wc, bc, tail[2], tail[3])
            y._fmc_tail = True
            return y
        if blocked:
            return K.linear_from_blocked(mid, out.weight, out.bias, residual)
        return out(mid, residual=residual)

    def forward(self, hidden_states, scale: float = 1.0, residual: Optional[torch.Tensor] = None):
        proj, out = self.net[0], self.net[2]
        il = proj.interleaved() if (hidden_states.is_cuda and hidden_states.dtype == torch.bfloat16 and not torch.is_grad_enabled()) else None
        if il is not None and K.ff_blocked_ok(hidden_states, il[2], out.weight, residual):
            mid = K.geglu_linear_blocked(hidden_states, il[2], il[3])
            return K.linear_from_blocked(mid, out.weight, out.bias, residual)
        return out(proj(hidden_states), residual=residual)


class BasicTransformerBlock(nn.Module):
    def __init__(self, dim, num_attention_heads, attention_head_dim, dropout=0.0, cross_attention_dim=None,
                 activation_fn="geglu", attention_bias=False, only_cross_attention=False,
                 double_self_attention=False, upcast_attention=False, norm_elementwise_affine=True,
                 norm_type="layer_norm", norm_eps=1e-5, final_dropout=False):
        super().__init__()
        assert norm_type == "layer_norm" and not only_cross_attention and not double_self_attention
        self.norm1 = LayerNorm(dim, elementwise_affine=norm_elementwise_affine, eps=norm_eps)
        self.attn1 = Attention(query_dim=dim, heads=num_attention_heads, dim_head=attention_head_dim, dropout=dropout,
                               bias=attention_bias, upcast_attention=upcast_attention)
        if cross_attention_dim is not None:
            self.norm2 = LayerNorm(dim, elementwise_affine=norm_elementwise_affine, eps=norm_eps)
            self.attn2 = Attention(query_dim=dim, cross_attention_dim=cross_attention_dim, heads=num_attention_heads,
                                   dim_head=attention_head_dim, dropout=dropout, bias=attention_bias,
                                   upcast_attention=upcast_attention)
        else:
            self.norm2 = self.attn2 = None
        self.norm3 = LayerNorm(dim, elementwise_affine=norm_elementwise_affine, eps=norm_eps)
        self.ff = FeedForward(dim, dropout=dropout, activation_fn=activation_fn, final_dropout=final_dropout)

    def _attn2_weights(self, kw):
        from .attention_processor import LoRAAttnProcessor, _require_frozen, resolve_lora_scale
        attn, proc = self.attn2, self.attn2.processor
        lora, lora_scale = None, 1.0
        if isinstance(proc, LoRAAttnProcessor):
            _require_frozen(proc)
            lora = proc
            lora_scale = resolve_lora_scale(proc, kw["scale"]) if "scale" in kw else resolve_lora_scale(proc)
        return attn.fused_weights(lora, lora_scale)

    def prepare_text(self, text: torch.Tensor, cross_attention_kwargs=None) -> bool:
        from .attention_processor import AttnProcessor, LoRAAttnProcessor
        if self.attn2 is None or type(self.attn2.processor) not in (AttnProcessor, LoRAAttnProcessor) or torch.is_grad_enabled():
            return False
        kw = dict(cross_attention_kwargs) if cross_attention_kwargs is not None else {}
        _, w_kv, _ = self._attn2_weights(kw)
        self.attn2.text_kv(text, w_kv)
        return True
# ... 132 lines not shown
```

Before: 40.23 steps/s.

## Fold ResNet 1x1 shortcut conv into conv2 halo kernel reduction

Adds a shortcut mode to the halo 3x3 conv kernel that appends the 1x1 shortcut conv's input channels as extra K-chunks in the same MFMA reduction. The combined weight is packed once, and the shortcut bias is passed through the temb slot. This removes the separate shortcut conv launch and the write and reread of its output as a residual. The cost is a longer reduction with extra loads and LDS staging, and the path only applies to ResNet blocks that have a channel-changing shortcut and are not on the GN-fused path.

```diff
diff --git a/include/fmc_hip.h b/include/fmc_hip.h
--- a/include/fmc_hip.h
+++ b/include/fmc_hip.h
@@ -140,6 +140,13 @@
 int fmc_conv3x3_halo_bf16(const void* x, const void* x2, int Cin1, const void* w_packed, const void* bias, const void* temb, const void* residual,
                           void* out, int n_img, int H, int W, int Cin, int Cout, int64_t temb_row_stride, int temb_img_div, int upsample2x,
                           const float* gn_coef, int gn_act, float* gn_partials, void* stream);
+int fmc_conv3x3_halo_sc_supported(int n_img, int H, int W, int Cin, int Cout, int Cin_sc, int Cin_sc1);
+int64_t fmc_conv3x3_halo_sc_packed_bytes(int Cin, int Cout, int Cin_sc);
+int64_t fmc_conv3x3_halo_sc_pack_source(int64_t chunk, int Cin, int Cin_sc, int tile_channels, int* from_shortcut);
+int fmc_conv3x3_halo_sc_pack_weight(const void* w, const void* w_sc, void* dst, int Cin, int Cout, int Cin_sc, int tile_channels, void* stream);
+int fmc_conv3x3_halo_sc_bf16(const void* x, const void* w_packed, const void* bias, const void* temb, void* out, const void* xs, const void* xs2,
+                             int Cin_sc1, int Cin_sc, int n_img, int H, int W, int Cin, int Cout, int64_t temb_row_stride, int temb_img_div,
+                             float* gn_partials, void* stream);
 int fmc_conv3x3_halo4_supported(int n_img, int H, int W, int Cin, int Cin1, int Cout, int upsample2x, int wide);
 int fmc_conv3x3_halo4_pack_weight(const void* w, void* dst, int Cin, int Cout, int wide, void* stream);
 int fmc_conv3x3_halo4_row_blocks_per_image(int H, int W);
diff --git a/synfmc_amd/_lib.py b/synfmc_amd/_lib.py
--- a/synfmc_amd/_lib.py
+++ b/synfmc_amd/_lib.py
@@ -70,6 +70,12 @@
     "fmc_conv3x3_halo_packed_bytes": (c_int64, [c_int, c_int]),
     "fmc_conv3x3_halo_pack_weight": (c_int, [c_void_p, c_void_p, c_int, c_int, c_void_p]),
     "fmc_conv3x3_halo_tiles_per_image": (c_int, [c_int, c_int]),
+    "fmc_conv3x3_halo_sc_supported": (c_int, [c_int, c_int, c_int, c_int, c_int, c_int, c_int]),
+    "fmc_conv3x3_halo_sc_packed_bytes": (c_int64, [c_int, c_int, c_int]),
+    "fmc_conv3x3_halo_sc_pack_source": (c_int64, [c_int64, c_int, c_int, c_int, ctypes.POINTER(c_int)]),
+    "fmc_conv3x3_halo_sc_pack_weight": (c_int, [c_void_p, c_void_p, c_void_p, c_int, c_int, c_int, c_int, c_void_p]),
+    "fmc_conv3x3_halo_sc_bf16": (c_int, [c_void_p, c_void_p, c_void_p, c_void_p, c_void_p, c_void_p, c_void_p, c_int, c_int, c_int, c_int, c_int,
+                                         c_int, c_int, c_int64, c_int, c_void_p, c_void_p]),
     "fmc_conv3x3_halo_bf16": (c_int, [c_void_p, c_void_p, c_int, c_void_p, c_void_p, c_void_p, c_void_p, c_void_p, c_int, c_int, c_int, c_int, c_int,
                                       c_int64, c_int, c_int, c_void_p, c_int, c_void_p, c_void_p]),
     "fmc_conv3x3_halo4_supported": (c_int, [c_int, c_int, c_int, c_int, c_int, c_int, c_int, c_int]),
diff --git a/synfmc_amd/csrc/conv_halo.hip b/synfmc_amd/csrc/conv_halo.hip
--- a/synfmc_amd/csrc/conv_halo.hip
+++ b/synfmc_amd/csrc/conv_halo.hip
@@ -20,6 +20,11 @@
     int tiles_y, tiles_x, tiles_n;
     int64_t x_bytes, x2_bytes, w_bytes;
 };
+struct CHParamsSC : CHParams {
+    const bf16_t* xs; const bf16_t* xs2;
+    int cs1, cin_sc;
+    int64_t xs_bytes, xs2_bytes;
+};
 
 __device__ __forceinline__ float silu_fast(float z) { return z * __builtin_amdgcn_rcpf(1.f + __builtin_amdgcn_exp2f(-1.4426950408889634f * z)); }
 
@@ -27,9 +32,13 @@
 
 constexpr int nhp(int i) { return (i >= 0 && i <= 3) ? (i < 3 ? 2 : 1) : 0; }
 
-template <int GN, bool PH = false>
+constexpr int NSCP = 5;
+template <bool SC> constexpr int nreq(int i) { return nh(i) + (SC && i == 16 ? NSCP : 0); }
+
+template <int GN, bool PH = false, bool SC = false>
 __global__ __launch_bounds__(512, 2)
-void conv_halo_kernel(const CHParams P) {
+void conv_halo_kernel(const std::conditional_t<SC, CHParamsSC, CHParams> P) {
+    static_assert(!SC || (GN == 0 && !PH), "the shortcut mode is a plain 9-tap convolution");
     extern __shared__ __attribute__((aligned(16))) unsigned char smem_raw[];
     const int tid = threadIdx.x, lane = tid & 63;
     const int wave = __builtin_amdgcn_readfirstlane(tid >> 6);
@@ -53,7 +62,10 @@
     const int tn1 = P.cout / BN;
     const int phase = PH ? tile_n / tn1 : 0, py = phase >> 1, px_ = phase & 1;
     const int n0 = (tile_n - phase * tn1) * BN;
-    const int nchunk = P.cin >> 6, nsub = nchunk * NS;
+    const int nchunk = P.cin >> 6;
+    int nsc = 0;
+    if constexpr (SC) nsc = P.cin_sc >> 6;
+    const int nsub = nchunk * NS + 2 * nsc;
 
     const int Hs = P.ups ? P.H >> 1 : P.H, Ws = P.ups ? P.W >> 1 : P.W;
     const int pp = lane & 7, pg = ((lane & 7) + (lane >> 3)) & 7;
@@ -74,7 +86,31 @@
     const __amdgpu_buffer_rsrc_t rsW = __builtin_amdgcn_make_buffer_rsrc((void*)P.w, 0, (int)P.w_bytes, 0x00020000);
     const int c2 = P.cin - P.c1;
     u32x4 hreg[2];
-    auto halo_load = [&](int j, int ch64, u32x4& dst) { dst = halo::piece_load(rsX, rsX2, P.c1, c2, h_pix[j], pg, ch64 * 64, ch64, nchunk); };
+    __amdgpu_buffer_rsrc_t rsS = rsX, rsS2 = rsX;
+    int cs1 = 0, cs2 = 0;
+    if constexpr (SC) {
+        rsS = __builtin_amdgcn_make_buffer_rsrc((void*)P.xs, 0, (int)P.xs_bytes, 0x00020000);
+        rsS2 = __builtin_amdgcn_make_buffer_rsrc((void*)(P.xs2 ? P.xs2 : P.xs), 0, (int)(P.xs2 ? P.xs2_bytes : P.xs_bytes), 0x00020000);
+        cs1 = P.cs1; cs2 = P.cin_sc - P.cs1;
+    }
+    auto halo_load = [&](int j, int ch64, u32x4& dst) {
+        if constexpr (SC) {
+            const bool sc = ch64 >= nchunk;
+            const int k = sc ? ch64 - nchunk : ch64;
+            dst = halo::piece_load(sc ? rsS : rsX, sc ? rsS2 : rsX2, sc ? cs1 : P.c1, sc ? cs2 : c2, h_pix[j], pg, k * 64, k, sc ? nsc : nchunk);
+        } else {
+            dst = halo::piece_load(rsX, rsX2, P.c1, c2, h_pix[j], pg, ch64 * 64, ch64, nchunk);
+        }
+    };
+    const int sc_row = wave >> 2;
+    const int sc_pix0 = (img * P.H + y0 + sc_row) * P.W + x0 + 8 * (wave & 3) + pp;
+    const int sc_lds = pg * PLANE + ((sc_row + 1) * HWID + 8 * (wave & 3) + pp + 1) * 16;
+    u32x4 hsc[NSCP];
+    auto sc_load = [&](int j, int k, u32x4& dst) {
+        const int hp = (k >= 0 && y0 + sc_row + 2 * j < P.H) ? sc_pix0 + 2 * j * P.W : -1;
+        dst = halo::piece_load(rsS, rsS2, cs1, cs2, hp, pg, k * 64, k, nsc);
+    };
+    auto sc_store = [&](int j, int buf, const u32x4& v) { *reinterpret_cast<u32x4*>(smem_raw + buf * HALO + sc_lds + j * (2 * HWID * 16)) = v; };
     auto halo_transform = [&](int j, int coefbuf, const u32x4& raw) -> u32x4 {
         if constexpr (GN == 0) return raw;
         const f32x4* src = reinterpret_cast<const f32x4*>(smem_raw + OFF_COEF + coefbuf * 512 + pg * 64);
@@ -217,9 +253,13 @@
                 }
                 if constexpr (nh(i) == 1) halo_load(i / 2, c + 1, hreg[(i / 2) & 1]);
                 if constexpr (i == 13) coef_next = coef_fetch(c + 2);
+                if constexpr (SC && i == 16) {
+#pragma unroll
+                    for (int j = 0; j < NSCP; ++j) sc_load(j, c + 2 - nchunk, hsc[j]);
+                }
                 w_issue(cls);
                 {
-                    constexpr int extra = nh(i - 1) + nh(i) + (i == 13 || i == 14 ? 1 : 0);
+                    constexpr int extra = nreq<SC>(i - 1) + nreq<SC>(i) + (i == 13 || i == 14 ? 1 : 0);
                     asm volatile("s_waitcnt vmcnt(%0)" ::"n"(2 * NW + extra) : "memory");
                 }
                 __builtin_amdgcn_sched_barrier(0);
@@ -248,6 +288,55 @@
             sub(IC<6>{}); sub(IC<7>{}); sub(IC<8>{}); sub(IC<9>{}); sub(IC<10>{}); sub(IC<11>{});
             sub(IC<12>{}); sub(IC<13>{}); sub(IC<14>{}); sub(IC<15>{}); sub(IC<16>{}); sub(IC<17>{});
             cbuf = nbuf;
+        }
+        if constexpr (SC) {
+            for (int k = 0; k < nsc; ++k) {
+                const int abase = cbuf * HALO, nbuf = cbuf ^ 1;
+                auto subs = [&](auto ic) {
+                    constexpr int hk = decltype(ic)::value;
+                    constexpr int aimm = hk * 4 * PLANE + (HWID + 1) * 16;
+                    if constexpr (hk == 1) {
+                        asm volatile("s_waitcnt vmcnt(%0)" ::"n"(2 * NW) : "memory");
+#pragma unroll
+                        for (int j = 0; j < NSCP; ++j) sc_store(j, nbuf, hsc[j]);
+                    }
+                    {
+                        const unsigned char* Wp = smem_raw + wfrag + rd_slot * WSUB;
+#pragma unroll
+                        for (int nb = 0; nb < 5; ++nb) wf[nb] = __builtin_bit_cast(bf16x8, *reinterpret_cast<const u32x4*>(Wp + nb * 1024));
+#pragma unroll
+                        for (int mb = 0; mb < 5; ++mb)
+                            af[mb] = __builtin_bit_cast(bf16x8, *reinterpret_cast<const u32x4*>(smem_raw + abase + afrag[mb] + aimm));
+                        rd_slot = rd_slot + 1 == NBW ? 0 : rd_slot + 1;
+                    }
+                    if constexpr (hk == 1) {
+#pragma unroll
+                        for (int j = 0; j < NSCP; ++j) sc_load(j, k + 2, hsc[j]);
+                    }
+                    w_issue(cls);
+                    if constexpr (hk == 0) {
+                        if (k == 0) asm volatile("s_waitcnt vmcnt(%0)" ::"n"(2 * NW) : "memory");
+                        else asm volatile("s_waitcnt vmcnt(%0)" ::"n"(2 * NW + NSCP) : "memory");
+                    } else {
+                        asm volatile("s_waitcnt vmcnt(%0) lgkmcnt(0)" ::"n"(2 * NW + NSCP) : "memory");
+                    }
+                    __builtin_amdgcn_sched_barrier(0);
+                    __builtin_amdgcn_s_barrier();
+                    __builtin_amdgcn_sched_barrier(0);
+                    __builtin_amdgcn_s_setprio(1);
+#pragma unroll
+                    for (int mb = 0; mb < 5; ++mb)
+#pragma unroll
+                        for (int nb = 0; nb < 5; ++nb)
+                            acc[mb][nb] = __builtin_amdgcn_mfma_f32_16x16x32_bf16(wf[nb], af[mb], acc[mb][nb], 0, 0, 0);
+                    __builtin_amdgcn_s_setprio(0);
+                    __builtin_amdgcn_sched_barrier(0);
+                    __builtin_amdgcn_s_barrier();
+                    __builtin_amdgcn_sched_barrier(0);
+                };
+                subs(IC<0>{}); subs(IC<1>{});
+                cbuf = nbuf;
+            }
         }
     };
     if (clsA) main_loop(std::true_type{}); else main_loop(std::false_type{});
@@ -372,6 +461,16 @@
         const int lc = p ^ (3 * ((row >> 3) & 1));
         const int64_t src = (((int64_t)(nt * BN + row) * 9 + tap) * cin + ch64 * 64 + hk * 32 + lc * 8);
         *reinterpret_cast<u32x4*>(dst + id * 8) = *reinterpret_cast<const u32x4*>(w + src);
+    }
+}
+
+__global__ __launch_bounds__(256) void conv_halo_sc_pack_kernel(const bf16_t* __restrict__ w, const bf16_t* __restrict__ wsc, bf16_t* __restrict__ dst,
+                                                                int cout, int cin, int cin_sc, int BN) {
+    const int64_t total = (int64_t)cout * (9 * cin + cin_sc) / 8;
+    for (int64_t id = (int64_t)blockIdx.x * blockDim.x + threadIdx.x; id < total; id += (int64_t)gridDim.x * blockDim.x) {
+        int from_sc;
+        const int64_t src = halo::sc_pack_source(id, cin, cin_sc, BN, &from_sc);
+        *reinterpret_cast<u32x4*>(dst + id * 8) = *reinterpret_cast<const u32x4*>((from_sc ? wsc : w) + src);
     }
 }
 
@@ -482,6 +581,58 @@
     return 0;
 }
 
+void halo::pack_filter_sc(const bf16_t* w, const bf16_t* w_sc, bf16_t* dst, int Cin, int Cout, int Cin_sc, int bn, hipStream_t st) {
+    const int64_t chunks = (int64_t)Cout * (9 * Cin + Cin_sc) / 8;
+    const int grid = (int)((chunks + 255) / 256 < 4096 ? (chunks + 255) / 256 : 4096);
+    hipLaunchKernelGGL(conv_halo_sc_pack_kernel, dim3(grid), dim3(256), 0, st, w, w_sc, dst, Cout, Cin, Cin_sc, bn);
+}
+
+extern "C" int64_t fmc_conv3x3_halo_sc_packed_bytes(int Cin, int Cout, int Cin_sc) { return (int64_t)Cout * (9 * Cin + Cin_sc) * 2; }
+
+extern "C" int fmc_conv3x3_halo_sc_pack_weight(const void* w, const void* w_sc, void* dst, int Cin, int Cout, int Cin_sc, int tile_channels, void* stream) {
+    if (!w || !w_sc || !dst) FMC_FAIL(FMC_E_NULL, "conv3x3_halo_sc_pack_weight: NULL pointer");
+    if ((tile_channels != 80 && tile_channels != 160) || Cin < 64 || Cin % 64 || Cin_sc < 64 || Cin_sc % 64 || Cout % tile_channels)
+        FMC_FAIL(FMC_E_SHAPE, "conv3x3_halo_sc_pack_weight: tile_channels 80 / 160, Cin %% 64, Cin_sc %% 64, Cout %% tile_channels (Cin=%d Cin_sc=%d Cout=%d tile=%d)",
+                 Cin, Cin_sc, Cout, tile_channels);
+    if (!fmc_aligned16(w) || !fmc_aligned16(w_sc) || !fmc_aligned16(dst)) FMC_FAIL(FMC_E_ALIGN, "conv3x3_halo_sc_pack_weight: pointers must be 16-byte aligned");
+    halo::pack_filter_sc((const bf16_t*)w, (const bf16_t*)w_sc, (bf16_t*)dst, Cin, Cout, Cin_sc, tile_channels, (hipStream_t)stream);
+    FMC_CHECK_LAUNCH("fmc_conv3x3_halo_sc_pack_weight");
+    return 0;
+}
+
+extern "C" int64_t fmc_conv3x3_halo_sc_pack_source(int64_t chunk, int Cin, int Cin_sc, int tile_channels, int* from_shortcut) {
+    int from_sc = 0;
+    const int64_t src = halo::sc_pack_source(chunk, Cin, Cin_sc, tile_channels, &from_sc);
+    if (from_shortcut) *from_shortcut = from_sc;
+    return src;
+}
+
+extern "C" int fmc_conv3x3_halo_sc_supported(int n_img, int H, int W, int Cin, int Cout, int Cin_sc, int Cin_sc1) {
+    if (!fmc_conv3x3_halo_supported(n_img, H, W, Cin, Cin, Cout, 0)) return 0;
+    return halo::sc_sources_ok(n_img, H, W, Cin, Cout, Cin_sc, Cin_sc1);
+}
+
+extern "C" int fmc_conv3x3_halo_sc_bf16(const void* x, const void* w_packed, const void* bias, const void* temb, void* out, const void* xs,
+                                        const void* xs2, int Cin_sc1, int Cin_sc, int n_img, int H, int W, int Cin, int Cout,
+                                        int64_t temb_row_stride, int temb_img_div, float* gn_partials, void* stream) {
+    if (!xs2) Cin_sc1 = Cin_sc;
+    if (int e = halo::check_args("conv3x3_halo_sc", true, x, nullptr, w_packed, bias, temb, nullptr, out, temb_row_stride, temb_img_div, gn_partials, Cout, BN,
+                                 fmc_conv3x3_halo_sc_supported(n_img, H, W, Cin, Cout, Cin_sc, Cin_sc1),
+                                 "%s: needs W %% 32 == 0, Cin %% 64 == 0, shortcut channels %% 64 == 0 (both sources), Cout %% 160 == 0, operands < 2 GiB "
+                                 "(n=%d H=%d W=%d Cin=%d Cout=%d shortcut=%d+%d)", n_img, H, W, Cin, Cout, Cin_sc1, Cin_sc - Cin_sc1))
+        return e;
+    if (int e = halo::check_sc_args("conv3x3_halo_sc", xs, xs2)) return e;
+    CHParamsSC P;
+    halo::fill_params(P, x, nullptr, Cin, w_packed, bias, temb, nullptr, out, n_img, H, W, Cin, Cout, temb_row_stride, temb_img_div, 0, gn_partials, 9);
+    halo::fill_params_sc(P, xs, xs2, Cin_sc1, Cin_sc);
+    P.gn_coef = nullptr; P.gn_act = 0;
+    P.tiles_y = (H + TH - 1) / TH; P.tiles_x = W / TW; P.tiles_n = Cout / BN;
+    const unsigned grid = (unsigned)(n_img * P.tiles_y * P.tiles_x * P.tiles_n);
+    fmc_launch<conv_halo_kernel<0, false, true>>(dim3(grid), dim3(512), LDS_BYTES, (hipStream_t)stream, P);
+    FMC_CHECK_LAUNCH("fmc_conv3x3_halo_sc_bf16");
+    return 0;
+}
+
 extern "C" int64_t fmc_conv3x3_upfold_packed_bytes(int Cin, int Cout) { return (int64_t)Cout * 16 * Cin * 2; }
 
 extern "C" int fmc_conv3x3_upfold_pack_weight(const void* w, void* dst, int Cin, int Cout, int tile_channels, void* stream) {
diff --git a/synfmc_amd/csrc/conv_halo_common.h b/synfmc_amd/csrc/conv_halo_common.h
--- a/synfmc_amd/csrc/conv_halo_common.h
+++ b/synfmc_amd/csrc/conv_halo_common.h
@@ -45,6 +45,7 @@
 };
 
 void pack_filter(const bf16_t* w, bf16_t* dst, int Cin, int Cout, int bn, hipStream_t st);
+void pack_filter_sc(const bf16_t* w, const bf16_t* w_sc, bf16_t* dst, int Cin, int Cout, int Cin_sc, int bn, hipStream_t st);
 
 template <class... A>
 int check_args(const char* name, bool full, const void* x, const void* x2, const void* w, const void* bias, const void* temb, const void* residual,
@@ -62,6 +63,43 @@
     return 0;
 }
 
+__host__ __device__ inline int64_t sc_pack_source(int64_t id, int cin, int cin_sc, int bn, int* from_sc) {
+    const int n3 = (cin >> 6) * 18, nsub = n3 + (cin_sc >> 6) * 2;
+    int64_t t = id;
+    const int p = (int)(t & 3); t >>= 2;
+    const int row = (int)(t % bn); t /= bn;
+    const int sub = (int)(t % nsub), nt = (int)(t / nsub);
+    const int lc = p ^ (3 * ((row >> 3) & 1));
+    const int64_t co = (int64_t)nt * bn + row;
+    *from_sc = sub >= n3;
+    if (sub < n3) {
+        const int hk = sub & 1, tap = (sub >> 1) % 9, ch64 = sub / 18;
+        return (co * 9 + tap) * cin + ch64 * 64 + hk * 32 + lc * 8;
+    }
+    const int hk = (sub - n3) & 1, ch64 = (sub - n3) >> 1;
+    return co * cin_sc + ch64 * 64 + hk * 32 + lc * 8;
+}
+
+inline int sc_sources_ok(int n_img, int H, int W, int Cin, int Cout, int Cin_sc, int Cin_sc1) {
+    if (Cin_sc < 64 || Cin_sc % 64 || Cin_sc1 <= 0 || Cin_sc1 > Cin_sc || Cin_sc1 % 64) return 0;
+    const int64_t px = (int64_t)n_img * H * W;
+    if (px * Cin_sc1 * 2 >= (1ll << 31) || px * (Cin_sc - Cin_sc1) * 2 >= (1ll << 31)) return 0;
+    if ((int64_t)Cout * (9 * (int64_t)Cin + Cin_sc) * 2 >= (1ll << 31)) return 0;
+    return 1;
+}
+inline int check_sc_args(const char* name, const void* xs, const void* xs2) {
+    if (!xs) FMC_FAIL(FMC_E_NULL, "%s: NULL shortcut input", name);
+    if (!fmc_aligned16(xs) || (xs2 && !fmc_aligned16(xs2))) FMC_FAIL(FMC_E_ALIGN, "%s: the shortcut inputs must be 16-byte aligned", name);
+    return 0;
+}
+template <class P_>
+void fill_params_sc(P_& P, const void* xs, const void* xs2, int Cin_sc1, int Cin_sc) {
+    P.xs = (const bf16_t*)xs; P.xs2 = (const bf16_t*)xs2; P.cs1 = Cin_sc1; P.cin_sc = Cin_sc;
+    const int64_t px = (int64_t)P.n_img * P.H * P.W;
+    P.xs_bytes = px * Cin_sc1 * 2; P.xs2_bytes = px * (Cin_sc - Cin_sc1) * 2;
+    P.w_bytes += (int64_t)P.cout * Cin_sc * 2;
+}
+
 template <class P_>
 void fill_params(P_& P, const void* x, const void* x2, int Cin1, const void* w, const void* bias, const void* temb, const void* residual, void* out,
                  int n_img, int H, int W, int Cin, int Cout, int64_t temb_row_stride, int temb_img_div, int upsample2x, float* gn_partials, int taps) {
diff --git a/synfmc_amd/hip_ops.py b/synfmc_amd/hip_ops.py
--- a/synfmc_amd/hip_ops.py
+++ b/synfmc_amd/hip_ops.py
@@ -1698,6 +1698,40 @@
     return _w_packed(weight_cl, "halo", 9, "fmc_conv3x3_halo_pack_weight")
 
 
+SHORTCUT_FOLD = os.environ.get("FMC_SHORTCUT_FOLD", "1") != "0"
+shortcut_fold_calls = {"folded": 0}
+
+
+def conv3x3_halo_sc_supported(n: int, h: int, w: int, cin: int, cout: int, cin_sc: int, cin_sc1: int) -> bool:
+    return bool(_lib.load().fmc_conv3x3_halo_sc_supported(n, h, w, cin, cout, cin_sc, cin_sc1))
+
+
+def _w_halo_sc_packed(weight_cl: torch.Tensor, w_sc: torch.Tensor, bn: int = 160) -> torch.Tensor:
+    def build():
+        cout, cin = weight_cl.shape[:2]
+        assert weight_cl.is_contiguous(memory_format=torch.channels_last) and w_sc.is_contiguous() and w_sc.shape[0] == cout
+        out = torch.empty(cout * (9 * cin + w_sc.shape[1]), dtype=weight_cl.dtype, device=weight_cl.device)
+        _lib.check(_lib.load().fmc_conv3x3_halo_sc_pack_weight(weight_cl.data_ptr(), w_sc.data_ptr(), out.data_ptr(), cin, cout, w_sc.shape[1], bn,
+                                                               _stream()), "fmc_conv3x3_halo_sc_pack_weight")
+        return out, w_sc
+    return derived_on_owner(weight_cl, "_fmc_wtm", ("halo_sc", bn, w_sc.data_ptr(), w_sc._version, w_sc.storage_offset(), tuple(w_sc.shape)), build)[0]
+
+
+def shortcut_fold_ok(x_nchw: torch.Tensor, weight_cl: torch.Tensor, xs: torch.Tensor, xs2: Optional[torch.Tensor]) -> bool:
+    if not (SHORTCUT_FOLD and CONV_HALO and not torch.is_grad_enabled() and x_nchw.is_cuda and weight_cl.dtype == torch.bfloat16
+            and all(t is None or (t.is_cuda and t.dtype == torch.bfloat16 and t.dim() == 4 and t.permute(0, 2, 3, 1).is_contiguous()) for t in (x_nchw, xs, xs2))
+            and weight_cl.is_contiguous(memory_format=torch.channels_last)):
+        return False
+    n, cin, h, w = x_nchw.shape
+    cout = weight_cl.shape[0]
+    if weight_cl.shape[1] != cin or xs.shape[0] != n or tuple(xs.shape[2:]) != (h, w) or (xs2 is not None and (xs2.shape[0] != n or tuple(xs2.shape[2:]) != (h, w))):
+        return False
+    cs1 = xs.shape[1]
+    cin_sc = cs1 + (xs2.shape[1] if xs2 is not None else 0)
+    return (conv3x3_halo_sc_supported(n, h, w, cin, cout, cin_sc, cs1)
+            and n * _lib.load().fmc_conv3x3_halo_tiles_per_image(h, w) * (cout // 160) >= CONV_HALO_MIN_TILES)
+
+
 def _gn_tagged(y, want: bool, cout: int):
     if not want:
         return y.permute(0, 3, 1, 2)
@@ -1788,14 +1822,32 @@
 
 
 def conv3x3_halo(x_nhwc: torch.Tensor, weight_cl: torch.Tensor, bias=None, temb=None, residual_nhwc=None, temb_div: int = 1, upsample: bool = False,
-                 x2_nhwc: Optional[torch.Tensor] = None, gn_coef: Optional[torch.Tensor] = None, gn_act: bool = True, emit_gn: bool = False):
+                 x2_nhwc: Optional[torch.Tensor] = None, gn_coef: Optional[torch.Tensor] = None, gn_act: bool = True, emit_gn: bool = False,
+                 shortcut=None):
     _dev(x_nhwc, weight_cl, bias, temb, residual_nhwc, x2_nhwc, gn_coef)
     n, h, w, c1, cin, cout = _halo_args(x_nhwc, weight_cl, temb, residual_nhwc, temb_div, upsample, x2_nhwc)
     assert gn_coef is None or (gn_coef.shape == (n, cin, 2) and gn_coef.dtype == torch.float32 and gn_coef.is_contiguous())
     L = _lib.load()
+    part = torch.empty(n, L.fmc_conv3x3_halo_tiles_per_image(h, w), 32, 2, dtype=torch.float32, device=x_nhwc.device) if emit_gn else None
+    if shortcut is not None:
+        xs, xs2, w_sc, b_sc = shortcut
+        _dev(xs, xs2, w_sc, b_sc)
+        assert temb is None and residual_nhwc is None and x2_nhwc is None and gn_coef is None and not upsample
+        cs1, cin_sc = xs.shape[3], w_sc.shape[1]
+        assert xs.is_contiguous() and xs.dtype == torch.bfloat16 and xs.shape[:3] == (n, h, w) and w_sc.shape[0] == cout and w_sc.dtype == torch.bfloat16
+        assert (cs1 == cin_sc) if xs2 is None else (xs2.is_contiguous() and xs2.dtype == xs.dtype and xs2.shape == (n, h, w, cin_sc - cs1))
+        assert b_sc is None or (b_sc.shape == (cout,) and b_sc.dtype == torch.bfloat16 and b_sc.is_contiguous())
+        wp = _w_halo_sc_packed(weight_cl, w_sc)
+        out = torch.empty(n, h, w, cout, dtype=x_nhwc.dtype, device=x_nhwc.device)
+        conv_halo_calls["conv"] += 1
+        shortcut_fold_calls["folded"] += 1
+        if call_log is not None:
+            call_log.append(("conv_halo", (n, h, w, cin, cout, False, cin_sc), 2.0 * n * h * w * cout * (9 * cin + cin_sc)))
+        _lib.check(L.fmc_conv3x3_halo_sc_bf16(x_nhwc.data_ptr(), wp.data_ptr(), _p(bias), _p(b_sc), out.data_ptr(), xs.data_ptr(), _p(xs2), cs1, cin_sc,
+                                              n, h, w, cin, cout, cout, n, _p(part), _stream()), "fmc_conv3x3_halo_sc_bf16")
+        return (out, part) if emit_gn else out
     wp = _w_halo_packed(weight_cl)
     out = torch.empty(n, h, w, cout, dtype=x_nhwc.dtype, device=x_nhwc.device)
-    part = torch.empty(n, L.fmc_conv3x3_halo_tiles_per_image(h, w), 32, 2, dtype=torch.float32, device=x_nhwc.device) if emit_gn else None
     conv_halo_calls["conv"] += 1
     conv_halo_calls["gn_fused"] += gn_coef is not None
     if call_log is not None:
@@ -2289,8 +2341,21 @@
 
 
 def conv3x3(x_nchw: torch.Tensor, weight_cl: torch.Tensor, bias, temb=None, residual_nchw=None, stride=(1, 1),
-            padding=(1, 1), temb_div: int = 1, upsample: bool = False, emit_gn: bool = False, own_only: bool = False) -> torch.Tensor:
+            padding=(1, 1), temb_div: int = 1, upsample: bool = False, emit_gn: bool = False, own_only: bool = False, shortcut=None) -> torch.Tensor:
     import torch.nn.functional as F
+
+    if shortcut is not None:
+        n, cin, h, w = x_nchw.shape
+        cout = weight_cl.shape[0]
+        xs, xs2, w_sc, b_sc = shortcut
+        assert temb is None and residual_nchw is None and not upsample and tuple(stride) == (1, 1) and tuple(padding) == (1, 1)
+        if not shortcut_fold_ok(x_nchw, weight_cl, xs, xs2):
+            raise RuntimeError("conv3x3: no kernel takes this shape with the shortcut in the reduction")
+        want = bool(emit_gn and GN_EPILOGUE and cout % 64 == 0 and 160 % (cout // 32) == 0)
+        dispatch_calls["conv3x3"]["own"] += 1
+        y = conv3x3_halo(x_nchw.permute(0, 2, 3, 1), weight_cl, bias, emit_gn=want,
+                         shortcut=(xs.permute(0, 2, 3, 1), None if xs2 is None else xs2.permute(0, 2, 3, 1), w_sc, b_sc))
+        return _gn_tagged(y, want, cout)
 
     def lib():
         xin = F.interpolate(x_nchw, scale_factor=2.0, mode="nearest") if upsample else x_nchw
diff --git a/synfmc_amd/models/layers.py b/synfmc_amd/models/layers.py
--- a/synfmc_amd/models/layers.py
+++ b/synfmc_amd/models/layers.py
@@ -136,7 +136,12 @@
 
     def forward(self, x: torch.Tensor, scale: float = 1.0, temb: Optional[torch.Tensor] = None,
                 residual: Optional[torch.Tensor] = None, temb_div: int = 1, upsample: bool = False,
-                x2: Optional[torch.Tensor] = None, emit_gn: bool = False) -> torch.Tensor:
+                x2: Optional[torch.Tensor] = None, emit_gn: bool = False, shortcut=None) -> torch.Tensor:
+        if shortcut is not None:
+            xs, xs2, sc = shortcut
+            assert temb is None and residual is None and not upsample and x2 is None
+            return K.conv3x3(x, self._weight_cl(), self.bias, emit_gn=emit_gn,
+                             shortcut=(xs, xs2, sc.weight.view(sc.out_channels, sc.in_channels), sc.bias))
         if self.kernel_size == (1, 1) and self.stride == (1, 1) and self.padding == (0, 0):
             n, c, h, w = x.shape
             assert temb is None
@@ -338,10 +343,23 @@
         if K.CONV_GN_FUSED and self._gn_fused_ok(input_tensor, skip, t):
             return self._forward_gn_fused(input_tensor, skip, t, div)
         h = self.conv1(self.norm1(input_tensor, act=True, x2=skip), temb=t, temb_div=div, emit_gn=True)
+        a2 = self.norm2(h, act=True)
+        if self.conv_shortcut is not None and self._shortcut_fold_ok(a2, input_tensor, skip):
+            out = self.conv2(a2, emit_gn=True, shortcut=(input_tensor, skip, self.conv_shortcut))
+            return out if self.output_scale_factor == 1.0 else out / self.output_scale_factor
         if self.conv_shortcut is not None:
             input_tensor = self.conv_shortcut(input_tensor, x2=skip)
-        out = self.conv2(self.norm2(h, act=True), residual=input_tensor, emit_gn=True)
+        out = self.conv2(a2, residual=input_tensor, emit_gn=True)
         return out if self.output_scale_factor == 1.0 else out / self.output_scale_factor
+
+    def _shortcut_fold_ok(self, a2, x, skip) -> bool:
+        c2, sc = self.conv2, self.conv_shortcut
+        if not (a2.is_cuda and a2.dtype == torch.bfloat16 and c2.weight.dtype == torch.bfloat16 and sc.weight.dtype == torch.bfloat16
+                and not torch.is_grad_enabled() and sc.kernel_size == (1, 1) and sc.stride == (1, 1) and sc.padding == (0, 0)
+                and sc.weight.is_contiguous() and c2.kernel_size == (3, 3) and c2.stride == (1, 1) and c2.padding == (1, 1)
+                and c2.dilation == (1, 1) and c2.groups == 1 and a2.is_contiguous(memory_format=torch.channels_last)):
+            return False
+        return K.shortcut_fold_ok(a2, c2._weight_cl(), x, skip)
 
 
     def _gn_fused_ok(self, x, skip, t) -> bool:
```

New measurement: 40.65 steps/s, median of 6. 1.01x the previous value.
